# CSU-KangHu/HiTE

Measured on AMD Instinct MI355X. Metric: candidate TE boundaries/sec on 1 Gbp synthetic genome (fine stage: copy finding+gather+align+vote+judge), higher is better.
Workload: dtype u8; 1 GPU; C3: 1000 Mbp synthetic genome, 2500 TIR + 2500 LTR families, 50000 candidates/GPU judged as TIR (copy finding by minimizer-index lookup inside the timed step; index build 0.0 s untimed); genome_bp=1000000000, candidates_per_gpu=50000, candidate_bases=192511237, copies=799813, copy_table=found, is_te=34225, parallelism=replicated genome, candidates per rank x1, all-gather of 32-B calls

## Files before the change

hite_amd/csrc/hite_align.hip:

```cpp
#include "hite_common.h"
#include "hite_scan.h"
#include "hite_arena.h"
#include "hite_sort.h"
#include "hite_align.h"

#define AL_GAP 3
#define AL_STEER 24
#define AL_MARGIN 48
#define AL_PADR 1056
#define AL_WIDE_NW 64
#define AL_STRIP 16
#define AL_RECB 4096
#define AL_DEFAULT_CAP 8
#define AL_KBINS 2048
#define AL_LANES_MIN_STRIPS 32

struct AlignArgs {
    const uint8_t *win;
    const int64_t *win_off;
    const int32_t *win_len;
    const int32_t *row_first;
    int n_cand;
    const int32_t *row_cand;
    const uint4 *planes;
    const int64_t *plane_off;
    const unsigned long long *rec;
    int32_t *U, *kst, *st, *lvl, *U4;
    const int64_t *ops_base;
    uint16_t *ops;
    const int64_t *full_off;
    uint32_t *fullbuf;
    int32_t *fullt;
};

__device__ __forceinline__ uint32_t alignbit(uint32_t hi, uint32_t lo, uint32_t sh) { return __builtin_amdgcn_alignbit(hi, lo, sh); }
__device__ __forceinline__ uint32_t add_co_mask(uint32_t a, uint32_t b, unsigned long long &carry_mask) {
    uint32_t r;
    asm volatile("v_add_co_u32_e64 %0, %1, %2, %3" : "=v"(r), "=s"(carry_mask) : "v"(a), "v"(b));
    return r;
}
__device__ __forceinline__ uint32_t add_mask_bit(uint32_t a, unsigned long long mask) {
    uint32_t r;
    unsigned long long dummy;
    asm volatile("v_addc_co_u32_e64 %0, %1, %2, 0, %3" : "=v"(r), "=s"(dummy) : "v"(a), "s"(mask));
    return r;
}
__device__ __forceinline__ int wave_max_i32(int v) {
#pragma unroll
    for (int d = 32; d >= 1; d >>= 1) { int o = __shfl_xor(v, d, 64); v = o > v ? o : v; }
    return v;
}
__device__ __forceinline__ bool is_acgt_byte(unsigned c) { c &= 0xdfu; return c - 0x41u < 32u && ((0x00080045u >> (c - 0x41u)) & 1u); }

struct BaseMask { uint32_t m0, m1, inv; };
__device__ __forceinline__ BaseMask base_mask(unsigned ch) {
    BaseMask b;
    b.m0 = (uint32_t)(-(int)((ch >> 1) & 1u));
    b.m1 = (uint32_t)(-(int)((ch >> 2) & 1u));
    b.inv = is_acgt_byte(ch) ? 0u : 0xffffffffu;
    return b;
}

template <int NW, bool DIRS, int TAP>
__device__ __forceinline__ void bp_core(uint32_t (&X2)[NW], uint32_t (&X1)[NW], uint32_t (&X0)[NW], const uint32_t (&A0)[NW],
                                        const uint32_t (&A1)[NW], const uint32_t (&AN)[NW], const BaseMask bm, uint32_t cin, uint32_t vpc,
                                        uint32_t h2c, uint32_t h1c, uint32_t h0c, uint32_t *dg, uint32_t *up, uint32_t *tap) {
#pragma unroll
    for (int w = 0; w < NW; w++) {
        if (TAP >= 0 && w == TAP) { tap[0] = cin; tap[1] = vpc; tap[2] = h2c; tap[3] = h1c; tap[4] = h0c; }
        const uint32_t eq = ~((A0[w] ^ bm.m0) | (A1[w] ^ bm.m1) | AN[w] | bm.inv);
        const uint32_t x2 = X2[w], x1 = X1[w], x0 = X0[w];
        const uint32_t vneg = ~(x2 | x1 | x0), vpos = x2 & x1;
        const uint32_t B = eq | vneg, P = (vpos << 1) | vpc;
        vpc = vpos >> 31;
        const uint32_t Y = P | B;
        unsigned cout;
        const uint32_t sum = __builtin_addc(B, Y, cin, &cout);
        cin = cout;
        const uint32_t Z = B | (P & (sum ^ B ^ Y));
        const uint32_t h0 = ~(Z ^ x0), b1 = Z & x0, h1 = ~(x1 ^ b1), b2 = x1 & b1, h2 = ~(x2 ^ b2);
        const uint32_t s2 = (h2 << 1) | h2c, s1 = (h1 << 1) | h1c, s0 = (h0 << 1) | h0c;
        h2c = h2 >> 31; h1c = h1 >> 31; h0c = h0 >> 31;
        const uint32_t n0 = ~(Z ^ s0), c1 = Z & s0, n1 = ~(s1 ^ c1), c2 = s1 & c1, n2 = ~(s2 ^ c2);
        X2[w] = n2; X1[w] = n1; X0[w] = n0;
        if (DIRS) { dg[w] = eq | ~Z; up[w] = n2 & n1; }
    }
}
__device__ __forceinline__ int slope_count(uint32_t x2, uint32_t x1, uint32_t x0) { return __popc(x2) - __popc(~x2 & ~(x1 & x0)); }
__device__ __forceinline__ int plane_sum(uint32_t x2, uint32_t x1, uint32_t x0, uint32_t mask) {
    return 4 * __popc(x2 & mask) + 2 * __popc(x1 & mask) + __popc(x0 & mask);
}

__global__ void __launch_bounds__(256) align_rows_kernel(int n_cand, const int32_t *__restrict__ row_first,
                                                         const int32_t *__restrict__ win_len, int32_t *__restrict__ row_cand,
                                                         int32_t *__restrict__ strips, unsigned long long *__restrict__ keys,
                                                         unsigned *__restrict__ vals) {
    const int c = blockIdx.x;
    if (c >= n_cand) return;
    const int g0 = row_first[c], g1 = row_first[c + 1];
    for (int g = g0 + threadIdx.x; g < g1; g += 256) {
        row_cand[g] = c;
        const int k = g == g0 ? 0 : (win_len[g] + AL_STRIP - 1) / AL_STRIP;
        strips[g] = k;
        keys[g] = (unsigned long long)(AL_KBINS - 1 - (k >= AL_KBINS ? AL_KBINS - 1 : k));
        vals[g] = (unsigned)g;
    }
}
__global__ void align_plane_words_kernel(int n_cand, const int32_t *__restrict__ row_first, const int32_t *__restrict__ win_len,
                                         int32_t *__restrict__ words) {
    const int c = blockIdx.x * blockDim.x + threadIdx.x;
    if (c >= n_cand) return;
    const int g0 = row_first[c];
    words[c] = row_first[c + 1] > g0 ? (win_len[g0] + 2 * AL_PADR) / 32 + 3 : 0;
}
__global__ void __launch_bounds__(256) align_planes_kernel(int n_cand, const uint8_t *__restrict__ win, const int64_t *__restrict__ win_off,
                                                           const int32_t *__restrict__ win_len, const int32_t *__restrict__ row_first,
                                                           const int64_t *__restrict__ plane_off, uint4 *__restrict__ planes) {
    const int c = blockIdx.x;
    if (c >= n_cand) return;
    const int g0 = row_first[c];
    if (row_first[c + 1] <= g0) return;
    const int m = win_len[g0];
    const uint8_t *a = win + win_off[g0];
    const int nw = (m + 2 * AL_PADR) / 32 + 3;
    uint4 *out = planes + plane_off[c];
    for (int wi = threadIdx.x; wi < nw; wi += 256) {
        uint32_t p0 = 0, p1 = 0, pn = 0;
        unsigned chs[32];
#pragma unroll
        for (int k = 0; k < 32; k++) {
            const int r = wi * 32 + k - AL_PADR + 1;
            chs[k] = a[r < 1 || m < 1 ? 0 : (r > m ? m - 1 : r - 1)];
        }
#pragma unroll
        for (int k = 0; k < 32; k++) {
            const int r = wi * 32 + k - AL_PADR + 1;
            const unsigned ch = (r >= 1 && r <= m) ? chs[k] : 0u;
            if (is_acgt_byte(ch)) { p0 |= ((ch >> 1) & 1u) << k; p1 |= ((ch >> 2) & 1u) << k; }
            else pn |= 1u << k;
        }
        out[wi] = make_uint4(p0, p1, pn, 0u);
    }
}

#ifdef ALIGN_CLOCKS
#define ALIGN_CLK_MAX (1 << 17)
__device__ unsigned long long g_aclk[2][4][ALIGN_CLK_MAX];
extern "C" int hite_debug_align_clocks(int which, unsigned long long *out, int n) {
    if (which < 0 || which > 1 || n > ALIGN_CLK_MAX) return -1;
    for (int k = 0; k < 4; k++)
        if (hipMemcpyFromSymbol(out + (size_t)k * n, HIP_SYMBOL(g_aclk), sizeof(unsigned long long) * n,
                                ((size_t)which * 4 + k) * ALIGN_CLK_MAX * sizeof(unsigned long long)) != hipSuccess) return -1;
    unsigned long long *z = (unsigned long long *)calloc((size_t)4 * ALIGN_CLK_MAX, sizeof(unsigned long long));
    if (z) { (void)hipMemcpyToSymbol(HIP_SYMBOL(g_aclk), z, sizeof(unsigned long long) * 4 * ALIGN_CLK_MAX, (size_t)which * 4 * ALIGN_CLK_MAX * sizeof(unsigned long long)); free(z); }
    return 0;
}
__device__ __forceinline__ unsigned aclk_hw_id() {
    unsigned v, x;
    asm volatile("s_getreg_b32 %0, hwreg(HW_REG_HW_ID)" : "=s"(v));
    asm volatile("s_getreg_b32 %0, hwreg(HW_REG_XCC_ID)" : "=s"(x));
    return ((x & 0xfu) << 16) | (v & 0xffffu);
}
#define ACLK_BEGIN(which) const unsigned long long aclk_t0 = wall_clock64(); const int aclk_w = (which)
#define ACLK_END() do { if (threadIdx.x == 0 && blockIdx.x < ALIGN_CLK_MAX) { g_aclk[aclk_w][0][blockIdx.x] = aclk_t0; \
    g_aclk[aclk_w][1][blockIdx.x] = wall_clock64(); g_aclk[aclk_w][2][blockIdx.x] = aclk_hw_id(); g_aclk[aclk_w][3][blockIdx.x] = (unsigned long long)nmax; } } while (0)
#else
#define ACLK_BEGIN(which) do { } while (0)
#define ACLK_END() do { } while (0)
#endif

template <int NW>
__device__ __forceinline__ void align_fwd_body(const AlignArgs &P, const int32_t *__restrict__ list, int nlist) {
    constexpr int W = 32 * NW, H = W / 2, S0 = NW / 2 - 1;
    ACLK_BEGIN(0);
    const int li = blockIdx.x * 64 + threadIdx.x;
    const int g = li < nlist ? list[li] : -1;
    int m = 0, n = 0, g0 = 0, c = 0;
    if (g >= 0) {
        c = P.row_cand[g];
        g0 = P.row_first[c];
        if (g != g0) { m = P.win_len[g0]; n = P.win_len[g]; }
    }
    const int nmax = wave_max_i32(n);
    if (nmax == 0) return;
    const uint8_t *b = P.win + (g >= 0 ? P.win_off[g] : 0);
    const uint4 *pl = P.planes + (g >= 0 ? P.plane_off[c] : 0);
    char *rec0 = g >= 0 ? reinterpret_cast<char *>(P.rec[g]) : nullptr;
    uint32_t X2[NW], X1[NW], X0[NW], A0[NW], A1[NW], AN[NW];
    int t = -H;
#pragma unroll
    for (int w = 0; w < NW; w++) { X2[w] = w >= NW / 2 ? 0xffffffffu : 0u; X1[w] = X2[w]; X0[w] = 0u; }
    bool act = n > 0;
    if (act) {
        const int q0 = (t + AL_PADR) >> 5;
#pragma unroll
        for (int w = 0; w < NW; w++) { const uint4 v = pl[q0 + w]; A0[w] = v.x; A1[w] = v.y; AN[w] = v.z; }
    } else {
#pragma unroll
        for (int w = 0; w < NW; w++) { A0[w] = 0; A1[w] = 0; AN[w] = 0xffffffffu; }
    }
    int stop = AL_GAP * H, LO = -(1 << 28), HI = 1 << 28, status = 0;
    int fq = (t + W + AL_PADR) >> 5;
    uint4 Wa = make_uint4(0, 0, 0xffffffffu, 0), Wb = Wa, Wc = Wa, bnext = make_uint4(0, 0, 0, 0);
    if (act) { Wa = pl[fq]; Wb = pl[fq + 1]; Wc = pl[fq + 2]; bnext = *reinterpret_cast<const uint4 *>(b); }
    for (int k = 0; k * AL_STRIP < nmax; k++) {
        const bool sa = act && k * AL_STRIP < n;
        uint4 bw = make_uint4(0, 0, 0, 0);
        uint32_t f0 = 0, f1 = 0, fn = 0;
        uint32_t brec[8] = {0, 0, 0, 0, 0, 0, 0, 0};
        if (sa) {
            uint4 *ck = reinterpret_cast<uint4 *>(rec0 + (size_t)k * AL_RECB);
            ck[0] = make_uint4(X2[S0], X2[S0 + 1], X1[S0], X1[S0 + 1]);
            ck[1] = make_uint4(X0[S0], X0[S0 + 1], (uint32_t)(t + 32 * S0), 0u);
            bw = bnext;
            if ((k + 1) * AL_STRIP < n) bnext = *reinterpret_cast<const uint4 *>(b + (k + 1) * AL_STRIP);
            const int fx = t + W + AL_PADR;
            if ((fx >> 5) != fq) { Wa = Wb; Wb = Wc; fq++; Wc = pl[fq + 2]; }
            const uint32_t sh = (uint32_t)fx & 31u;
            f0 = alignbit(Wb.x, Wa.x, sh); f1 = alignbit(Wb.y, Wa.y, sh); fn = alignbit(Wb.z, Wa.z, sh);
        }
#pragma unroll
        for (int cc = 0; cc < AL_STRIP; cc++) {
            const int j = k * AL_STRIP + cc + 1;
            if (sa && j <= n) {
                if ((cc & 3) == 0) {
                    const int ds = slope_count(X2[S0], X1[S0], X0[S0]) + slope_count(X2[S0 + 1], X1[S0 + 1], X0[S0 + 1]);
                    int s = ds > AL_STEER ? 0 : (ds < -AL_STEER ? 8 : 4);
                    const int tr = m - H;
                    if (t + s > tr) s = (tr - t) & ~3;
                    const int need = tr - 3 - 8 * ((n - j) >> 2) - t;
                    if (s < need) s = (need + 3) & ~3;
                    if (s > 8) { status = 2; act = false; s = 8; }
                    stop += plane_sum(X2[0], X1[0], X0[0], (1u << s) - 1u) - AL_GAP * s;
                    unsigned long long rec = (unsigned long long)(s >> 2);
                    if (NW > 2) {
                        rec |= (unsigned long long)(X2[S0 + 2 < NW ? S0 + 2 : 0] & 0xffu) << 2;
                        rec |= (unsigned long long)(X1[S0 + 2 < NW ? S0 + 2 : 0] & 0xffu) << 10;
                        rec |= (unsigned long long)(X0[S0 + 2 < NW ? S0 + 2 : 0] & 0xffu) << 18;
                    }
                    brec[(cc >> 2) * 2] = (uint32_t)rec;
#pragma unroll
                    for (int w = 0; w < NW - 1; w++) {
                        X2[w] = alignbit(X2[w + 1], X2[w], (uint32_t)s); X1[w] = alignbit(X1[w + 1], X1[w], (uint32_t)s);
                        X0[w] = alignbit(X0[w + 1], X0[w], (uint32_t)s);
                        A0[w] = alignbit(A0[w + 1], A0[w], (uint32_t)s); A1[w] = alignbit(A1[w + 1], A1[w], (uint32_t)s);
                        AN[w] = alignbit(AN[w + 1], AN[w], (uint32_t)s);
                    }
                    X2[NW - 1] = alignbit(0xffffffffu, X2[NW - 1], (uint32_t)s);
                    X1[NW - 1] = alignbit(0xffffffffu, X1[NW - 1], (uint32_t)s);
                    X0[NW - 1] = X0[NW - 1] >> s;
                    A0[NW - 1] = alignbit(f0, A0[NW - 1], (uint32_t)s); A1[NW - 1] = alignbit(f1, A1[NW - 1], (uint32_t)s);
                    AN[NW - 1] = alignbit(fn, AN[NW - 1], (uint32_t)s);
                    f0 >>= s; f1 >>= s; fn >>= s;
                    t += s;
                    if (t >= 1) { const int v = t + 1 - j; LO = v > LO ? v : LO; }
                    if (t + W < m) { const int jl = j + 3 < n ? j + 3 : n; const int v = t + W - jl; HI = v < HI ? v : HI; }
                }
                stop += AL_GAP;
                const uint32_t word = cc < 4 ? bw.x : (cc < 8 ? bw.y : (cc < 12 ? bw.z : bw.w));
                const BaseMask bm = base_mask((word >> (8 * (cc & 3))) & 0xffu);
                uint32_t tap[5] = {0, 0, 1, 1, 0};
                bp_core<NW, false, (NW > 2 ? S0 : -1)>(X2, X1, X0, A0, A1, AN, bm, 0u, 0u, 1u, 1u, 0u, nullptr, nullptr, tap);
                if (NW > 2) {
                    const uint32_t c5 = tap[0] | (tap[1] << 1) | (tap[2] << 2) | (tap[3] << 3) | (tap[4] << 4);
                    const int sh = 26 + 5 * (cc & 3);
                    if (sh + 5 <= 32) brec[(cc >> 2) * 2] |= c5 << sh;
                    else if (sh >= 32) brec[(cc >> 2) * 2 + 1] |= c5 << (sh - 32);
                    else { brec[(cc >> 2) * 2] |= c5 << sh; brec[(cc >> 2) * 2 + 1] |= c5 >> (32 - sh); }
                    brec[(cc >> 2) * 2 + 1] |= ((bm.m0 & 1u) | (bm.m1 & 2u) | (bm.inv & 4u)) << (14 + 3 * (cc & 3));
                }
            }
        }
        if (NW > 2 && sa) {
            uint4 *bp = reinterpret_cast<uint4 *>(rec0 + (size_t)k * AL_RECB + AL_RECB / 2);
            bp[0] = make_uint4(brec[0], brec[1], brec[2], brec[3]);
            bp[1] = make_uint4(brec[4], brec[5], brec[6], brec[7]);
        }
    }
    if (n > 0) {
        int U = -1, kstar = -1;
        if (status == 0) {
            int u = stop - AL_GAP * H;
#pragma unroll
            for (int w = 0; w < NW / 2; w++) u += plane_sum(X2[w], X1[w], X0[w], 0xffffffffu);
            {
                const int extra = m - H - t;
                u += plane_sum(X2[NW / 2], X1[NW / 2], X0[NW / 2], (1u << extra) - 1u) - AL_GAP * extra;
            }
            U = u;
            const int d = m - n, dmin = d < 0 ? d : 0, dmax = d > 0 ? d : 0, ad = d < 0 ? -d : d;
            int E = dmin - LO;
            if (HI - dmax < E) E = HI - dmax;
            if (E > (1 << 27)) kstar = 0x7fffffff;
            else if (E >= 0) kstar = AL_GAP * ad + 2 * AL_GAP * E + 2 * AL_GAP - 1;
        }
        P.U[g] = U; P.kst[g] = kstar; P.st[g] = status; P.lvl[g] = NW;
        if (NW == 4) P.U4[g] = U;
    }
    if (NW == 4) ACLK_END();
}
template <int NW>
__global__ void __launch_bounds__(64) align_fwd_kernel(AlignArgs P, const int32_t *__restrict__ list, int nlist) { align_fwd_body<NW>(P, list, nlist); }
#ifdef ALIGN_FWD4_OCC
#define ALIGN_FWD4_ATTR __attribute__((amdgpu_waves_per_eu(ALIGN_FWD4_OCC, ALIGN_FWD4_OCC)))
#else
#define ALIGN_FWD4_ATTR
#endif
__global__ void __launch_bounds__(64) ALIGN_FWD4_ATTR align_fwd4_kernel(AlignArgs P, const int32_t *__restrict__ list, int nlist) { align_fwd_body<4>(P, list, nlist); }

__device__ __forceinline__ uint32_t pair_partner(uint32_t v) { return (uint32_t)__builtin_amdgcn_update_dpp(0, (int)v, 0xB1, 0xf, 0xf, false); }

__global__ void __launch_bounds__(64) align_fwd8_pair_kernel(AlignArgs P, const int32_t *__restrict__ list, int nlist) {
    constexpr int NW = 8, HW = 4, W = 32 * NW, H = W / 2, S0 = NW / 2 - 1;
    const int half = threadIdx.x & 1;
    const int li = blockIdx.x * 32 + (threadIdx.x >> 1);
    const int g = li < nlist ? list[li] : -1;
    int m = 0, n = 0, g0 = 0, c = 0;
    if (g >= 0) {
        c = P.row_cand[g];
        g0 = P.row_first[c];
        if (g != g0) { m = P.win_len[g0]; n = P.win_len[g]; }
    }
    const int nmax = wave_max_i32(n);
    if (nmax == 0) return;
    const uint8_t *b = P.win + (g >= 0 ? P.win_off[g] : 0);
    const uint4 *pl = P.planes + (g >= 0 ? P.plane_off[c] : 0);
    char *rec0 = g >= 0 ? reinterpret_cast<char *>(P.rec[g]) : nullptr;
    uint32_t X2[HW], X1[HW], X0[HW], A0[HW], A1[HW], AN[HW];
    int t = -H;
#pragma unroll
    for (int w = 0; w < HW; w++) { X2[w] = half ? 0xffffffffu : 0u; X1[w] = X2[w]; X0[w] = 0u; }
    bool act = n > 0;
    if (act) {
        const int q0 = ((t + AL_PADR) >> 5) + half * HW;
#pragma unroll
        for (int w = 0; w < HW; w++) { const uint4 v = pl[q0 + w]; A0[w] = v.x; A1[w] = v.y; AN[w] = v.z; }
    } else {
#pragma unroll
        for (int w = 0; w < HW; w++) { A0[w] = 0; A1[w] = 0; AN[w] = 0xffffffffu; }
    }
    int stop = AL_GAP * H, LO = -(1 << 28), HI = 1 << 28, status = 0;
    int fq = (t + W + AL_PADR) >> 5;
    uint4 Wa = make_uint4(0, 0, 0xffffffffu, 0), Wb = Wa, Wc = Wa, bnext = make_uint4(0, 0, 0, 0);
    if (act) { Wa = pl[fq]; Wb = pl[fq + 1]; Wc = pl[fq + 2]; bnext = *reinterpret_cast<const uint4 *>(b); }
    for (int k = 0; k * AL_STRIP < nmax; k++) {
        const bool sa = act && k * AL_STRIP < n;
        uint4 bw = make_uint4(0, 0, 0, 0);
        uint32_t f0 = 0, f1 = 0, fn = 0;
        uint32_t brec[8] = {0, 0, 0, 0, 0, 0, 0, 0};
        {
            const uint32_t p2 = pair_partner(X2[0]), p1 = pair_partner(X1[0]), p0 = pair_partner(X0[0]);
            if (sa && !half) {
                uint4 *ck = reinterpret_cast<uint4 *>(rec0 + (size_t)k * AL_RECB);
                ck[0] = make_uint4(X2[HW - 1], p2, X1[HW - 1], p1);
                ck[1] = make_uint4(X0[HW - 1], p0, (uint32_t)(t + 32 * S0), 0u);
            }
        }
        if (sa) {
            bw = bnext;
            if ((k + 1) * AL_STRIP < n) bnext = *reinterpret_cast<const uint4 *>(b + (k + 1) * AL_STRIP);
            const int fx = t + W + AL_PADR;
            if ((fx >> 5) != fq) { Wa = Wb; Wb = Wc; fq++; Wc = pl[fq + 2]; }
            const uint32_t sh = (uint32_t)fx & 31u;
            f0 = alignbit(Wb.x, Wa.x, sh); f1 = alignbit(Wb.y, Wa.y, sh); fn = alignbit(Wb.z, Wa.z, sh);
        }
#pragma unroll
        for (int cc = 0; cc < AL_STRIP; cc++) {
            const int j = k * AL_STRIP + cc + 1;
            const bool on = sa && j <= n;
            if ((cc & 3) == 0) {
                const int own = half ? slope_count(X2[0], X1[0], X0[0]) : slope_count(X2[HW - 1], X1[HW - 1], X0[HW - 1]);
                const int ds = own + (int)pair_partner((uint32_t)own);
                const uint32_t i2 = pair_partner(X2[1] & 0xffu), i1 = pair_partner(X1[1] & 0xffu), i0 = pair_partner(X0[1] & 0xffu);
                const uint32_t u2 = pair_partner(X2[0]), u1 = pair_partner(X1[0]), u0 = pair_partner(X0[0]);
                const uint32_t ua0 = pair_partner(A0[0]), ua1 = pair_partner(A1[0]), uan = pair_partner(AN[0]);
                if (on) {
                    int s = ds > AL_STEER ? 0 : (ds < -AL_STEER ? 8 : 4);
                    const int tr = m - H;
                    if (t + s > tr) s = (tr - t) & ~3;
                    const int need = tr - 3 - 8 * ((n - j) >> 2) - t;
                    if (s < need) s = (need + 3) & ~3;
                    if (s > 8) { status = 2; act = false; s = 8; }
                    if (!half) {
                        stop += plane_sum(X2[0], X1[0], X0[0], (1u << s) - 1u) - AL_GAP * s;
                        brec[(cc >> 2) * 2] = (uint32_t)(s >> 2) | (i2 << 2) | (i1 << 10) | (i0 << 18);
                    }
#pragma unroll
                    for (int w = 0; w < HW - 1; w++) {
                        X2[w] = alignbit(X2[w + 1], X2[w], (uint32_t)s); X1[w] = alignbit(X1[w + 1], X1[w], (uint32_t)s);
                        X0[w] = alignbit(X0[w + 1], X0[w], (uint32_t)s);
                        A0[w] = alignbit(A0[w + 1], A0[w], (uint32_t)s); A1[w] = alignbit(A1[w + 1], A1[w], (uint32_t)s);
                        AN[w] = alignbit(AN[w + 1], AN[w], (uint32_t)s);
                    }
                    X2[HW - 1] = alignbit(half ? 0xffffffffu : u2, X2[HW - 1], (uint32_t)s);
                    X1[HW - 1] = alignbit(half ? 0xffffffffu : u1, X1[HW - 1], (uint32_t)s);
                    X0[HW - 1] = alignbit(half ? 0u : u0, X0[HW - 1], (uint32_t)s);
                    A0[HW - 1] = alignbit(half ? f0 : ua0, A0[HW - 1], (uint32_t)s);
                    A1[HW - 1] = alignbit(half ? f1 : ua1, A1[HW - 1], (uint32_t)s);
                    AN[HW - 1] = alignbit(half ? fn : uan, AN[HW - 1], (uint32_t)s);
                    f0 >>= s; f1 >>= s; fn >>= s;
                    t += s;
                    if (t >= 1) { const int v = t + 1 - j; LO = v > LO ? v : LO; }
                    if (t + W < m) { const int jl = j + 3 < n ? j + 3 : n; const int v = t + W - jl; HI = v < HI ? v : HI; }
                }
            }
            const uint32_t word = cc < 4 ? bw.x : (cc < 8 ? bw.y : (cc < 12 ? bw.z : bw.w));
            const BaseMask bm = base_mask((word >> (8 * (cc & 3))) & 0xffu);
            uint32_t Bv[HW], Pv[HW], Yv[HW], Sv[HW], eqv[HW], vposv[HW];
#pragma unroll
            for (int w = 0; w < HW; w++) {
                eqv[w] = ~((A0[w] ^ bm.m0) | (A1[w] ^ bm.m1) | AN[w] | bm.inv);
                vposv[w] = X2[w] & X1[w];
                Bv[w] = eqv[w] | ~(X2[w] | X1[w] | X0[w]);
            }
            const uint32_t pvpos = pair_partner(vposv[HW - 1]);
            const uint32_t vin = half ? pvpos >> 31 : 0u;
            uint32_t cin = 0u, tap0 = 0u;
#pragma unroll
            for (int w = 0; w < HW; w++) {
                if (w == HW - 1) tap0 = cin;
                Pv[w] = (vposv[w] << 1) | (w ? vposv[w - 1] >> 31 : vin);
                Yv[w] = Pv[w] | Bv[w];
                unsigned cout;
                Sv[w] = __builtin_addc(Bv[w], Yv[w], cin, &cout);
                cin = cout;
            }
            {
                const uint32_t pc = pair_partner(cin);
                uint32_t e = half ? pc : 0u;
#pragma unroll
                for (int w = 0; w < HW; w++) { const uint32_t o = Sv[w]; Sv[w] = o + e; e &= (o == 0xffffffffu) ? 1u : 0u; }
            }
            uint32_t Zv[HW], h2v[HW], h1v[HW], h0v[HW];
#pragma unroll
            for (int w = 0; w < HW; w++) {
                Zv[w] = Bv[w] | (Pv[w] & (Sv[w] ^ Bv[w] ^ Yv[w]));
                const uint32_t b1 = Zv[w] & X0[w], b2 = X1[w] & b1;
                h0v[w] = ~(Zv[w] ^ X0[w]); h1v[w] = ~(X1[w] ^ b1); h2v[w] = ~(X2[w] ^ b2);
            }
            const uint32_t q2 = pair_partner(h2v[HW - 1]) >> 31, q1 = pair_partner(h1v[HW - 1]) >> 31, q0 = pair_partner(h0v[HW - 1]) >> 31;
            const uint32_t hin2 = half ? q2 : 1u, hin1 = half ? q1 : 1u, hin0 = half ? q0 : 0u;
            if (on) {
#pragma unroll
                for (int w = 0; w < HW; w++) {
                    const uint32_t s2 = (h2v[w] << 1) | (w ? h2v[w - 1] >> 31 : hin2), s1 = (h1v[w] << 1) | (w ? h1v[w - 1] >> 31 : hin1),
                                   s0 = (h0v[w] << 1) | (w ? h0v[w - 1] >> 31 : hin0);
                    const uint32_t c1 = Zv[w] & s0, c2 = s1 & c1;
                    X0[w] = ~(Zv[w] ^ s0); X1[w] = ~(s1 ^ c1); X2[w] = ~(s2 ^ c2);
                }
                if (!half) {
                    stop += AL_GAP;
                    const uint32_t c5 = tap0 | ((vposv[HW - 2] >> 31) << 1) | ((h2v[HW - 2] >> 31) << 2) | ((h1v[HW - 2] >> 31) << 3) | ((h0v[HW - 2] >> 31) << 4);
                    const int sh = 26 + 5 * (cc & 3);
                    if (sh + 5 <= 32) brec[(cc >> 2) * 2] |= c5 << sh;
                    else if (sh >= 32) brec[(cc >> 2) * 2 + 1] |= c5 << (sh - 32);
                    else { brec[(cc >> 2) * 2] |= c5 << sh; brec[(cc >> 2) * 2 + 1] |= c5 >> (32 - sh); }
                    brec[(cc >> 2) * 2 + 1] |= ((bm.m0 & 1u) | (bm.m1 & 2u) | (bm.inv & 4u)) << (14 + 3 * (cc & 3));
                }
            }
        }
        if (sa && !half) {
            uint4 *bp = reinterpret_cast<uint4 *>(rec0 + (size_t)k * AL_RECB + AL_RECB / 2);
            bp[0] = make_uint4(brec[0], brec[1], brec[2], brec[3]);
            bp[1] = make_uint4(brec[4], brec[5], brec[6], brec[7]);
        }
    }
    {
        const int extra = m - H - t;
        const uint32_t part = pair_partner((uint32_t)plane_sum(X2[0], X1[0], X0[0], (1u << (extra & 31)) - 1u));
        if (n > 0 && !half) {
            int U = -1, kstar = -1;
            if (status == 0) {
                int u = stop - AL_GAP * H;
#pragma unroll
                for (int w = 0; w < HW; w++) u += plane_sum(X2[w], X1[w], X0[w], 0xffffffffu);
                u += (int)part - AL_GAP * extra;
                U = u;
                const int d = m - n, dmin = d < 0 ? d : 0, dmax = d > 0 ? d : 0, ad = d < 0 ? -d : d;
                int E = dmin - LO;
                if (HI - dmax < E) E = HI - dmax;
                if (E > (1 << 27)) kstar = 0x7fffffff;
                else if (E >= 0) kstar = AL_GAP * ad + 2 * AL_GAP * E + 2 * AL_GAP - 1;
            }
            P.U[g] = U; P.kst[g] = kstar; P.st[g] = status; P.lvl[g] = NW;
        }
    }
}

template <int CTRL>
__device__ __forceinline__ uint32_t dpp_row(uint32_t v) { return (uint32_t)__builtin_amdgcn_update_dpp(0, (int)v, CTRL, 0xf, 0xf, true); }
template <int G>
__device__ __forceinline__ int grp_sum(int v) {
    v += (int)dpp_row<0xB1>((uint32_t)v);
    v += (int)dpp_row<0x4E>((uint32_t)v);
    if (G == 8) v += (int)dpp_row<0x141>((uint32_t)v);
    return v;
}
__device__ __forceinline__ int wave_min_i32(int v) {
#pragma unroll
    for (int d = 32; d >= 1; d >>= 1) { int o = __shfl_xor(v, d, 64); v = o < v ? o : v; }
    return v;
}
__device__ __forceinline__ uint32_t bit_mask(uint32_t w, int bit) { return (uint32_t)((int32_t)(w << (31 - bit)) >> 31); }
template <int GI>
__device__ __forceinline__ uint32_t quad_bcast(uint32_t v) { return dpp_row<GI * 0x55>(v); }
struct LaneFwd {
    uint32_t X2, X1, X0, A0, A1, AN, f0, f1, fn;
    int t, stop, LO, HI, status;
    bool act;
};
template <int G, bool FULL>
__device__ __forceinline__ void lanes_strip(LaneFwd &S, const uint4 bw, const uint32_t invm, const uint32_t code12, const bool sa, const int k,
                                            const int m, const int n, const int q, const uint32_t K1, const unsigned long long TOPM, uint32_t (&brec)[8]) {
    constexpr int NW = G, W = 32 * NW, H = W / 2, S0 = NW / 2 - 1;
    const bool top = q == G - 1;
#pragma unroll
    for (int cc = 0; cc < AL_STRIP; cc++) {
        const int j = k * AL_STRIP + cc + 1;
        const bool on = FULL || (sa && j <= n);
        if ((cc & 3) == 0) {
            const int ds = grp_sum<G>((q == S0 || q == S0 + 1) ? slope_count(S.X2, S.X1, S.X0) : 0);
            const uint32_t i2 = dpp_row<0x102>(S.X2) & 0xffu, i1 = dpp_row<0x102>(S.X1) & 0xffu, i0 = dpp_row<0x102>(S.X0) & 0xffu;
            const uint32_t u2 = dpp_row<0x101>(S.X2), u1 = dpp_row<0x101>(S.X1), u0 = dpp_row<0x101>(S.X0);
            const uint32_t ua0 = dpp_row<0x101>(S.A0), ua1 = dpp_row<0x101>(S.A1), uan = dpp_row<0x101>(S.AN);
            constexpr int gi = 0;
            const uint32_t cg = (cc >> 2) == 0 ? quad_bcast<0>(code12) : ((cc >> 2) == 1 ? quad_bcast<1>(code12) : ((cc >> 2) == 2 ? quad_bcast<2>(code12) : quad_bcast<3>(code12)));
            (void)gi;
            if (on) {
                int s = ds > AL_STEER ? 0 : (ds < -AL_STEER ? 8 : 4);
                const int tr = m - H;
                if (S.t + s > tr) s = (tr - S.t) & ~3;
                const int need = tr - 3 - 8 * ((n - j) >> 2) - S.t;
                if (s < need) s = (need + 3) & ~3;
                if (s > 8) { S.status = 2; S.act = false; s = 8; }
                S.stop += plane_sum(S.X2, S.X1, S.X0, (1u << s) - 1u) - AL_GAP * s;
                brec[(cc >> 2) * 2] = (uint32_t)(s >> 2) | (i2 << 2) | (i1 << 10) | (i0 << 18);
                brec[(cc >> 2) * 2 + 1] = cg << 14;
                S.X2 = alignbit(top ? 0xffffffffu : u2, S.X2, (uint32_t)s);
                S.X1 = alignbit(top ? 0xffffffffu : u1, S.X1, (uint32_t)s);
                S.X0 = alignbit(top ? 0u : u0, S.X0, (uint32_t)s);
                S.A0 = alignbit(top ? S.f0 : ua0, S.A0, (uint32_t)s);
                S.A1 = alignbit(top ? S.f1 : ua1, S.A1, (uint32_t)s);
                S.AN = alignbit(top ? S.fn : uan, S.AN, (uint32_t)s);
                S.f0 >>= s; S.f1 >>= s; S.fn >>= s;
                S.t += s;
                if (S.t >= 1) { const int v = S.t + 1 - j; S.LO = v > S.LO ? v : S.LO; }
                if (S.t + W < m) { const int jl = j + 3 < n ? j + 3 : n; const int v = S.t + W - jl; S.HI = v < S.HI ? v : S.HI; }
            }
        }
        const uint32_t word = cc < 4 ? bw.x : (cc < 8 ? bw.y : (cc < 12 ? bw.z : bw.w));
        const uint32_t m0 = bit_mask(word, 8 * (cc & 3) + 1), m1 = bit_mask(word, 8 * (cc & 3) + 2), inv = bit_mask(invm, cc);
        const uint32_t eq = ~((S.A0 ^ m0) | (S.A1 ^ m1) | S.AN | inv);
        const uint32_t vpos = S.X2 & S.X1;
        const uint32_t B = eq | ~(S.X2 | S.X1 | S.X0);
        const uint32_t pvr = dpp_row<0x111>(vpos);
        const uint32_t Pp = alignbit(vpos, pvr, 31) & ~K1;
        const uint32_t Y = Pp | B;
        unsigned long long Gm;
        const uint32_t sum0 = add_co_mask(B, Y, Gm);
        uint32_t sum;
        {
            const unsigned long long Pm = __ballot(sum0 == 0xffffffffu);
            const unsigned long long Gc = Gm & ~TOPM, Yy = (Pm | Gm) & ~TOPM, ss = Gc + Yy;
            sum = add_mask_bit(sum0, ss ^ Gc ^ Yy);
        }
        const uint32_t Z = B | (Pp & (sum ^ B ^ Y));
        const uint32_t h0 = ~(Z ^ S.X0), b1 = Z & S.X0, h1 = ~(S.X1 ^ b1), b2 = S.X1 & b1, h2 = ~(S.X2 ^ b2);
        const uint32_t r2 = dpp_row<0x111>(h2), r1 = dpp_row<0x111>(h1), r0 = dpp_row<0x111>(h0);
        if (on) {
            const uint32_t s2 = alignbit(h2, r2, 31) | K1, s1 = alignbit(h1, r1, 31) | K1, s0 = alignbit(h0, r0, 31) & ~K1;
            const uint32_t c1 = Z & s0, c2 = s1 & c1;
            S.X0 = ~(Z ^ s0); S.X1 = ~(s1 ^ c1); S.X2 = ~(s2 ^ c2);
            uint32_t c5 = alignbit(r0 >> 31, r1, 31);
            c5 = alignbit(c5, r2, 31);
            c5 = alignbit(c5, pvr, 31);
            c5 = (c5 << 1) | (sum - sum0);
            const int sh = 26 + 5 * (cc & 3);
            if (sh + 5 <= 32) brec[(cc >> 2) * 2] |= c5 << sh;
            else if (sh >= 32) brec[(cc >> 2) * 2 + 1] |= c5 << (sh - 32);
            else { brec[(cc >> 2) * 2] |= c5 << sh; brec[(cc >> 2) * 2 + 1] |= c5 >> (32 - sh); }
        }
    }
}
__device__ __forceinline__ uint32_t decode_bases4(uint32_t w) {
    uint32_t r = 0;
#pragma unroll
    for (int x = 0; x < 4; x++) {
        const unsigned ch = (w >> (8 * x)) & 0xffu;
        const uint32_t bad = is_acgt_byte(ch) ? 0u : 1u;
        r |= (bad << x) | ((((ch >> 1) & 3u) | (bad << 2)) << (4 + 3 * x));
    }
    return r;
}
template <int G>
__global__ void __launch_bounds__(64) align_fwd_lanes_kernel(AlignArgs P, const int32_t *__restrict__ list, int nlist) {
    constexpr int NW = G, W = 32 * NW, H = W / 2, S0 = NW / 2 - 1, PPW = 64 / G;
    const int q = threadIdx.x & (G - 1);
    const int li = blockIdx.x * PPW + (int)(threadIdx.x / G);
    const int g = li < nlist ? list[li] : -1;
    int m = 0, n = 0, g0 = 0, c = 0;
    if (g >= 0) {
        c = P.row_cand[g];
        g0 = P.row_first[c];
        if (g != g0) { m = P.win_len[g0]; n = P.win_len[g]; }
    }
    const int nmax = wave_max_i32(n);
    if (nmax == 0) return;
    const int nfull = wave_min_i32(n > 0 ? n : 0x7fffffff);
    const bool wr = q == S0;
    const uint32_t K1 = q == 0 ? 1u : 0u;
    const unsigned long long TOPM = G == 4 ? 0x8888888888888888ull : 0x8080808080808080ull;
    const uint8_t *b = P.win + (g >= 0 ? P.win_off[g] : 0);
    const uint4 *pl = P.planes + (g >= 0 ? P.plane_off[c] : 0);
    char *rec0 = g >= 0 ? reinterpret_cast<char *>(P.rec[g]) : nullptr;
    LaneFwd S;
    S.X2 = q >= NW / 2 ? 0xffffffffu : 0u; S.X1 = S.X2; S.X0 = 0u; S.A0 = 0u; S.A1 = 0u; S.AN = 0xffffffffu;
    S.f0 = S.f1 = S.fn = 0u;
    S.t = -H;
    S.act = n > 0;
    if (S.act) { const uint4 v = pl[((S.t + AL_PADR) >> 5) + q]; S.A0 = v.x; S.A1 = v.y; S.AN = v.z; }
    S.stop = AL_GAP * H; S.LO = -(1 << 28); S.HI = 1 << 28; S.status = 0;
    int fq = (S.t + W + AL_PADR) >> 5;
    uint4 Wa = make_uint4(0, 0, 0xffffffffu, 0), Wb = Wa, Wc = Wa, bnext = make_uint4(0, 0, 0, 0);
    if (S.act) { Wa = pl[fq]; Wb = pl[fq + 1]; Wc = pl[fq + 2]; bnext = *reinterpret_cast<const uint4 *>(b); }
    for (int k = 0; k * AL_STRIP < nmax; k++) {
        const bool sa = S.act && k * AL_STRIP < n;
        uint4 bw = make_uint4(0, 0, 0, 0);
        uint32_t brec[8] = {0, 0, 0, 0, 0, 0, 0, 0};
        {
            const uint32_t p2 = dpp_row<0x101>(S.X2), p1 = dpp_row<0x101>(S.X1), p0 = dpp_row<0x101>(S.X0);
            if (sa && wr) {
                uint4 *ck = reinterpret_cast<uint4 *>(rec0 + (size_t)k * AL_RECB);
                ck[0] = make_uint4(S.X2, p2, S.X1, p1);
                ck[1] = make_uint4(S.X0, p0, (uint32_t)(S.t + 32 * S0), 0u);
            }
        }
        S.f0 = S.f1 = S.fn = 0u;
        if (sa) {
            bw = bnext;
            if ((k + 1) * AL_STRIP < n) bnext = *reinterpret_cast<const uint4 *>(b + (k + 1) * AL_STRIP);
            const int fx = S.t + W + AL_PADR;
            if ((fx >> 5) != fq) { Wa = Wb; Wb = Wc; fq++; Wc = pl[fq + 2]; }
            const uint32_t sh = (uint32_t)fx & 31u;
            S.f0 = alignbit(Wb.x, Wa.x, sh); S.f1 = alignbit(Wb.y, Wa.y, sh); S.fn = alignbit(Wb.z, Wa.z, sh);
        }
        const uint32_t dq = (q & 3) == 0 ? bw.x : ((q & 3) == 1 ? bw.y : ((q & 3) == 2 ? bw.z : bw.w));
        const uint32_t dec = decode_bases4(dq);
        uint32_t invm = (dec & 15u) << (4 * (q & 3));
        invm |= dpp_row<0xB1>(invm);
        invm |= dpp_row<0x4E>(invm);
        const bool failed = __any(n > 0 && S.status != 0);
        if ((k + 1) * AL_STRIP <= nfull && !failed) lanes_strip<G, true>(S, bw, invm, dec >> 4, sa, k, m, n, q, K1, TOPM, brec);
        else lanes_strip<G, false>(S, bw, invm, dec >> 4, sa, k, m, n, q, K1, TOPM, brec);
        if (sa && wr) {
            uint4 *bp = reinterpret_cast<uint4 *>(rec0 + (size_t)k * AL_RECB + AL_RECB / 2);
            bp[0] = make_uint4(brec[0], brec[1], brec[2], brec[3]);
            bp[1] = make_uint4(brec[4], brec[5], brec[6], brec[7]);
        }
    }
    {
        const int extra = m - H - S.t;
        const int part = q < NW / 2 ? plane_sum(S.X2, S.X1, S.X0, 0xffffffffu) : (q == NW / 2 ? plane_sum(S.X2, S.X1, S.X0, (1u << (extra & 31)) - 1u) : 0);
        const int tot = grp_sum<G>(part + (q == 0 ? S.stop : 0));
        if (n > 0 && wr) {
            int U = -1, kstar = -1;
            if (S.status == 0) {
                U = tot + AL_GAP * n - AL_GAP * H - AL_GAP * extra;
                const int d = m - n, dmin = d < 0 ? d : 0, dmax = d > 0 ? d : 0, ad = d < 0 ? -d : d;
                int E = dmin - S.LO;
                if (S.HI - dmax < E) E = S.HI - dmax;
                if (E > (1 << 27)) kstar = 0x7fffffff;
                else if (E >= 0) kstar = AL_GAP * ad + 2 * AL_GAP * E + 2 * AL_GAP - 1;
            }
            P.U[g] = U; P.kst[g] = kstar; P.st[g] = S.status; P.lvl[g] = NW;
            if (NW == 4) P.U4[g] = U;
        }
    }
}

typedef unsigned int tb_u32x4 __attribute__((ext_vector_type(4)));
#if defined(ALIGN_TB_STORE8)
struct OpsOut {
    uint16_t *ops;
    unsigned long long acc, top;
    int m;
    __device__ __forceinline__ void init(uint16_t *row, int m_) { ops = row; m = m_; acc = 0ull; top = 0ull; }
    __device__ __forceinline__ void push(int pos, uint32_t val) {
        acc = (acc << 16) | (unsigned long long)(val & 0xffffu);
        if ((pos & 3) == 0) {
            if (pos + 4 <= m) *reinterpret_cast<unsigned long long *>(ops + pos) = acc;
            else top = acc;
        }
    }
    __device__ __forceinline__ void finish() {
        const int k = m & 3, p0 = m & ~3;
        for (int x = 0; x < k; x++) ops[p0 + x] = (uint16_t)(top >> (16 * x));
    }
};
#elif defined(ALIGN_TB_STORE32)
struct OpsOut {
    uint16_t *ops;
    unsigned long long acc;
    unsigned long long g0, g1, g2, g3;
    int m, off;
    int q_low;
    __device__ __forceinline__ void init(uint16_t *row, int m_) {
        ops = row; m = m_; acc = 0ull; g0 = g1 = g2 = g3 = 0ull;
        off = (int)((reinterpret_cast<uintptr_t>(row) >> 1) & 15);
        q_low = m_ + off;
    }
    __device__ __forceinline__ uint16_t held(int q, int q_acc_low) const {
        if ((q >> 2) == (q_acc_low >> 2) && (q_acc_low & 3)) return (uint16_t)(acc >> (16 * (q - q_acc_low)));
        const int g = (q >> 2) & 3;
        const unsigned long long s = g == 0 ? g0 : (g == 1 ? g1 : (g == 2 ? g2 : g3));
        return (uint16_t)(s >> (16 * (q & 3)));
    }
    __device__ __forceinline__ void push(int pos, uint32_t val) {
        acc = (acc << 16) | (unsigned long long)(val & 0xffffu);
        const int q = pos + off;
        if ((q & 3) == 0) {
            const int g = (q >> 2) & 3;
            g0 = g == 0 ? acc : g0; g1 = g == 1 ? acc : g1; g2 = g == 2 ? acc : g2; g3 = g == 3 ? acc : g3;
            if (g == 0) {
                if (pos + 16 <= m) {
                    tb_u32x4 *dst = reinterpret_cast<tb_u32x4 *>(ops + pos);
                    tb_u32x4 v0, v1;
                    v0.x = (unsigned)g0; v0.y = (unsigned)(g0 >> 32); v0.z = (unsigned)g1; v0.w = (unsigned)(g1 >> 32);
                    v1.x = (unsigned)g2; v1.y = (unsigned)(g2 >> 32); v1.z = (unsigned)g3; v1.w = (unsigned)(g3 >> 32);
                    dst[0] = v0; dst[1] = v1;
                } else {
                    for (int x = pos; x < m; x++) ops[x] = held(x + off, q);
                }
                q_low = q;
            }
        }
    }
    __device__ __forceinline__ void finish() {
        const int top = q_low - off < m ? q_low - off : m;
        for (int x = 0; x < top; x++) ops[x] = held(x + off, off);
    }
};

#else
struct OpsOut {
    uint16_t *ops;
    unsigned long long acc, hi;
    unsigned long long tacc, thi;
    int m, off;
    __device__ __forceinline__ void init(uint16_t *row, int m_) {
        ops = row; m = m_; acc = 0ull; hi = 0ull; tacc = 0ull; thi = 0ull;
        off = (int)((reinterpret_cast<uintptr_t>(row) >> 1) & 7);
    }
    __device__ __forceinline__ void push(int pos, uint32_t val) {
        acc = (acc << 16) | (unsigned long long)(val & 0xffffu);
        const int q = pos + off;
        if ((q & 3) == 0) {
            if (q & 4) hi = acc;
            else if (pos + 8 <= m) {
                tb_u32x4 v;
                v.x = (unsigned)acc; v.y = (unsigned)(acc >> 32); v.z = (unsigned)hi; v.w = (unsigned)(hi >> 32);
                *reinterpret_cast<tb_u32x4 *>(ops + pos) = v;
            } else { tacc = acc; thi = hi; }
        }
    }
    __device__ __forceinline__ void finish() {
        const int t0 = m - ((m + off) & 7);
        if (t0 >= 0) for (int x = t0; x < m; x++) { const int qq = x + off; ops[x] = (uint16_t)(((qq & 4) ? thi : tacc) >> (16 * (qq & 3))); }
        const int b0 = (8 - off) & 7;
        const int lowm = b0 < m ? b0 : m;
        for (int x = 0; x < lowm; x++) {
            const int qq = x + off;
            const bool in_acc = (off & 3) != 0 && (qq >> 2) == (off >> 2);
            ops[x] = in_acc ? (uint16_t)(acc >> (16 * x)) : (uint16_t)(hi >> (16 * (qq & 3)));
        }
    }
};
#endif

#ifdef ALIGN_TB_OCC
#define ALIGN_TB_ATTR __attribute__((amdgpu_waves_per_eu(ALIGN_TB_OCC, ALIGN_TB_OCC)))
#else
#define ALIGN_TB_ATTR
#endif
__global__ void __launch_bounds__(64) ALIGN_TB_ATTR align_tb_kernel(AlignArgs P, const int32_t *__restrict__ list, int nlist) {
    ACLK_BEGIN(1);
    const int li = blockIdx.x * 64 + threadIdx.x;
    const int g = li < nlist ? list[li] : -1;
    int m = 0, n = 0, g0 = 0, c = 0;
    if (g >= 0) {
        c = P.row_cand[g];
        g0 = P.row_first[c];
        if (g != g0 && P.st[g] == 0) { m = P.win_len[g0]; n = P.win_len[g]; }
    }
    const int nmax = wave_max_i32(n);
    if (nmax == 0) return;
    const uint4 *pl = P.planes + (g >= 0 ? P.plane_off[c] : 0);
    const char *rec0 = g >= 0 ? reinterpret_cast<const char *>(P.rec[g]) : nullptr;
    uint16_t *ops = P.ops + (g >= 0 ? P.ops_base[c] + (int64_t)(g - g0) * (m + 1) : 0);
    int i = m, j = n;
    bool fail = false;
    OpsOut out;
    out.init(ops, m);
    const int Kmax = (nmax + AL_STRIP - 1) / AL_STRIP;
    const int K = (n + AL_STRIP - 1) / AL_STRIP;
    struct Pw { uint32_t x, y, z; };
    uint4 ckA0, ckA1, ckB0, ckB1, bdA0, bdA1;
    Pw plA[4];
    ckA0 = ckA1 = ckB0 = ckB1 = bdA0 = bdA1 = make_uint4(0, 0, 0, 0);
#pragma unroll
    for (int w = 0; w < 4; w++) { plA[w].x = 0; plA[w].y = 0; plA[w].z = 0; }
    {
        const int k = Kmax - 1;
        if (k < K) {
            const uint4 *ck = reinterpret_cast<const uint4 *>(rec0 + (size_t)k * AL_RECB);
            ckA0 = ck[0]; ckA1 = ck[1];
            const uint4 *bp = reinterpret_cast<const uint4 *>(rec0 + (size_t)k * AL_RECB + AL_RECB / 2);
            bdA0 = bp[0]; bdA1 = bp[1];
            const int q0 = ((int)ckA1.z + AL_PADR) >> 5;
#pragma unroll
            for (int w = 0; w < 4; w++) { const uint4 v = pl[q0 + w]; plA[w].x = v.x; plA[w].y = v.y; plA[w].z = v.z; }
        }
        if (k >= 1 && k - 1 < K) {
            const uint4 *ck = reinterpret_cast<const uint4 *>(rec0 + (size_t)(k - 1) * AL_RECB);
            ckB0 = ck[0]; ckB1 = ck[1];
        }
    }
    for (int k = Kmax - 1; k >= 0; k--) {
        const bool sa = n > 0 && !fail && i > 0 && k < K;
        uint4 ckC0 = make_uint4(0, 0, 0, 0), ckC1 = ckC0, bdB0 = ckC0, bdB1 = ckC0;
        Pw plB[4];
#pragma unroll
        for (int w = 0; w < 4; w++) { plB[w].x = 0; plB[w].y = 0; plB[w].z = 0; }
        if (k >= 1 && k - 1 < K && !fail && i > 0) {
            const uint4 *bp = reinterpret_cast<const uint4 *>(rec0 + (size_t)(k - 1) * AL_RECB + AL_RECB / 2);
            bdB0 = bp[0]; bdB1 = bp[1];
            const int q0 = ((int)ckB1.z + AL_PADR) >> 5;
#pragma unroll
            for (int w = 0; w < 4; w++) { const uint4 v = pl[q0 + w]; plB[w].x = v.x; plB[w].y = v.y; plB[w].z = v.z; }
        }
        if (k >= 2 && k - 2 < K && !fail && i > 0) {
            const uint4 *ck = reinterpret_cast<const uint4 *>(rec0 + (size_t)(k - 2) * AL_RECB);
            ckC0 = ck[0]; ckC1 = ck[1];
        }
        if (__any(sa)) {
        uint32_t X2[2], X1[2], X0[2], A0[2], A1[2], AN[2];
        uint32_t f0 = 0, f1 = 0, fn = 0;
        uint32_t brec[8] = {0, 0, 0, 0, 0, 0, 0, 0};
        int t = 0;
        if (sa) {
            X2[0] = ckA0.x; X2[1] = ckA0.y; X1[0] = ckA0.z; X1[1] = ckA0.w; X0[0] = ckA1.x; X0[1] = ckA1.y;
            t = (int)ckA1.z;
            brec[0] = bdA0.x; brec[1] = bdA0.y; brec[2] = bdA0.z; brec[3] = bdA0.w;
            brec[4] = bdA1.x; brec[5] = bdA1.y; brec[6] = bdA1.z; brec[7] = bdA1.w;
            const uint32_t sh = (uint32_t)(t + AL_PADR) & 31u;
#pragma unroll
            for (int w = 0; w < 2; w++) {
                A0[w] = alignbit(plA[w + 1].x, plA[w].x, sh); A1[w] = alignbit(plA[w + 1].y, plA[w].y, sh);
                AN[w] = alignbit(plA[w + 1].z, plA[w].z, sh);
            }
            f0 = alignbit(plA[3].x, plA[2].x, sh); f1 = alignbit(plA[3].y, plA[2].y, sh); fn = alignbit(plA[3].z, plA[2].z, sh);
        } else {
#pragma unroll
            for (int w = 0; w < 2; w++) { X2[w] = 0; X1[w] = 0; X0[w] = 0; A0[w] = 0; A1[w] = 0; AN[w] = 0; }
        }
        unsigned long long dg[AL_STRIP], up[AL_STRIP];
        uint32_t sbits = 0;
#pragma unroll
        for (int cc = 0; cc < AL_STRIP; cc++) {
            const int jc = k * AL_STRIP + cc + 1;
            dg[cc] = 0ull; up[cc] = 0ull;
            if (sa && jc <= n) {
                const uint32_t rlo = brec[(cc >> 2) * 2], rhi = brec[(cc >> 2) * 2 + 1];
                if ((cc & 3) == 0) {
                    const uint32_t s = (rlo & 3u) << 2;
                    const uint32_t in2 = (rlo >> 2) & 0xffu, in1 = (rlo >> 10) & 0xffu, in0 = (rlo >> 18) & 0xffu;
                    X2[0] = alignbit(X2[1], X2[0], s); X1[0] = alignbit(X1[1], X1[0], s); X0[0] = alignbit(X0[1], X0[0], s);
                    A0[0] = alignbit(A0[1], A0[0], s); A1[0] = alignbit(A1[1], A1[0], s); AN[0] = alignbit(AN[1], AN[0], s);
                    X2[1] = alignbit(in2, X2[1], s); X1[1] = alignbit(in1, X1[1], s); X0[1] = alignbit(in0, X0[1], s);
                    A0[1] = alignbit(f0, A0[1], s); A1[1] = alignbit(f1, A1[1], s); AN[1] = alignbit(fn, AN[1], s);
                    f0 >>= s; f1 >>= s; fn >>= s;
                    t += (int)s;
                    sbits |= (rlo & 3u) << (2 * (cc >> 2));
                }
                const int sh = 26 + 5 * (cc & 3);
                const uint32_t c5 = (sh + 5 <= 32 ? rlo >> sh : (sh >= 32 ? rhi >> (sh - 32) : (rlo >> sh) | (rhi << (32 - sh)))) & 31u;
                const uint32_t code = rhi >> (14 + 3 * (cc & 3));
                BaseMask bm;
                bm.m0 = 0u - (code & 1u); bm.m1 = 0u - ((code >> 1) & 1u); bm.inv = 0u - ((code >> 2) & 1u);
                uint32_t tap[5], dgc[2], upc[2];
                bp_core<2, true, -1>(X2, X1, X0, A0, A1, AN, bm, c5 & 1u, (c5 >> 1) & 1u, (c5 >> 2) & 1u, (c5 >> 3) & 1u, (c5 >> 4) & 1u, dgc, upc, tap);
                dg[cc] = ((unsigned long long)dgc[1] << 32) | dgc[0];
                up[cc] = ((unsigned long long)upc[1] << 32) | upc[0];
            }
        }
        int tcur = t;
#pragma unroll
        for (int cc = AL_STRIP - 1; cc >= 0; cc--) {
            const int jc = k * AL_STRIP + cc + 1;
            if (sa && !fail && i > 0 && j == jc) {
                const int kb = i - tcur - 1;
                if ((unsigned)kb >= 64u) fail = true;
                else {
                    const unsigned long long stopm = (dg[cc] | ~up[cc]) & (0xffffffffffffffffull >> (63 - kb));
                    if (stopm == 0ull) fail = true;
                    else {
                        const int ps = 63 - __clzll(stopm);
                        int ups = kb - ps;
                        if (ups > i) ups = i;
                        const uint32_t gapv = (uint32_t)j | 0x8000u;
                        for (int x = 0; x < ups; x++) out.push(i - 1 - x, gapv);
                        i -= ups;
                        if (i > 0) {
                            if ((dg[cc] >> ps) & 1ull) { out.push(i - 1, (uint32_t)(j - 1)); i--; j--; }
                            else j--;
                        }
                    }
                }
            }
            if ((cc & 3) == 0) tcur -= (int)(((sbits >> (2 * (cc >> 2))) & 3u) << 2);
        }
        }
        ckA0 = ckB0; ckA1 = ckB1; ckB0 = ckC0; ckB1 = ckC1; bdA0 = bdB0; bdA1 = bdB1;
#pragma unroll
        for (int w = 0; w < 4; w++) plA[w] = plB[w];
    }
    if (n > 0) {
        if (fail) P.st[g] = 1;
        else {
            for (int q = i - 1; q >= 0; q--) out.push(q, 0x8000u);
            out.finish();
        }
    }
    ACLK_END();
}

__device__ __forceinline__ uint32_t lane_above(uint32_t v, uint32_t fill) { return (uint32_t)__builtin_amdgcn_update_dpp((int)fill, (int)v, 0x130, 0xf, 0xf, false); }
__device__ __forceinline__ uint32_t lane_below(uint32_t v, uint32_t fill) { return (uint32_t)__builtin_amdgcn_update_dpp((int)fill, (int)v, 0x138, 0xf, 0xf, false); }
__device__ __forceinline__ int wave_sum_i32(int v) {
#pragma unroll
    for (int d = 32; d >= 1; d >>= 1) v += __shfl_xor(v, d, 64);
    return v;
}

__device__ __forceinline__ uint32_t lane_below_keep(uint32_t v, uint32_t &keep) {
    asm volatile("s_nop 1\n\tv_mov_b32_dpp %0, %1 wave_shr:1 row_mask:0xf bank_mask:0xf" : "+v"(keep) : "v"(v));
    return keep;
}
__device__ __forceinline__ void lane_below_keep3(uint32_t v2, uint32_t v1, uint32_t v0, uint32_t &k2, uint32_t &k1, uint32_t &k0) {
    asm volatile("s_nop 1\n\tv_mov_b32_dpp %0, %3 wave_shr:1 row_mask:0xf bank_mask:0xf\n\tv_mov_b32_dpp %1, %4 wave_shr:1 row_mask:0xf bank_mask:0xf\n\t"
                 "v_mov_b32_dpp %2, %5 wave_shr:1 row_mask:0xf bank_mask:0xf" : "+v"(k2), "+v"(k1), "+v"(k0) : "v"(v2), "v"(v1), "v"(v0));
}
struct WideFwd {
    uint32_t X2, X1, X0, A0, A1, AN, f0, f1, fn;
    uint32_t kz0, kz1, ko0, ko1;
    int t, stop, LO, HI, status;
};
template <bool FULL>
__device__ __forceinline__ void wide_fwd_strip(WideFwd &S, const AlignArgs &P, int lane, int m, int n, int j0, int64_t full0, unsigned long long M0,
                                               unsigned long long M1, unsigned long long MI) {
    constexpr int NW = AL_WIDE_NW, W = 32 * NW, H = W / 2, S0 = NW / 2 - 1;
    uint32_t *fb = P.fullbuf + (full0 + j0) * (2 * NW) + lane;
#pragma unroll
    for (int cc = 0; cc < AL_STRIP; cc++) {
        const int j = j0 + cc;
        if (FULL || (j <= n && S.status == 0)) {
            if ((cc & 3) == 0) {
                const int dv = slope_count(S.X2, S.X1, S.X0);
                const int ds = __builtin_amdgcn_readlane(dv, S0) + __builtin_amdgcn_readlane(dv, S0 + 1);
                int s = ds > AL_STEER ? 0 : (ds < -AL_STEER ? 8 : 4);
                const int tr = m - H;
                if (S.t + s > tr) s = (tr - S.t) & ~3;
                const int need = tr - 3 - 8 * ((n - j) >> 2) - S.t;
                if (s < need) s = (need + 3) & ~3;
                if (s > 8) { S.status = 2; s = 8; }
                const uint32_t smask = (1u << s) - 1u;
                S.stop += plane_sum((uint32_t)__builtin_amdgcn_readlane((int)S.X2, 0), (uint32_t)__builtin_amdgcn_readlane((int)S.X1, 0),
                                    (uint32_t)__builtin_amdgcn_readlane((int)S.X0, 0), smask) - AL_GAP * s;
                S.X2 = alignbit(lane_above(S.X2, 0xffffffffu), S.X2, (uint32_t)s);
                S.X1 = alignbit(lane_above(S.X1, 0xffffffffu), S.X1, (uint32_t)s);
                S.X0 = alignbit(lane_above(S.X0, 0u), S.X0, (uint32_t)s);
                S.A0 = alignbit(lane_above(S.A0, S.f0), S.A0, (uint32_t)s);
                S.A1 = alignbit(lane_above(S.A1, S.f1), S.A1, (uint32_t)s);
                S.AN = alignbit(lane_above(S.AN, S.fn), S.AN, (uint32_t)s);
                S.f0 >>= s; S.f1 >>= s; S.fn >>= s;
                S.t += s;
                if (S.t >= 1) { const int v = S.t + 1 - j; S.LO = v > S.LO ? v : S.LO; }
                if (S.t + W < m) { const int jl = j + 3 < n ? j + 3 : n; const int v = S.t + W - jl; S.HI = v < S.HI ? v : S.HI; }
                if (lane < 4 && j + lane <= n) P.fullt[full0 + j + lane] = S.t;
            }
            S.stop += AL_GAP;
            BaseMask bm;
            bm.m0 = 0u - (uint32_t)((M0 >> cc) & 1ull); bm.m1 = 0u - (uint32_t)((M1 >> cc) & 1ull); bm.inv = 0u - (uint32_t)((MI >> cc) & 1ull);
            const uint32_t eq = ~((S.A0 ^ bm.m0) | (S.A1 ^ bm.m1) | S.AN | bm.inv);
            const uint32_t vneg = ~(S.X2 | S.X1 | S.X0), vpos = S.X2 & S.X1;
            const uint32_t B = eq | vneg, Pp = alignbit(vpos, lane_below_keep(vpos, S.kz0), 31);
            const uint32_t Y = Pp | B;
            unsigned long long Gm;
            uint32_t sum = add_co_mask(B, Y, Gm);
            {
                const unsigned long long Pm = __ballot(sum == 0xffffffffu);
                const unsigned long long Yy = Pm | Gm, ss = Gm + Yy;
                const unsigned long long into = ss ^ Gm ^ Yy;
                sum = add_mask_bit(sum, into);
            }
            const uint32_t Z = B | (Pp & (sum ^ B ^ Y));
            const uint32_t h0 = ~(Z ^ S.X0), b1 = Z & S.X0, h1 = ~(S.X1 ^ b1), b2 = S.X1 & b1, h2 = ~(S.X2 ^ b2);
            lane_below_keep3(h2, h1, h0, S.ko0, S.ko1, S.kz1);
            const uint32_t s2 = alignbit(h2, S.ko0, 31), s1 = alignbit(h1, S.ko1, 31), s0 = alignbit(h0, S.kz1, 31);
            const uint32_t n0 = ~(Z ^ s0), c1 = Z & s0, n1 = ~(s1 ^ c1), c2 = s1 & c1, n2 = ~(s2 ^ c2);
            S.X2 = n2; S.X1 = n1; S.X0 = n0;
            fb[cc * (2 * NW)] = eq | ~Z;
            fb[cc * (2 * NW) + NW] = n2 & n1;
        }
    }
}
__global__ void __launch_bounds__(64) align_wide_fwd_kernel(AlignArgs P, const int32_t *__restrict__ list, int nlist) {
    constexpr int NW = AL_WIDE_NW, W = 32 * NW, H = W / 2;
    const int pi = blockIdx.x;
    if (pi >= nlist) return;
    const int lane = threadIdx.x;
    const int g = list[pi];
    const int c = P.row_cand[g], g0 = P.row_first[c];
    if (g == g0) return;
    const int m = P.win_len[g0], n = P.win_len[g];
    const uint8_t *b = P.win + P.win_off[g];
    const uint4 *pl = P.planes + P.plane_off[c];
    const int64_t full0 = P.full_off[g];
    WideFwd S;
    S.t = -H;
    S.X2 = lane >= NW / 2 ? 0xffffffffu : 0u; S.X1 = S.X2; S.X0 = 0u;
    { const uint4 v = pl[((S.t + AL_PADR) >> 5) + lane]; S.A0 = v.x; S.A1 = v.y; S.AN = v.z; }
    S.stop = AL_GAP * H; S.LO = -(1 << 28); S.HI = 1 << 28; S.status = 0;
    S.kz0 = 0u; S.kz1 = 0u; S.ko0 = 0x80000000u; S.ko1 = 0x80000000u;
    unsigned chn = b[lane & 15];
    for (int j0 = 1; j0 <= n && S.status == 0; j0 += AL_STRIP) {
        const unsigned ch = chn;
        chn = b[j0 - 1 + AL_STRIP + (lane & 15)];
        const unsigned long long M0 = __ballot((ch >> 1) & 1u), M1 = __ballot((ch >> 2) & 1u), MI = __ballot(!is_acgt_byte(ch));
        {
            const int fx = S.t + W + AL_PADR;
            const uint4 F = pl[fx >> 5], G = pl[(fx >> 5) + 1];
            const uint32_t sh = (uint32_t)fx & 31u;
            S.f0 = alignbit(G.x, F.x, sh); S.f1 = alignbit(G.y, F.y, sh); S.fn = alignbit(G.z, F.z, sh);
        }
        if (j0 + AL_STRIP - 1 <= n) wide_fwd_strip<true>(S, P, lane, m, n, j0, full0, M0, M1, MI);
        else wide_fwd_strip<false>(S, P, lane, m, n, j0, full0, M0, M1, MI);
    }
    int U = -1, kstar = -1;
    if (S.status == 0) {
        const int extra = m - H - S.t;
        U = S.stop - AL_GAP * H - AL_GAP * extra +
            wave_sum_i32(lane < NW / 2 ? plane_sum(S.X2, S.X1, S.X0, 0xffffffffu) : (lane == NW / 2 ? plane_sum(S.X2, S.X1, S.X0, (1u << extra) - 1u) : 0));
        const int d = m - n, dmin = d < 0 ? d : 0, dmax = d > 0 ? d : 0, ad = d < 0 ? -d : d;
        int E = dmin - S.LO;
        if (S.HI - dmax < E) E = S.HI - dmax;
        if (E > (1 << 27)) kstar = 0x7fffffff;
        else if (E >= 0) kstar = AL_GAP * ad + 2 * AL_GAP * E + 2 * AL_GAP - 1;
    }
    if (lane == 0) { P.U[g] = U; P.kst[g] = kstar; P.st[g] = S.status; P.lvl[g] = NW | 0x100; }
}

struct WideOps {
    uint16_t *ops;
    int m, lane;
    uint32_t acc;
    __device__ __forceinline__ void flush(int base) { if (base + lane < m) ops[base + lane] = (uint16_t)acc; }
    __device__ __forceinline__ void put(int pos, uint32_t val) {
        if (lane == (pos & 63)) acc = val;
        if ((pos & 63) == 0) flush(pos);
    }
    __device__ __forceinline__ void run_diag(int hi, int count, int delta) {
        while (count > 0) {
            const int base = hi & ~63;
            const int lo = hi - count + 1 > base ? hi - count + 1 : base;
            if (base + lane >= lo && base + lane <= hi) acc = (uint32_t)(base + lane + delta);
            const int k = hi - lo + 1;
            count -= k; hi -= k;
            if (lo == base) flush(base);
        }
    }
    __device__ __forceinline__ void run(int hi, int count, uint32_t val) {
        while (count > 0) {
            const int base = hi & ~63;
            const int lo = hi - count + 1 > base ? hi - count + 1 : base;
            if (base + lane >= lo && base + lane <= hi) acc = val;
            const int k = hi - lo + 1;
            count -= k; hi -= k;
            if (lo == base) flush(base);
        }
    }
};
__global__ void __launch_bounds__(64) align_wide_tb_kernel(AlignArgs P, const int32_t *__restrict__ list, int nlist) {
    constexpr int NW = AL_WIDE_NW, W = 32 * NW, PF = 8;
    const int pi = blockIdx.x;
    if (pi >= nlist) return;
    const int lane = threadIdx.x;
    const int g = list[pi];
    const int c = P.row_cand[g], g0 = P.row_first[c];
    if (g == g0 || P.st[g] != 0) return;
    const int m = P.win_len[g0], n = P.win_len[g];
    WideOps out;
    out.ops = P.ops + P.ops_base[c] + (int64_t)(g - g0) * (m + 1); out.m = m; out.lane = lane; out.acc = 0u;
    const int64_t full0 = P.full_off[g];
    int i = m, j = n;
    bool fail = false;
    uint32_t dgn[PF];
    int ttn[PF];
#pragma unroll
    for (int q = 0; q < PF; q++) {
        const int jq = j - q > 0 ? j - q : 1;
        dgn[q] = P.fullbuf[(full0 + jq) * (2 * NW) + lane]; ttn[q] = P.fullt[full0 + jq];
    }
    while (i > 0 && j > 0 && !fail) {
        uint32_t dgs[PF];
        int tts[PF];
#pragma unroll
        for (int q = 0; q < PF; q++) { dgs[q] = dgn[q]; tts[q] = ttn[q]; }
#pragma unroll
        for (int q = 0; q < PF; q++) {
            const int jq = j - PF - q > 0 ? j - PF - q : 1;
            dgn[q] = P.fullbuf[(full0 + jq) * (2 * NW) + lane]; ttn[q] = P.fullt[full0 + jq];
        }
#pragma unroll
        for (int q = 0; q < PF; q++) {
            if (i > 0 && j > 0 && !fail) {
                const uint32_t dgw = dgs[q];
                const int kb = i - tts[q] - 1;
                if ((unsigned)kb >= (unsigned)W) fail = true;
                else {
                    const int wq = kb >> 5;
                    const uint32_t dcur = (uint32_t)__builtin_amdgcn_readlane((int)dgw, wq);
                    if ((dcur >> (kb & 31)) & 1u) { out.put(i - 1, (uint32_t)(j - 1)); i--; j--; }
                    else {
                        const uint32_t upw = P.fullbuf[(full0 + j) * (2 * NW) + NW + lane];
                        const uint32_t low = 0xffffffffu >> (31 - (kb & 31));
                        const uint32_t sbit = dgw | ~upw;
                        const uint32_t mk = lane > wq ? 0u : (lane == wq ? sbit & low : sbit);
                        const unsigned long long nz = __ballot(mk != 0u);
                        if (nz == 0ull) fail = true;
                        else {
                            const int tl = 63 - __clzll(nz);
                            const uint32_t mt = (uint32_t)__builtin_amdgcn_readlane((int)mk, tl), dt = (uint32_t)__builtin_amdgcn_readlane((int)dgw, tl);
                            const int ps = 32 * tl + 31 - __clz(mt);
                            int nup = kb - ps;
                            if (nup > i) nup = i;
                            out.run(i - 1, nup, (uint32_t)j | 0x8000u);
                            i -= nup;
                            if (i > 0) {
                                if ((dt >> (ps & 31)) & 1u) { out.put(i - 1, (uint32_t)(j - 1)); i--; j--; }
                                else j--;
                            }
                        }
                    }
                }
            }
        }
    }
    if (fail) { if (lane == 0) P.st[g] = 1; }
    else out.run(i - 1, i, 0x8000u);
}

__device__ __forceinline__ unsigned long long readlane_u64(unsigned long long v, int l) {
    return ((unsigned long long)(uint32_t)__builtin_amdgcn_readlane((int)(uint32_t)(v >> 32), l) << 32) | (uint32_t)__builtin_amdgcn_readlane((int)(uint32_t)v, l);
}
__global__ void __launch_bounds__(64) align_tb_strips_kernel(AlignArgs P, const int32_t *__restrict__ list, int nlist) {
    __shared__ unsigned long long s_dg[64][AL_STRIP + 1], s_up[64][AL_STRIP + 1];
    __shared__ int s_t[64][4];
    const int pi = blockIdx.x;
    if (pi >= nlist) return;
    const int lane = threadIdx.x;
    const int g = list[pi];
    const int c = P.row_cand[g], g0 = P.row_first[c];
    if (g == g0 || P.st[g] != 0) return;
    const int m = P.win_len[g0], n = P.win_len[g];
    if (n <= 0) return;
    const uint4 *pl = P.planes + P.plane_off[c];
    const char *rec0 = reinterpret_cast<const char *>(P.rec[g]);
    WideOps out;
    out.ops = P.ops + P.ops_base[c] + (int64_t)(g - g0) * (m + 1); out.m = m; out.lane = lane; out.acc = 0u;
    const int K = (n + AL_STRIP - 1) / AL_STRIP;
    int i = m, j = n;
    bool fail = false;
    for (int kb0 = K - 1; kb0 >= 0 && !fail && i > 0; kb0 -= 64) {
        {
            const int k = kb0 - lane;
            if (k >= 0) {
                const uint4 *ck = reinterpret_cast<const uint4 *>(rec0 + (size_t)k * AL_RECB);
                const uint4 *bp = reinterpret_cast<const uint4 *>(rec0 + (size_t)k * AL_RECB + AL_RECB / 2);
                const uint4 ck0 = ck[0], ck1 = ck[1], bd0 = bp[0], bd1 = bp[1];
                uint32_t X2[2] = {ck0.x, ck0.y}, X1[2] = {ck0.z, ck0.w}, X0[2] = {ck1.x, ck1.y}, A0[2], A1[2], AN[2];
                int t = (int)ck1.z;
                const uint32_t brec[8] = {bd0.x, bd0.y, bd0.z, bd0.w, bd1.x, bd1.y, bd1.z, bd1.w};
                const int q0 = (t + AL_PADR) >> 5;
                const uint4 p0 = pl[q0], p1 = pl[q0 + 1], p2 = pl[q0 + 2], p3 = pl[q0 + 3];
                const uint32_t sh = (uint32_t)(t + AL_PADR) & 31u;
                A0[0] = alignbit(p1.x, p0.x, sh); A1[0] = alignbit(p1.y, p0.y, sh); AN[0] = alignbit(p1.z, p0.z, sh);
                A0[1] = alignbit(p2.x, p1.x, sh); A1[1] = alignbit(p2.y, p1.y, sh); AN[1] = alignbit(p2.z, p1.z, sh);
                uint32_t f0 = alignbit(p3.x, p2.x, sh), f1 = alignbit(p3.y, p2.y, sh), fn = alignbit(p3.z, p2.z, sh);
#pragma unroll
                for (int cc = 0; cc < AL_STRIP; cc++) {
                    const int jc = k * AL_STRIP + cc + 1;
                    unsigned long long dgv = 0ull, upv = 0ull;
                    if (jc <= n) {
                        const uint32_t rlo = brec[(cc >> 2) * 2], rhi = brec[(cc >> 2) * 2 + 1];
                        if ((cc & 3) == 0) {
                            const uint32_t s = (rlo & 3u) << 2;
                            const uint32_t in2 = (rlo >> 2) & 0xffu, in1 = (rlo >> 10) & 0xffu, in0 = (rlo >> 18) & 0xffu;
                            X2[0] = alignbit(X2[1], X2[0], s); X1[0] = alignbit(X1[1], X1[0], s); X0[0] = alignbit(X0[1], X0[0], s);
                            A0[0] = alignbit(A0[1], A0[0], s); A1[0] = alignbit(A1[1], A1[0], s); AN[0] = alignbit(AN[1], AN[0], s);
                            X2[1] = alignbit(in2, X2[1], s); X1[1] = alignbit(in1, X1[1], s); X0[1] = alignbit(in0, X0[1], s);
                            A0[1] = alignbit(f0, A0[1], s); A1[1] = alignbit(f1, A1[1], s); AN[1] = alignbit(fn, AN[1], s);
                            f0 >>= s; f1 >>= s; fn >>= s;
                            t += (int)s;
                        }
                        const int sh5 = 26 + 5 * (cc & 3);
                        const uint32_t c5 = (sh5 + 5 <= 32 ? rlo >> sh5 : (sh5 >= 32 ? rhi >> (sh5 - 32) : (rlo >> sh5) | (rhi << (32 - sh5)))) & 31u;
                        const uint32_t code = rhi >> (14 + 3 * (cc & 3));
                        BaseMask bm;
                        bm.m0 = 0u - (code & 1u); bm.m1 = 0u - ((code >> 1) & 1u); bm.inv = 0u - ((code >> 2) & 1u);
                        uint32_t tap[5], dgc[2], upc[2];
                        bp_core<2, true, -1>(X2, X1, X0, A0, A1, AN, bm, c5 & 1u, (c5 >> 1) & 1u, (c5 >> 2) & 1u, (c5 >> 3) & 1u, (c5 >> 4) & 1u, dgc, upc, tap);
                        dgv = ((unsigned long long)dgc[1] << 32) | dgc[0];
                        upv = ((unsigned long long)upc[1] << 32) | upc[0];
                    }
                    s_dg[lane][cc] = dgv; s_up[lane][cc] = upv;
                    if ((cc & 3) == 0) s_t[lane][cc >> 2] = t;
                }
            }
        }
        __syncthreads();
        const int nst = kb0 + 1 < 64 ? kb0 + 1 : 64;
        unsigned long long dgn = s_dg[0][lane & 15], upn = s_up[0][lane & 15];
        int tn = s_t[0][(lane & 15) >> 2];
        for (int l = 0; l < nst && !fail && i > 0; l++) {
            const unsigned long long dgl = dgn, upl = upn;
            const int tl = tn;
            if (l + 1 < nst) { dgn = s_dg[l + 1][lane & 15]; upn = s_up[l + 1][lane & 15]; tn = s_t[l + 1][(lane & 15) >> 2]; }
            const int j0 = (kb0 - l) * AL_STRIP;
            while (!fail && i > 0) {
                i = __builtin_amdgcn_readfirstlane(i); j = __builtin_amdgcn_readfirstlane(j);
                const int cur = j - j0 - 1;
                if (cur < 0) break;
                {
                    const int back = cur - (lane & 15);
                    const int kbl = i - back - tl - 1;
                    const bool ok = back >= 0 && i - back >= 1 && (unsigned)kbl < 64u && ((dgl >> (kbl & 63)) & 1ull);
                    const uint32_t okm = (uint32_t)__ballot(ok) & 0xffffu;
                    const uint32_t bad = ~okm & ((2u << cur) - 1u);
                    const int run = bad ? cur - (31 - __clz(bad)) : cur + 1;
                    if (run > 0) { out.run_diag(i - 1, run, j - i); i -= run; j -= run; }
                    if (run == cur + 1 || i <= 0) continue;
                }
                {
                    const int cc = j - j0 - 1;
                    const int kb = i - __builtin_amdgcn_readlane(tl, cc) - 1;
                    if ((unsigned)kb >= 64u) { fail = true; break; }
                    const unsigned long long dgv = readlane_u64(dgl, cc), upv = readlane_u64(upl, cc);
                    const unsigned long long stopm = (dgv | ~upv) & (0xffffffffffffffffull >> (63 - kb));
                    if (stopm == 0ull) { fail = true; break; }
                    const int ps = 63 - __clzll(stopm);
                    int ups = kb - ps;
                    if (ups > i) ups = i;
                    out.run(i - 1, ups, (uint32_t)j | 0x8000u);
                    i -= ups;
                    if (i > 0) {
                        if ((dgv >> ps) & 1ull) { out.put(i - 1, (uint32_t)(j - 1)); i--; j--; }
                        else j--;
                    }
                }
            }
        }
        __syncthreads();
    }
    if (fail) { if (lane == 0) P.st[g] = 1; }
    else out.run(i - 1, i, 0x8000u);
}

__global__ void align_flag_kernel(int64_t nrows, const int32_t *__restrict__ order, const int32_t *__restrict__ strips, AlignArgs P,
                                  int what, int level, int cap, int32_t *__restrict__ flag, int32_t *__restrict__ cols) {
    const int64_t x = (int64_t)blockIdx.x * blockDim.x + threadIdx.x;
    if (x >= nrows) return;
    const int g = order[x];
    int f = 0;
    if (strips[g] > 0) {
        if (what == 0) {
            const int u4 = P.U4[g];
            if (P.st[g] == 0 && u4 >= 0 && u4 + AL_GAP * AL_MARGIN <= 32 * AL_GAP * cap) {
                int first = 8;
                while (32 * AL_GAP * first < u4 + AL_GAP * AL_MARGIN) first *= 2;
                const bool cert = P.U[g] <= P.kst[g];
                f = level >= first && !cert;
            }
        } else if (what == 1) f = P.st[g] == 1;
        else {
            const int u4 = P.U4[g];
            const bool esc = P.st[g] == 0 && u4 >= 0 && u4 + AL_GAP * AL_MARGIN <= 32 * AL_GAP * cap && !(P.U[g] <= P.kst[g]);
            f = what == 2 ? esc : !esc;
        }
    }
    flag[x] = f;
    if (cols) cols[x] = f ? P.win_len[g] + 1 : 0;
}
__global__ void align_compact_kernel(int64_t nrows, const int32_t *__restrict__ order, const int32_t *__restrict__ flag,
                                     const int64_t *__restrict__ pos, int32_t *__restrict__ out, const int64_t *__restrict__ colpos,
                                     int64_t *__restrict__ full_off, int32_t *__restrict__ st) {
    const int64_t x = (int64_t)blockIdx.x * blockDim.x + threadIdx.x;
    if (x >= nrows) return;
    if (flag[x]) {
        const int g = order[x];
        out[pos[x]] = g;
        if (full_off) { full_off[g] = colpos[x]; st[g] = 0; }
    }
}
__global__ void __launch_bounds__(256) align_blockmax_kernel(int64_t cnt, const int32_t *__restrict__ list, const int32_t *__restrict__ strips,
                                                             int32_t *__restrict__ bk) {
    const int64_t x = (int64_t)blockIdx.x * 256 + threadIdx.x;
    const int k = wave_max_i32(x < cnt ? strips[list[x]] : 0);
    if ((threadIdx.x & 63) == 0 && x < cnt) bk[x >> 6] = k;
}
__global__ void align_assign_kernel(int64_t cnt, const int32_t *__restrict__ list, const int64_t *__restrict__ boff, char *region,
                                    unsigned long long *__restrict__ rec) {
    const int64_t x = (int64_t)blockIdx.x * blockDim.x + threadIdx.x;
    if (x < cnt) rec[list[x]] = (unsigned long long)(uintptr_t)(region + boff[x >> 6] * (int64_t)AL_RECB + (x & 63) * 32);
}
struct LaneCost { float thread_chain, lane_chain, thread_work, lane_work; };
__device__ __forceinline__ double lane_cost_at(int64_t k, int64_t nb, const int32_t *bk, const int64_t *boff, const LaneCost c) {
    const double chain_l = k > 0 ? (double)bk[0] * c.lane_chain : 0.0, chain_t = k < nb ? (double)bk[k] * c.thread_chain : 0.0;
    const double work = (double)boff[k] * c.lane_work + (double)(boff[nb] - boff[k]) * c.thread_work;
    double t = chain_l > chain_t ? chain_l : chain_t;
    return t > work ? t : work;
}
__global__ void align_long_blocks_kernel(int64_t nb, const int32_t *__restrict__ bk, const int64_t *__restrict__ boff, int64_t fixed_strips,
                                         LaneCost cf, LaneCost ct, int64_t *__restrict__ out) {
    if (blockIdx.x || threadIdx.x) return;
    for (int w = 0; w < 2; w++) {
        int64_t lo = 0, hi = nb;
        if (fixed_strips >= 0) {
            while (lo < hi) { const int64_t mid = (lo + hi) >> 1; if ((int64_t)bk[mid] >= fixed_strips) lo = mid + 1; else hi = mid; }
        } else {
            const LaneCost c = w ? ct : cf;
            while (lo < hi) {
                const int64_t mid = (lo + hi) >> 1;
                const double a = (double)bk[0] * c.lane_chain, wk = (double)boff[mid] * c.lane_work + (double)(boff[nb] - boff[mid]) * c.thread_work;
                const double tc = mid < nb ? (double)bk[mid] * c.thread_chain : 0.0;
                if ((a > wk ? a : wk) < tc) lo = mid + 1; else hi = mid;
            }
            if (lo > 0 && lane_cost_at(lo - 1, nb, bk, boff, c) <= lane_cost_at(lo, nb, bk, boff, c)) lo--;
            if (lo > 0 && (bk[0] < AL_LANES_MIN_STRIPS || lane_cost_at(lo, nb, bk, boff, c) > 0.9 * lane_cost_at(0, nb, bk, boff, c))) lo = 0;
        }
        out[w] = lo;
    }
}
__global__ void __launch_bounds__(256) align_stats_kernel(int64_t total_rows, const int32_t *__restrict__ strips, AlignArgs P, int32_t *__restrict__ row_dead,
                                                          int32_t *__restrict__ cand_status, unsigned long long *__restrict__ acc) {
    __shared__ unsigned long long s_acc[4][7];
    unsigned long long v[7] = {0, 0, 0, 0, 0, 0, 0};
    for (int64_t g = (int64_t)blockIdx.x * blockDim.x + threadIdx.x; g < total_rows; g += (int64_t)gridDim.x * blockDim.x) {
        if (strips[g] <= 0) {
            const bool empty_row = g != P.row_first[P.row_cand[g]];
            if (empty_row) { P.st[g] = 2; P.U[g] = -1; P.kst[g] = -1; P.lvl[g] = 0; v[0] += 1ull; v[4] += 1ull; }
            if (row_dead) row_dead[g] = empty_row;
            if (empty_row && cand_status) atomicExch(&cand_status[P.row_cand[g]], 2);
        }
        else {
            const int st = P.st[g];
            v[0] += 1ull;
            v[1] += st == 0 && P.U[g] <= P.kst[g];
            v[2] += st == 0 && (P.lvl[g] & 0xff) > 4;
            v[3] += (P.lvl[g] & 0x100) != 0;
            v[4] += st != 0;
            v[5] += st == 0 ? (unsigned long long)P.U[g] : 0ull;
            v[6] += (unsigned long long)P.win_len[g];
            if (row_dead) row_dead[g] = st != 0;
            if (st != 0 && cand_status) atomicExch(&cand_status[P.row_cand[g]], 2);
        }
    }
#pragma unroll
    for (int q = 0; q < 7; q++) {
        unsigned long long x = v[q];
#pragma unroll
        for (int d = 32; d >= 1; d >>= 1) x += __shfl_xor(x, d, 64);
        if ((threadIdx.x & 63) == 0) s_acc[threadIdx.x >> 6][q] = x;
    }
    __syncthreads();
    if (threadIdx.x < 7) {
        const unsigned long long x = s_acc[0][threadIdx.x] + s_acc[1][threadIdx.x] + s_acc[2][threadIdx.x] + s_acc[3][threadIdx.x];
        if (x) atomicAdd(&acc[threadIdx.x], x);
    }
}
__global__ void align_info_kernel(int64_t total_rows, AlignArgs P, int32_t *__restrict__ info ) {
    const int64_t g = (int64_t)blockIdx.x * blockDim.x + threadIdx.x;
    if (g >= total_rows) return;
    const int c = P.row_cand[g];
    if (g == P.row_first[c]) { for (int q = 0; q < 5; q++) info[g * 5 + q] = 0; return; }
    info[g * 5 + 0] = P.U[g];
    info[g * 5 + 1] = P.st[g] != 2 && P.U[g] <= P.kst[g];
    info[g * 5 + 2] = P.st[g];
    info[g * 5 + 3] = P.kst[g];
    info[g * 5 + 4] = P.lvl[g];
}

struct AlignState {
    Arena arena;
    int64_t *h_pin = nullptr;
    int64_t *d_scal = nullptr;
    int exact_cap = -1;
    int lanes_min = -1;
    float lanes_scale[4] = {1.f, 1.f, 1.f, 1.f};
    bool sort_attr = false;
    hipStream_t st2 = nullptr;
    hipEvent_t ev = nullptr, ev_fork = nullptr, ev_join = nullptr;
    int64_t stats[8] = {0, 0, 0, 0, 0, 0, 0, 0};
};

static hipError_t align_make_stream(hipStream_t *out) {
    int lo = 0, hi = 0;
    if (hipDeviceGetStreamPriorityRange(&lo, &hi) != hipSuccess) { lo = 0; hi = 0; }
    return hipStreamCreateWithPriority(out, hipStreamNonBlocking, hi);
}

static AlignState *align_state(hite_ctx *ctx) {
    if (!ctx->align_state) {
        AlignState *S = new AlignState();
        if (hipHostMalloc((void **)&S->h_pin, 64 * sizeof(int64_t)) != hipSuccess || hipMalloc((void **)&S->d_scal, 64 * sizeof(int64_t)) != hipSuccess ||
            align_make_stream(&S->st2) != hipSuccess || hipEventCreateWithFlags(&S->ev, hipEventDisableTiming) != hipSuccess ||
            hipEventCreateWithFlags(&S->ev_fork, hipEventDisableTiming) != hipSuccess || hipEventCreateWithFlags(&S->ev_join, hipEventDisableTiming) != hipSuccess) {
            delete S;
            return nullptr;
        }
        const char *e = getenv("HITE_ALIGN_EXACT");
        int cap = e && *e ? atoi(e) : AL_DEFAULT_CAP;
        if (cap != 0 && cap != 8 && cap != 16 && cap != 32) cap = AL_DEFAULT_CAP;
        S->exact_cap = cap;
        const char *l = getenv("HITE_ALIGN_LANES");
        if (l && *l) { const int v = atoi(l); S->lanes_min = v < -2 ? -1 : v; }
        const char *sc = getenv("HITE_ALIGN_LANES_SCALE");
        if (sc && *sc) sscanf(sc, "%f,%f,%f,%f", &S->lanes_scale[0], &S->lanes_scale[1], &S->lanes_scale[2], &S->lanes_scale[3]);
        ctx->align_state = S;
    }
    return (AlignState *)ctx->align_state;
}
void hite_align_release(hite_ctx *ctx) {
    AlignState *S = (AlignState *)ctx->align_state;
    if (!S) return;
    arena_free(S->arena);
    if (S->h_pin) (void)hipHostFree(S->h_pin);
    if (S->d_scal) (void)hipFree(S->d_scal);
    if (S->st2) (void)hipStreamDestroy(S->st2);
    if (S->ev) (void)hipEventDestroy(S->ev);
    if (S->ev_fork) (void)hipEventDestroy(S->ev_fork);
    if (S->ev_join) (void)hipEventDestroy(S->ev_join);
    delete S;
    ctx->align_state = nullptr;
}

extern "C" int hite_align_config(hite_ctx *ctx, int32_t exact_cap) {
    if (!ctx || (exact_cap != 0 && exact_cap != 8 && exact_cap != 16 && exact_cap != 32)) return HITE_EINVAL;
    AlignState *S = align_state(ctx);
    if (!S) return HITE_ENOMEM;
    S->exact_cap = exact_cap;
    return HITE_OK;
}
extern "C" int hite_align_lanes(hite_ctx *ctx, int32_t min_cols) {
    if (!ctx || min_cols < -2 || min_cols > 32767) return HITE_EINVAL;
    AlignState *S = align_state(ctx);
    if (!S) return HITE_ENOMEM;
    S->lanes_min = min_cols;
    return HITE_OK;
}
extern "C" int hite_align_stats(hite_ctx *ctx, int64_t *out8, int32_t reset) {
    if (!ctx || !out8) return HITE_EINVAL;
    AlignState *S = align_state(ctx);
    if (!S) return HITE_ENOMEM;
    memcpy(out8, S->stats, sizeof S->stats);
    out8[7] = S->exact_cap;
    if (reset) memset(S->stats, 0, sizeof S->stats);
    return HITE_OK;
}

#define ACHK(x) do { int rc__ = (x); if (rc__) return rc__; } while (0)

template <typename T>
static int aalloc(hite_ctx *ctx, Arena &A, size_t count, T **out) {
    void *p = nullptr;
    int rc = arena_alloc(ctx, A, count * sizeof(T), &p);
    *out = (T *)p;
    return rc;
}

static int build_list(hite_ctx *ctx, AlignState *S, hipStream_t st, int64_t nrows, const int32_t *order, const int32_t *strips,
                      AlignArgs &P, int what, int level, int cap, int32_t *flag, int32_t *cols, int64_t *pos, int64_t *colpos,
                      int64_t *scan_tmp, int32_t *list, int64_t *full_off, int64_t *count, int64_t *total_cols, int slot = 0) {
    const unsigned nb = (unsigned)((nrows + 255) / 256);
    hipLaunchKernelGGL(align_flag_kernel, dim3(nb), dim3(256), 0, st, nrows, order, strips, P, what, level, cap, flag, cols);
    ACHK(scan_excl_buf<int32_t>(ctx, scan_tmp, flag, nrows, pos, st));
    if (cols) ACHK(scan_excl_buf<int32_t>(ctx, scan_tmp, cols, nrows, colpos, st));
    hipLaunchKernelGGL(align_compact_kernel, dim3(nb), dim3(256), 0, st, nrows, order, flag, pos, list, cols ? colpos : nullptr,
                       cols ? full_off : nullptr, P.st);
    HITE_CHECK(ctx, hipMemcpyAsync(S->d_scal + slot, pos + nrows, 8, hipMemcpyDeviceToDevice, st));
    if (cols) HITE_CHECK(ctx, hipMemcpyAsync(S->d_scal + slot + 1, colpos + nrows, 8, hipMemcpyDeviceToDevice, st));
    HITE_CHECK(ctx, hipMemcpyAsync(S->h_pin + slot, S->d_scal + slot, 16, hipMemcpyDeviceToHost, st));
    HITE_CHECK(ctx, hipStreamSynchronize(st));
    *count = S->h_pin[slot];
    if (total_cols) *total_cols = cols ? S->h_pin[slot + 1] : 0;
    return HITE_OK;
}

static int assign_records(hite_ctx *ctx, AlignState *S, hipStream_t st, const int32_t *list, int64_t cnt, const int32_t *strips, int32_t *bk,
                          int64_t *boff, int64_t *scan_tmp, unsigned long long *rec, int slot, int words = 4, int64_t *n_long = nullptr, int64_t *n_long_tb = nullptr) {
    if (n_long) *n_long = 0;
    if (n_long_tb) *n_long_tb = 0;
    if (cnt <= 0) return HITE_OK;
    const int64_t nb = (cnt + 63) / 64;
    hipLaunchKernelGGL(align_blockmax_kernel, dim3((unsigned)((cnt + 255) / 256)), dim3(256), 0, st, cnt, list, strips, bk);
    ACHK(scan_excl_buf<int32_t>(ctx, scan_tmp, bk, nb, boff, st));
    HITE_CHECK(ctx, hipMemcpyAsync(S->d_scal + slot, boff + nb, 8, hipMemcpyDeviceToDevice, st));
    const bool lanes = n_long && S->lanes_min != -2;
    if (lanes) {
        LaneCost fwd4 = {5440.f, 3200.f, 4.3f, 12.5f}, fwd8 = {7040.f, 3200.f, 13.75f, 25.f}, tb = {6880.f, 530.f, 4.3f, 21.5f};
        fwd4.lane_work *= S->lanes_scale[0]; fwd8.lane_work *= S->lanes_scale[1]; tb.lane_work *= S->lanes_scale[2];
        fwd4.lane_chain *= S->lanes_scale[3]; fwd8.lane_chain *= S->lanes_scale[3];
        hipLaunchKernelGGL(align_long_blocks_kernel, dim3(1), dim3(1), 0, st, nb, bk, boff,
                           (int64_t)(S->lanes_min < 0 ? -1 : (S->lanes_min + AL_STRIP - 1) / AL_STRIP), words == 4 ? fwd4 : fwd8, tb, S->d_scal + slot + 1);
    }
    HITE_CHECK(ctx, hipMemcpyAsync(S->h_pin + slot, S->d_scal + slot, 24, hipMemcpyDeviceToHost, st));
    HITE_CHECK(ctx, hipStreamSynchronize(st));
    const int64_t block_strips = S->h_pin[slot];
    if (lanes) {
        const int64_t v = S->h_pin[slot + 1] * 64, vt = S->h_pin[slot + 2] * 64;
        *n_long = v < cnt ? v : cnt;
        if (n_long_tb) *n_long_tb = vt < cnt ? vt : cnt;
    }
    char *region;
    ACHK(aalloc(ctx, S->arena, (size_t)block_strips * AL_RECB + 256, &region));
    hipLaunchKernelGGL(align_assign_kernel, dim3((unsigned)((cnt + 255) / 256)), dim3(256), 0, st, cnt, list, boff, region, rec);
    return HITE_OK;
}

int hite_align_run(hite_ctx *ctx, int32_t n_cand, const uint8_t *d_win, const int64_t *d_win_off, const int32_t *d_win_len,
                   const int32_t *d_row_first, int64_t total_rows, const int64_t *d_ops_base, uint16_t *d_ops,
                   int32_t *d_row_dead, int32_t *d_cand_flag, int32_t *d_info, const char *tag, hipStream_t st) {
    if (!ctx || n_cand < 0 || total_rows < 0 || total_rows > 0x7fffffff) return HITE_EINVAL;
    if (n_cand == 0 || total_rows == 0) return HITE_OK;
    AlignState *S = align_state(ctx);
    if (!S) return HITE_ENOMEM;
    Arena &A = S->arena;
    ACHK(arena_reset(ctx, A, true));
    const int cap = S->exact_cap;
    AlignArgs P;
    memset(&P, 0, sizeof P);
    P.win = d_win; P.win_off = d_win_off; P.win_len = d_win_len; P.row_first = d_row_first; P.n_cand = n_cand;
    P.ops_base = d_ops_base; P.ops = d_ops;
    int32_t *row_cand, *strips, *order, *pwords, *flag, *flag2, *cols, *list, *list_esc, *list_fin;
    unsigned long long *skeys;
    int64_t *plane_off, *pos, *pos2, *colpos, *scan_tmp, *scan_tmp2, *full_off, *boff, *boff2;
    int32_t *bk, *bk2;
    unsigned long long *rec;
    ACHK(aalloc(ctx, A, (size_t)total_rows, &row_cand));
    ACHK(aalloc(ctx, A, (size_t)total_rows, &strips));
    ACHK(aalloc(ctx, A, (size_t)total_rows + 1, &skeys));
    ACHK(aalloc(ctx, A, (size_t)total_rows + 1, &order));
    Sorter srt;
    srt.ctx = ctx; srt.st = st; srt.cap = total_rows; srt.hist_n = sorter_hist_elems(total_rows);
    ACHK(aalloc(ctx, A, (size_t)total_rows + 1, &srt.k2));
    ACHK(aalloc(ctx, A, (size_t)total_rows + 1, &srt.v2));
    ACHK(aalloc(ctx, A, (size_t)srt.hist_n, &srt.hist));
    ACHK(aalloc(ctx, A, (size_t)srt.hist_n + 1, &srt.offs));
    ACHK(aalloc(ctx, A, (size_t)sorter_tmp_elems(srt.hist_n), &srt.bs));
    ACHK(aalloc(ctx, A, (size_t)n_cand, &pwords));
    ACHK(aalloc(ctx, A, (size_t)n_cand + 1, &plane_off));
    ACHK(aalloc(ctx, A, (size_t)total_rows, &rec));
    ACHK(aalloc(ctx, A, (size_t)total_rows / 64 + 2, &bk));
    ACHK(aalloc(ctx, A, (size_t)total_rows / 64 + 3, &boff));
    ACHK(aalloc(ctx, A, (size_t)total_rows / 64 + 2, &bk2));
    ACHK(aalloc(ctx, A, (size_t)total_rows / 64 + 3, &boff2));
    ACHK(aalloc(ctx, A, (size_t)total_rows, &flag));
    ACHK(aalloc(ctx, A, (size_t)total_rows, &cols));
    ACHK(aalloc(ctx, A, (size_t)total_rows, &list));
    ACHK(aalloc(ctx, A, (size_t)total_rows, &list_esc));
    ACHK(aalloc(ctx, A, (size_t)total_rows, &list_fin));
    ACHK(aalloc(ctx, A, (size_t)total_rows, &flag2));
    ACHK(aalloc(ctx, A, (size_t)total_rows + 1, &pos2));
    ACHK(aalloc(ctx, A, (size_t)scan_tmp_elems(total_rows) + 16, &scan_tmp2));
    ACHK(aalloc(ctx, A, (size_t)total_rows + 1, &pos));
    ACHK(aalloc(ctx, A, (size_t)total_rows + 1, &colpos));
    ACHK(aalloc(ctx, A, (size_t)total_rows, &full_off));
    ACHK(aalloc(ctx, A, (size_t)scan_tmp_elems(total_rows > n_cand ? total_rows : n_cand) + 16, &scan_tmp));
    ACHK(aalloc(ctx, A, (size_t)total_rows, &P.U));
    ACHK(aalloc(ctx, A, (size_t)total_rows, &P.kst));
    ACHK(aalloc(ctx, A, (size_t)total_rows, &P.st));
    ACHK(aalloc(ctx, A, (size_t)total_rows, &P.lvl));
    ACHK(aalloc(ctx, A, (size_t)total_rows, &P.U4));
    P.row_cand = row_cand; P.full_off = full_off;
    int tk = hite_prof_begin(ctx, "align_prep", st);
    HITE_CHECK(ctx, hipMemsetAsync(P.st, 0, (size_t)total_rows * 4, st));
    HITE_CHECK(ctx, hipMemsetAsync(P.lvl, 0, (size_t)total_rows * 4, st));
    hipLaunchKernelGGL(align_rows_kernel, dim3(n_cand), dim3(256), 0, st, n_cand, d_row_first, d_win_len, row_cand, strips, skeys, (unsigned *)order);
    if (!S->sort_attr) {
        HITE_CHECK(ctx, hipFuncSetAttribute(reinterpret_cast<const void *>(rs_scatter_staged_kernel<true>), hipFuncAttributeMaxDynamicSharedMemorySize, RSS_LDS_BYTES));
        S->sort_attr = true;
    }
    ACHK(sorter_sort(srt, skeys, (unsigned *)order, total_rows, 11));
    hipLaunchKernelGGL(align_plane_words_kernel, dim3((n_cand + 255) / 256), dim3(256), 0, st, n_cand, d_row_first, d_win_len, pwords);
    ACHK(scan_excl_buf<int32_t>(ctx, scan_tmp, pwords, n_cand, plane_off, st));
    HITE_CHECK(ctx, hipMemcpyAsync(S->d_scal, plane_off + n_cand, 8, hipMemcpyDeviceToDevice, st));
    HITE_CHECK(ctx, hipMemcpyAsync(S->h_pin, S->d_scal, 8, hipMemcpyDeviceToHost, st));
    int64_t nl4 = 0, nltb = 0;
    ACHK(assign_records(ctx, S, st, order, total_rows, strips, bk, boff, scan_tmp, rec, 1, 4, &nl4, &nltb));
    const int64_t plane_words = S->h_pin[0];
    uint4 *planes;
    ACHK(aalloc(ctx, A, (size_t)plane_words + 8, &planes));
    P.planes = planes; P.plane_off = plane_off; P.rec = rec;
    hipLaunchKernelGGL(align_planes_kernel, dim3(n_cand), dim3(256), 0, st, n_cand, d_win, d_win_off, d_win_len, d_row_first, plane_off, planes);
    hite_prof_end(ctx, tk, st);
    HITE_CHECK(ctx, hipGetLastError());
    char name[32];
    const int nrows = (int)total_rows;
    snprintf(name, sizeof name, "align_fwd4%s", tag ? tag : "");
    hipStream_t s2 = S->st2;
    char lname[40];
    if (getenv("HITE_ALIGN_DEBUG")) fprintf(stderr, "[align%s] rows %d  block-strips %lld  lane-parallel prefix %lld forward, %lld traceback\n", tag ? tag : "", nrows, (long long)S->h_pin[1], (long long)nl4, (long long)nltb);
    if (nl4 > 0) {
        HITE_CHECK(ctx, hipEventRecord(S->ev_fork, st));
        HITE_CHECK(ctx, hipStreamWaitEvent(s2, S->ev_fork, 0));
        snprintf(lname, sizeof lname, "align_fwd4_lanes%s", tag ? tag : "");
        const int tl = hite_prof_begin(ctx, lname, s2);
        hipLaunchKernelGGL(HIP_KERNEL_NAME(align_fwd_lanes_kernel<4>), dim3((unsigned)((nl4 + 15) / 16)), dim3(64), 0, s2, P, order, (int)nl4);
        hite_prof_end(ctx, tl, s2);
        HITE_CHECK(ctx, hipEventRecord(S->ev_join, s2));
    }
    if (nrows > nl4) {
        tk = hite_prof_begin(ctx, name, st);
        hipLaunchKernelGGL(align_fwd4_kernel, dim3((unsigned)((nrows - nl4 + 63) / 64)), dim3(64), 0, st, P, order + nl4, (int)(nrows - nl4));
        hite_prof_end(ctx, tk, st);
    }
    if (nl4 > 0) HITE_CHECK(ctx, hipStreamWaitEvent(st, S->ev_join, 0));
    snprintf(name, sizeof name, "align_tb%s", tag ? tag : "");
    char wname[32];
    snprintf(wname, sizeof wname, "align_fwd_wide%s", tag ? tag : "");
    int64_t n_esc = 0, n_fin = 0;
    const bool overlap = cap >= 16;
    if (cap >= 8 && !overlap) {
        tk = hite_prof_begin(ctx, wname, st);
        for (int level = 8; level <= cap; level *= 2) {
            int64_t cnt = 0;
            ACHK(build_list(ctx, S, st, total_rows, order, strips, P, 0, level, cap, flag, nullptr, pos, colpos, scan_tmp, list, nullptr, &cnt, nullptr));
            if (cnt == 0) continue;
            int64_t nl8 = 0;
            ACHK(assign_records(ctx, S, st, list, cnt, strips, bk, boff, scan_tmp, rec, 1, 8, &nl8));
            if (getenv("HITE_ALIGN_DEBUG")) fprintf(stderr, "[align%s] level %d: pairs %lld  block-strips %lld  lane-parallel prefix %lld\n", tag ? tag : "", level, (long long)cnt, (long long)S->h_pin[1], (long long)nl8);
            if (nl8 > 0) {
                HITE_CHECK(ctx, hipEventRecord(S->ev_fork, st));
                HITE_CHECK(ctx, hipStreamWaitEvent(s2, S->ev_fork, 0));
                snprintf(lname, sizeof lname, "align_fwd_wide_lanes%s", tag ? tag : "");
                const int tl = hite_prof_begin(ctx, lname, s2);
                hipLaunchKernelGGL(HIP_KERNEL_NAME(align_fwd_lanes_kernel<8>), dim3((unsigned)((nl8 + 7) / 8)), dim3(64), 0, s2, P, list, (int)nl8);
                hite_prof_end(ctx, tl, s2);
                HITE_CHECK(ctx, hipEventRecord(S->ev_join, s2));
            }
            if (cnt > nl8)
                hipLaunchKernelGGL(align_fwd8_pair_kernel, dim3((unsigned)((cnt - nl8 + 31) / 32)), dim3(64), 0, st, P, list + nl8, (int)(cnt - nl8));
            if (nl8 > 0) HITE_CHECK(ctx, hipStreamWaitEvent(st, S->ev_join, 0));
        }
        hite_prof_end(ctx, tk, st);
    }
    if (overlap) {
        ACHK(build_list(ctx, S, st, total_rows, order, strips, P, 2, 0, cap, flag, nullptr, pos, colpos, scan_tmp, list_esc, nullptr, &n_esc, nullptr));
        if (n_esc > 0)
            ACHK(build_list(ctx, S, st, total_rows, order, strips, P, 3, 0, cap, flag, nullptr, pos, colpos, scan_tmp, list_fin, nullptr, &n_fin, nullptr));
    }
    if (n_esc > 0) {
        if (n_fin > 0) {
            tk = hite_prof_begin(ctx, name, st);
            hipLaunchKernelGGL(align_tb_kernel, dim3((unsigned)((n_fin + 63) / 64)), dim3(64), 0, st, P, list_fin, (int)n_fin);
            hite_prof_end(ctx, tk, st);
        }
        tk = hite_prof_begin(ctx, wname, s2);
        for (int level = 8; level <= cap; level *= 2) {
            int64_t cnt = 0;
            ACHK(build_list(ctx, S, s2, total_rows, order, strips, P, 0, level, cap, flag2, nullptr, pos2, colpos, scan_tmp2, list, nullptr, &cnt, nullptr, 8));
            if (cnt == 0) continue;
            ACHK(assign_records(ctx, S, s2, list, cnt, strips, bk2, boff2, scan_tmp2, rec, 10));
            const dim3 grid((unsigned)((cnt + 63) / 64));
            if (level == 8) hipLaunchKernelGGL(HIP_KERNEL_NAME(align_fwd_kernel<8>), grid, dim3(64), 0, s2, P, list, (int)cnt);
            else if (level == 16) hipLaunchKernelGGL(HIP_KERNEL_NAME(align_fwd_kernel<16>), grid, dim3(64), 0, s2, P, list, (int)cnt);
            else hipLaunchKernelGGL(HIP_KERNEL_NAME(align_fwd_kernel<32>), grid, dim3(64), 0, s2, P, list, (int)cnt);
        }
        hite_prof_end(ctx, tk, s2);
        HITE_CHECK(ctx, hipEventRecord(S->ev, s2));
        HITE_CHECK(ctx, hipStreamWaitEvent(st, S->ev, 0));
        tk = hite_prof_begin(ctx, name, st);
        hipLaunchKernelGGL(align_tb_kernel, dim3((unsigned)((n_esc + 63) / 64)), dim3(64), 0, st, P, list_esc, (int)n_esc);
        hite_prof_end(ctx, tk, st);
    } else {
        if (nltb > 0) {
            HITE_CHECK(ctx, hipEventRecord(S->ev_fork, st));
            HITE_CHECK(ctx, hipStreamWaitEvent(s2, S->ev_fork, 0));
            snprintf(lname, sizeof lname, "align_tb_strips%s", tag ? tag : "");
            const int tl = hite_prof_begin(ctx, lname, s2);
            hipLaunchKernelGGL(align_tb_strips_kernel, dim3((unsigned)nltb), dim3(64), 0, s2, P, order, (int)nltb);
            hite_prof_end(ctx, tl, s2);
            HITE_CHECK(ctx, hipEventRecord(S->ev_join, s2));
        }
        if (nrows > nltb) {
            tk = hite_prof_begin(ctx, name, st);
            hipLaunchKernelGGL(align_tb_kernel, dim3((unsigned)((nrows - nltb + 63) / 64)), dim3(64), 0, st, P, order + nltb, (int)(nrows - nltb));
            hite_prof_end(ctx, tk, st);
        }
        if (nltb > 0) HITE_CHECK(ctx, hipStreamWaitEvent(st, S->ev_join, 0));
    }
    HITE_CHECK(ctx, hipGetLastError());
    {
        int64_t cnt = 0, tcols = 0;
        ACHK(build_list(ctx, S, st, total_rows, order, strips, P, 1, 0, cap, flag, cols, pos, colpos, scan_tmp, list, full_off, &cnt, &tcols));
        if (cnt > 0) {
            tk = hite_prof_begin(ctx, "align_fallback", st);
            ACHK(aalloc(ctx, A, (size_t)tcols * 2 * AL_WIDE_NW + 64, &P.fullbuf));
            ACHK(aalloc(ctx, A, (size_t)tcols + 16, &P.fullt));
            hipLaunchKernelGGL(align_wide_fwd_kernel, dim3((unsigned)cnt), dim3(64), 0, st, P, list, (int)cnt);
            hipLaunchKernelGGL(align_wide_tb_kernel, dim3((unsigned)cnt), dim3(64), 0, st, P, list, (int)cnt);
            hite_prof_end(ctx, tk, st);
        }
    }
    HITE_CHECK(ctx, hipMemsetAsync(S->d_scal, 0, 64, st));
    hipLaunchKernelGGL(align_stats_kernel, dim3((unsigned)(total_rows + 255 < 1024 * 256 ? (total_rows + 255) / 256 : 1024)), dim3(256), 0, st, total_rows, strips, P, d_row_dead, d_cand_flag,
                       (unsigned long long *)S->d_scal);
    if (d_info) hipLaunchKernelGGL(align_info_kernel, dim3((unsigned)((total_rows + 255) / 256)), dim3(256), 0, st, total_rows, P, d_info);
    HITE_CHECK(ctx, hipMemcpyAsync(S->h_pin, S->d_scal, 56, hipMemcpyDeviceToHost, st));
    HITE_CHECK(ctx, hipStreamSynchronize(st));
    for (int q = 0; q < 7; q++) S->stats[q] += S->h_pin[q];
    HITE_CHECK(ctx, hipGetLastError());
    return HITE_OK;
}
```

hite_amd/csrc/hite_pipeline.hip:

```cpp
#include "hite_common.h"
#include "hite_genome.h"
#include "hite_scan.h"
#include "hite_arena.h"
#include <vector>

extern "C" int hite_judge_dev(hite_ctx *ctx, int32_t te_type, int32_t plant, int32_t n, const uint8_t *d_msa,
                              const int64_t *d_msa_off, const int32_t *d_rows, const int32_t *d_cols,
                              const uint8_t *d_cand, const int64_t *d_cand_off, const int64_t *d_col_off,
                              int32_t max_cols, int32_t max_rows, hite_call *d_calls, uint8_t *d_cons, void *stream);

extern "C" int hite_judge_lds_enabled(int32_t n);
extern "C" int hite_judge_classify_dev(hite_ctx *ctx, int32_t n, const int32_t *d_rows, const int32_t *d_cols, uint8_t *d_cls, void *stream);

#define MAXROWS 100

struct PipeState {
    Arena keep, tmp;
    int64_t *h_pin = nullptr;
    int64_t *d_scal = nullptr;
};

extern "C" void hite_pipeline_release(void *state) {
    PipeState *s = (PipeState *)state;
    if (!s) return;
    arena_free(s->keep);
    arena_free(s->tmp);
    if (s->h_pin) (void)hipHostFree(s->h_pin);
    if (s->d_scal) (void)hipFree(s->d_scal);
    delete s;
}

template <typename TIn>
static int scan_excl(hite_ctx *ctx, Arena &tmp, const TIn *d_in, int64_t n, int64_t *d_out , hipStream_t st) {
    void *bs = nullptr;
    int rc = arena_alloc(ctx, tmp, (size_t)scan_tmp_elems(n) * 8, &bs);
    if (rc) return rc;
    return scan_excl_buf<TIn>(ctx, (int64_t *)bs, d_in, n, d_out, st);
}

__global__ void mode_a_kernel(int n, const int32_t *__restrict__ copy_first, const int64_t *__restrict__ len,
                              int32_t *__restrict__ mode) {
    int c = blockIdx.x * blockDim.x + threadIdx.x;
    if (c >= n) return;
    int any = 0, big = 0;
    for (int i = copy_first[c]; i < copy_first[c + 1]; i++) { any |= len[i] > 0; big |= len[i] > 1000; }
    mode[c] = big ? 2 : (any ? 1 : 0);
}
__global__ void mode_b_kernel(int n, const int32_t *__restrict__ mode_a, const hite_call *__restrict__ calls_a,
                              int32_t *__restrict__ mode) {
    int c = blockIdx.x * blockDim.x + threadIdx.x;
    if (c >= n) return;
    mode[c] = (mode_a[c] == 2 && calls_a[c].is_te) ? 1 : 0;
}

__device__ __forceinline__ int dec_digits(long long v) {
    int d = 1;
    while (v >= 10) { v /= 10; d++; }
    return d;
}
__device__ __forceinline__ long long pow10ll(int k) { long long r = 1; while (k-- > 0) r *= 10; return r; }
__device__ __forceinline__ int dec_str_cmp(long long a, long long b) {
    if (a == b) return 0;
    const int da = dec_digits(a), db = dec_digits(b);
    const int k = da < db ? da : db;
    const long long ta = a / pow10ll(da - k), tb = b / pow10ll(db - k);
    if (ta != tb) return ta < tb ? -1 : 1;
    return da < db ? -1 : 1;
}
__device__ __forceinline__ bool copy_name_gt(int r1, long long s1, long long e1, int m1, int r2, long long s2, long long e2, int m2) {
    if (r1 != r2) return r1 > r2;
    int c = dec_str_cmp(s1, s2);
    if (c) return c > 0;
    c = dec_str_cmp(e1, e2);
    if (c) return c > 0;
    return m1 > m2;
}

__global__ void __launch_bounds__(256) select_rows_kernel(int n, const int32_t *__restrict__ copy_first,
                                                          const int64_t *__restrict__ len,
                                                          const int32_t *__restrict__ mode, const int32_t *__restrict__ contig,
                                                          const int64_t *__restrict__ s1, const int64_t *__restrict__ e1,
                                                          const uint8_t *__restrict__ minus, const int32_t *__restrict__ contig_rank,
                                                          int32_t *__restrict__ nrows, int32_t *__restrict__ sel ) {
    __shared__ int s_scan[8];
    __shared__ int s_cnt;
    int c = blockIdx.x;
    if (c >= n) return;
    const int md = mode[c];
    const int f = copy_first[c], k = copy_first[c + 1] - f;
    if (md == 0 || k <= 0) { if (threadIdx.x == 0) nrows[c] = 0; return; }
    if (threadIdx.x == 0) s_cnt = 0;
    __syncthreads();
    int local = 0;
    for (int i = threadIdx.x; i < k; i += 256) { int64_t L = len[f + i]; local += md == 2 ? (L > 1000) : (L > 0); }
    atomicAdd(&s_cnt, local);
    __syncthreads();
    const int E = s_cnt;
    int running = 0;
    for (int base = 0; base < k; base += 256) {
        int i = base + threadIdx.x;
        int keep = 0;
        if (i < k) {
            int64_t L = len[f + i];
            bool el = md == 2 ? (L > 1000) : (L > 0);
            if (el) {
                if (E <= MAXROWS) keep = 1;
                else {
                    int64_t Li = md == 2 ? 1000 : L;
                    const int ri = contig_rank ? contig_rank[contig[f + i]] : contig[f + i];
                    const long long si = s1[f + i], ei = e1[f + i];
                    const int mi = minus[f + i] != 0;
                    int rank = 0;
                    for (int j = 0; j < k; j++) {
                        int64_t Lj = len[f + j];
                        bool ej = md == 2 ? (Lj > 1000) : (Lj > 0);
                        if (!ej) continue;
                        if (md == 2) Lj = 1000;
                        if (Lj > Li) rank++;
                        else if (Lj == Li && j != i) {
                            const int rj = contig_rank ? contig_rank[contig[f + j]] : contig[f + j];
                            const int mj = minus[f + j] != 0;
                            const bool gt = copy_name_gt(rj, s1[f + j], e1[f + j], mj, ri, si, ei, mi);
                            const bool same = rj == ri && s1[f + j] == si && e1[f + j] == ei && mj == mi;
                            rank += gt || (same && j < i);
                        }
                    }
                    keep = rank < MAXROWS;
                }
            }
        }
        int tot;
        int pre = block_excl_scan(keep, s_scan, &tot);
        if (keep) sel[(int64_t)c * MAXROWS + running + pre] = f + i;
        running += tot;
        __syncthreads();
    }
    if (threadIdx.x == 0) nrows[c] = running;
}

__device__ __forceinline__ void pad_lengths(const uint32_t *__restrict__ clip, const uint8_t *__restrict__ minus, int cp, int cp0, int &a, int &b) {
    a = 0; b = 0;
    if (!clip || cp == cp0) return;
    const uint32_t cl = clip[cp], c0 = clip[cp0];
    const bool mn = minus[cp] != 0, m0 = minus[cp0] != 0;
    const int ar = mn ? (int)(cl >> 16) : (int)(cl & 0xffffu), br = mn ? (int)(cl & 0xffffu) : (int)(cl >> 16);
    const int a0 = m0 ? (int)(c0 >> 16) : (int)(c0 & 0xffffu), b0 = m0 ? (int)(c0 & 0xffffu) : (int)(c0 >> 16);
    a = ar > a0 ? ar - a0 : 0;
    b = br > b0 ? br - b0 : 0;
}

__global__ void row_meta_kernel(int n, const int64_t *__restrict__ row_first, const int32_t *__restrict__ nrows,
                                const int32_t *__restrict__ sel, const int32_t *__restrict__ mode,
                                const int64_t *__restrict__ len, int32_t *__restrict__ row_first32,
                                int32_t *__restrict__ row_copy, int32_t *__restrict__ row_len,
                                int32_t *__restrict__ row_pad, uint8_t *__restrict__ row_trunc,
                                int32_t *__restrict__ maxlen, const uint32_t *__restrict__ clip ,
                                const uint8_t *__restrict__ minus,
                                int32_t *__restrict__ row_cp0 ) {
    int c = blockIdx.x;
    if (c >= n) return;
    if (threadIdx.x == 0) { row_first32[c] = (int32_t)row_first[c]; if (c == n - 1) row_first32[n] = (int32_t)row_first[n]; }
    int R = nrows[c];
    int md = mode[c];
    int mx = 0;
    for (int r = threadIdx.x; r < R; r += blockDim.x) {
        int64_t g = row_first[c] + r;
        int cp = sel[(int64_t)c * MAXROWS + r];
        int pa, pb;
        pad_lengths(clip, minus, cp, sel[(int64_t)c * MAXROWS], pa, pb);
        int L = md == 2 ? 1000 : (int)len[cp] + pa + pb;
        row_copy[g] = cp;
        if (clip) row_cp0[g] = sel[(int64_t)c * MAXROWS];
        row_len[g] = L;
        row_pad[g] = (L + 15) & ~15;
        row_trunc[g] = md == 2;
        mx = L > mx ? L : mx;
    }
#pragma unroll
    for (int d = 32; d >= 1; d >>= 1) { const int o = __shfl_xor(mx, d, 64); mx = o > mx ? o : mx; }
    if ((threadIdx.x & 63) == 0 && mx > 0 && mx > __atomic_load_n(maxlen, __ATOMIC_RELAXED)) atomicMax(maxlen, mx);
}

__device__ __forceinline__ unsigned window_byte(const uint32_t *__restrict__ bases, const uint32_t *__restrict__ nmask, int64_t g_lo, int64_t wlen,
                                                bool minus, int64_t p) {
    if (!minus) return fetch4(bases, nmask, g_lo + p) & 0xffu;
    const unsigned c = fetch4(bases, nmask, g_lo + wlen - 1 - p) & 0xffu;
    return c == 'A' ? 'T' : c == 'T' ? 'A' : c == 'C' ? 'G' : c == 'G' ? 'C' : 'N';
}
struct PadSrc { int64_t g_lo, len; bool minus; };
__device__ __forceinline__ void emit_padded(const uint32_t *__restrict__ bases, const uint32_t *__restrict__ nmask, int64_t g_lo, int64_t len,
                                            bool mn, int64_t a, int64_t b, int64_t ws, int64_t cnt, uint8_t *__restrict__ dst, int lane,
                                            const PadSrc &C) {
    int64_t n1 = a - ws; n1 = n1 < 0 ? 0 : (n1 > cnt ? cnt : n1);
    const int64_t off = ws + n1 - a;
    int64_t n2 = len - off; n2 = n2 < 0 ? 0 : (n2 > cnt - n1 ? cnt - n1 : n2);
    int64_t lead = n2 > 0 ? (int64_t)((0 - (uintptr_t)(dst + n1)) & 15) : 0;
    if (lead > n2) lead = n2;
    for (int64_t i = lane; i < n1 + lead; i += 64) {
        unsigned ch;
        if (i < n1) {
            const int64_t cpos = ws + i;
            ch = cpos < C.len ? (window_byte(bases, nmask, C.g_lo, C.len, C.minus, cpos) | 0x20u) : (unsigned)HITE_ROW_PAD;
        } else ch = window_byte(bases, nmask, g_lo, len, mn, off + (i - n1));
        dst[i] = (uint8_t)ch;
    }
    if (n2 > lead) emit_span(bases, nmask, g_lo, len, mn, off + lead, n2 - lead, dst + n1 + lead, lane);
    for (int64_t i = n1 + n2 + lane; i < cnt; i += 64) {
        const int64_t j = ws + i - a - len;
        const int64_t cpos = C.len - b + j;
        dst[i] = (cpos >= 0 && cpos < C.len) ? (uint8_t)(window_byte(bases, nmask, C.g_lo, C.len, C.minus, cpos) | 0x20u) : (uint8_t)HITE_ROW_PAD;
    }
}

__global__ void __launch_bounds__(256) row_gather_kernel(const uint32_t *__restrict__ bases,
                                                         const uint32_t *__restrict__ nmask,
                                                         const int64_t *__restrict__ coff, int32_t ncontig,
                                                         int64_t nrows_total, const int32_t *__restrict__ row_copy,
                                                         const uint8_t *__restrict__ row_trunc,
                                                         const int32_t *__restrict__ contig,
                                                         const int64_t *__restrict__ s1, const int64_t *__restrict__ e1,
                                                         const uint8_t *__restrict__ minus, int32_t flank,
                                                         const int64_t *__restrict__ win_off, uint8_t *__restrict__ win,
                                                         const uint32_t *__restrict__ clip, const int32_t *__restrict__ row_cp0) {
    int64_t g = (int64_t)blockIdx.x * 4 + (threadIdx.x >> 6);
    if (g >= nrows_total) return;
    int lane = threadIdx.x & 63;
    int cp = row_copy[g];
    int64_t len, tlen, g_lo;
    window_rule(coff, ncontig, contig[cp], s1[cp], e1[cp], flank, len, tlen, g_lo);
    if (len == 0) return;
    bool mn = minus[cp] != 0;
    uint8_t *dst = win + win_off[g];
    const int cp0 = clip ? row_cp0[g] : cp;
    int pa, pb;
    pad_lengths(clip, minus, cp, cp0, pa, pb);
    if (pa | pb) {
        const int64_t a = pa, b = pb;
        const int64_t plen = a + len + b;
        PadSrc C;
        int64_t tl0;
        window_rule(coff, ncontig, contig[cp0], s1[cp0], e1[cp0], flank, C.len, tl0, C.g_lo);
        C.minus = minus[cp0] != 0;
        if (row_trunc[g]) {
            emit_padded(bases, nmask, g_lo, len, mn, a, b, 0, 500, dst, lane, C);
            emit_padded(bases, nmask, g_lo, len, mn, a, b, plen - 500, 500, dst + 500, lane, C);
        } else {
            emit_padded(bases, nmask, g_lo, len, mn, a, b, 0, plen, dst, lane, C);
        }
        return;
    }
    if (row_trunc[g]) {
        emit_span(bases, nmask, g_lo, len, mn, 0, 500, dst, lane);
        emit_span(bases, nmask, g_lo, len, mn, len - 500, 500, dst + 500, lane);
    } else {
        emit_span(bases, nmask, g_lo, len, mn, 0, len, dst, lane);
    }
}

__global__ void ops_count_kernel(int n, const int64_t *__restrict__ row_first, const int32_t *__restrict__ nrows,
                                 const int32_t *__restrict__ row_len, int64_t *__restrict__ cnt,
                                 unsigned long long *__restrict__ acc) {
    int c = blockIdx.x * blockDim.x + threadIdx.x;
    unsigned long long bytes = 0, steps = 0;
    if (c < n) {
        int R = nrows[c];
        if (R <= 0) cnt[c] = 0;
        else {
            int64_t g0 = row_first[c];
            int64_t m = row_len[g0];
            cnt[c] = (int64_t)(R + 1) * (m + 1);
            for (int r = 1; r < R; r++) {
                int64_t nn = row_len[g0 + r];
                bytes += (unsigned long long)(m + nn + 2 * (m + 1));
                steps += (unsigned long long)(m + nn);
            }
        }
    }
#pragma unroll
    for (int d = 32; d >= 1; d >>= 1) {
        bytes += ((unsigned long long)(unsigned)__shfl_xor((int)(bytes >> 32), d, 64) << 32) | (unsigned)__shfl_xor((int)bytes, d, 64);
        steps += ((unsigned long long)(unsigned)__shfl_xor((int)(steps >> 32), d, 64) << 32) | (unsigned)__shfl_xor((int)steps, d, 64);
    }
    if ((threadIdx.x & 63) == 0 && bytes) { atomicAdd(&acc[0], bytes); atomicAdd(&acc[1], steps); }
}

__global__ void msa_size_kernel(int n, const int32_t *__restrict__ nrows, const int32_t *__restrict__ cols,
                                const uint8_t *__restrict__ cls, int64_t *__restrict__ bytes, int32_t *__restrict__ maxcols) {
    int c = blockIdx.x * blockDim.x + threadIdx.x;
    if (c >= n) return;
    int64_t b = (cls && cls[c] >= JUDGE_CLS_LDS) ? 0 : (int64_t)nrows[c] * cols[c];
    bytes[c] = (b + 15) & ~(int64_t)15;
    if (cols[c] > __atomic_load_n(maxcols, __ATOMIC_RELAXED)) atomicMax(maxcols, cols[c]);
}

__global__ void eff_rows_kernel(int n, const int32_t *__restrict__ nrows, const int32_t *__restrict__ cols,
                                int32_t *__restrict__ eff) {
    int c = blockIdx.x * blockDim.x + threadIdx.x;
    if (c >= n) return;
    eff[c] = cols[c] > 0 ? nrows[c] : 0;
}

extern "C" int hite_sparse_cols_dev(hite_ctx *ctx, int32_t n, const uint8_t *d_msa, const int64_t *d_msa_off,
                                    const int32_t *d_rows, const int32_t *d_cols, const int64_t *d_col_off,
                                    int64_t total_cols, uint8_t *d_out, int32_t *d_new_cols, void *stream);

__global__ void merge_calls_kernel(int n, const int32_t *__restrict__ mode_a, const hite_call *__restrict__ ca,
                                   const hite_call *__restrict__ cb, hite_call *__restrict__ out,
                                   int32_t *__restrict__ src_pass, int64_t *__restrict__ keep_len) {
    int c = blockIdx.x * blockDim.x + threadIdx.x;
    if (c >= n) return;
    hite_call r;
    r.is_te = 0; r.info = 0; r.row_num = 0; r.bstart = -1; r.bend = -1; r.cons_len = 0; r.cons_off = 0;
    int src = 0;
    if (mode_a[c] == 1) { r = ca[c]; src = 1; }
    else if (mode_a[c] == 2) {
        if (ca[c].is_te && cb) { r = cb[c]; src = 2; }
        else { r = ca[c]; src = 1; }
    }
    if (!r.is_te) r.cons_len = 0;
    out[c] = r;
    src_pass[c] = r.is_te ? src : 0;
    keep_len[c] = r.is_te ? r.cons_len : 0;
}
__global__ void __launch_bounds__(256) copy_cons_kernel(int n, hite_call *__restrict__ calls,
                                                        const int32_t *__restrict__ src_pass,
                                                        const uint8_t *__restrict__ cons_a,
                                                        const uint8_t *__restrict__ cons_b,
                                                        const int64_t *__restrict__ out_off, uint8_t *__restrict__ out,
                                                        int64_t out_cap) {
    int c = blockIdx.x;
    if (c >= n) return;
    int sp = src_pass[c];
    if (!sp) { if (threadIdx.x == 0) calls[c].cons_off = out_off[c]; return; }
    const uint8_t *src = (sp == 1 ? cons_a : cons_b) + calls[c].cons_off;
    int L = calls[c].cons_len;
    int64_t o = out_off[c];
    if (o + L <= out_cap) for (int i = threadIdx.x; i < L; i += 256) out[o + i] = src[i];
    __syncthreads();
    if (threadIdx.x == 0) calls[c].cons_off = o;
}

struct PassOut {
    hite_call *calls = nullptr;
    uint8_t *cons = nullptr;
};
struct StageTimes;

static int read_scalars(hite_ctx *ctx, PipeState *S, hipStream_t st, int count) {
    HITE_CHECK(ctx, hipMemcpyAsync(S->h_pin, S->d_scal, sizeof(int64_t) * count, hipMemcpyDeviceToHost, st));
    HITE_CHECK(ctx, hipStreamSynchronize(st));
    return HITE_OK;
}

#define ACHK(x) do { int rc__ = (x); if (rc__) return rc__; } while (0)

static int run_pass(hite_ctx *ctx, PipeState *S, int te_type, int plant, int n, const uint8_t *d_cand,
                    const int64_t *d_cand_off, const int32_t *d_copy_first, const int32_t *d_contig,
                    const int64_t *d_s1, const int64_t *d_e1, const uint8_t *d_minus, const uint32_t *d_clip, int flank, const int64_t *d_len,
                    const int32_t *d_mode, PassOut *out, int64_t *stats ,
                    int64_t *extra , int64_t *cols_acc , bool pass_b, hipStream_t st) {
    Arena &T = S->tmp, &K = S->keep;
    int32_t *nrows, *sel, *row_first32, *row_copy, *row_len, *row_pad, *cols, *status, *eff, *new_cols;
    int64_t *row_first, *win_off, *ops_cnt, *ops_base, *msa_bytes, *msa_off, *col_off2;
    uint8_t *row_trunc, *win, *clean;
    void *p;
    ACHK(arena_alloc(ctx, T, (size_t)n * 4, &p)); nrows = (int32_t *)p;
    ACHK(arena_alloc(ctx, T, (size_t)n * MAXROWS * 4, &p)); sel = (int32_t *)p;
    int tk = hite_prof_begin(ctx, "select_rows_kernel", st);
    hipLaunchKernelGGL(select_rows_kernel, dim3(n), dim3(256), 0, st, n, d_copy_first, d_len, d_mode, d_contig, d_s1, d_e1, d_minus,
                       (const int32_t *)ctx->d_contig_rank, nrows, sel);
    hite_prof_end(ctx, tk, st);
    ACHK(arena_alloc(ctx, T, (size_t)(n + 1) * 8, &p)); row_first = (int64_t *)p;
    ACHK(scan_excl<int32_t>(ctx, T, nrows, n, row_first, st));
    HITE_CHECK(ctx, hipMemcpyAsync(S->d_scal, row_first + n, 8, hipMemcpyDeviceToDevice, st));
    ACHK(read_scalars(ctx, S, st, 1));
    const int64_t total_rows = S->h_pin[0];
    stats[0] += total_rows;
    ACHK(arena_alloc(ctx, K, sizeof(hite_call) * (size_t)n, &p)); out->calls = (hite_call *)p;
    HITE_CHECK(ctx, hipMemsetAsync(out->calls, 0, sizeof(hite_call) * (size_t)n, st));
    if (total_rows == 0) { ACHK(arena_alloc(ctx, K, 256, &p)); out->cons = (uint8_t *)p; return HITE_OK; }
    if (total_rows > 0x7fffffff) return HITE_EINVAL;

    ACHK(arena_alloc(ctx, T, (size_t)(n + 1) * 4, &p)); row_first32 = (int32_t *)p;
    ACHK(arena_alloc(ctx, T, (size_t)total_rows * 4, &p)); row_copy = (int32_t *)p;
    ACHK(arena_alloc(ctx, T, (size_t)total_rows * 4, &p)); row_len = (int32_t *)p;
    ACHK(arena_alloc(ctx, T, (size_t)total_rows * 4, &p)); row_pad = (int32_t *)p;
    ACHK(arena_alloc(ctx, T, (size_t)total_rows, &p)); row_trunc = (uint8_t *)p;
    int32_t *row_cp0 = nullptr;
    if (d_clip) { ACHK(arena_alloc(ctx, T, (size_t)total_rows * 4, &p)); row_cp0 = (int32_t *)p; }
    HITE_CHECK(ctx, hipMemsetAsync(S->d_scal, 0, 64, st));
    hipLaunchKernelGGL(row_meta_kernel, dim3(n), dim3(128), 0, st, n, row_first, nrows, sel, d_mode, d_len, row_first32,
                       row_copy, row_len, row_pad, row_trunc, (int32_t *)(S->d_scal + 2), d_clip, d_minus, row_cp0);
    ACHK(arena_alloc(ctx, T, (size_t)(total_rows + 1) * 8, &p)); win_off = (int64_t *)p;
    ACHK(scan_excl<int32_t>(ctx, T, row_pad, total_rows, win_off, st));
    ACHK(arena_alloc(ctx, T, (size_t)n * 8, &p)); ops_cnt = (int64_t *)p;
    ACHK(arena_alloc(ctx, T, (size_t)(n + 1) * 8, &p)); ops_base = (int64_t *)p;
    hipLaunchKernelGGL(ops_count_kernel, dim3((n + 255) / 256), dim3(256), 0, st, n, row_first, nrows, row_len, ops_cnt,
                       (unsigned long long *)(S->d_scal + 4));
    ACHK(scan_excl<int64_t>(ctx, T, ops_cnt, n, ops_base, st));
    HITE_CHECK(ctx, hipMemcpyAsync(S->d_scal, win_off + total_rows, 8, hipMemcpyDeviceToDevice, st));
    HITE_CHECK(ctx, hipMemcpyAsync(S->d_scal + 1, ops_base + n, 8, hipMemcpyDeviceToDevice, st));
    ACHK(read_scalars(ctx, S, st, 6));
    const int64_t win_bytes = S->h_pin[0], ops_elems = S->h_pin[1];
    const int max_len = (int)(((int32_t *)(S->h_pin + 2))[0]);
    stats[1] += win_bytes;
    stats[3] += S->h_pin[4];
    extra[0] += S->h_pin[5];

    ACHK(arena_alloc(ctx, T, (size_t)win_bytes + 64, &p)); win = (uint8_t *)p;
    tk = hite_prof_begin(ctx, "row_gather_kernel", st);
    hipLaunchKernelGGL(row_gather_kernel, dim3((unsigned)((total_rows + 3) / 4)), dim3(256), 0, st, ctx->d_bases, ctx->d_nmask,
                       ctx->d_contig_off, ctx->n_contigs, total_rows, row_copy, row_trunc, d_contig, d_s1, d_e1, d_minus,
                       flank, win_off, win, d_clip, row_cp0);
    hite_prof_end(ctx, tk, st);
    HITE_CHECK(ctx, hipGetLastError());

    ACHK(arena_alloc(ctx, T, (size_t)n * 4, &p)); cols = (int32_t *)p;
    ACHK(arena_alloc(ctx, T, (size_t)n * 4, &p)); status = (int32_t *)p;
    ACHK(arena_alloc(ctx, T, (size_t)n * 4, &p)); new_cols = (int32_t *)p;
    int32_t *last_extra;
    ACHK(arena_alloc(ctx, T, (size_t)n * 4, &p)); last_extra = (int32_t *)p;
    int32_t *rows_al;
    ACHK(arena_alloc(ctx, T, (size_t)n * 4, &p)); rows_al = (int32_t *)p;
    ACHK(hite_star_msa_sparse_dev(ctx, n, win, win_off, row_len, row_first32, total_rows, ops_base, ops_elems, max_len > 0 ? max_len : 1,
                                  cols, status, new_cols, last_extra, rows_al, st));
    ACHK(arena_alloc(ctx, T, (size_t)n * 4, &p)); eff = (int32_t *)p;
    hipLaunchKernelGGL(eff_rows_kernel, dim3((n + 255) / 256), dim3(256), 0, st, n, rows_al, cols, eff);
    ACHK(arena_alloc(ctx, T, (size_t)n * 8, &p)); msa_bytes = (int64_t *)p;
    ACHK(arena_alloc(ctx, T, (size_t)(n + 1) * 8, &p)); msa_off = (int64_t *)p;
    ACHK(arena_alloc(ctx, T, (size_t)(n + 1) * 8, &p)); col_off2 = (int64_t *)p;
    HITE_CHECK(ctx, hipMemsetAsync(S->d_scal, 0, 64, st));
    uint8_t *jcls = nullptr;
    {
        const char *e = getenv("HITE_JUDGE_FUSE");
        if (!(e && *e && atoi(e) == 0) && hite_judge_lds_enabled(n)) {
            ACHK(arena_alloc(ctx, T, (size_t)n + 16, &p)); jcls = (uint8_t *)p;
            ACHK(hite_judge_classify_dev(ctx, n, eff, new_cols, jcls, st));
        }
    }
    hipLaunchKernelGGL(msa_size_kernel, dim3((n + 255) / 256), dim3(256), 0, st, n, eff, new_cols, jcls, msa_bytes, (int32_t *)(S->d_scal + 2));
    ACHK(scan_excl<int64_t>(ctx, T, msa_bytes, n, msa_off, st));
    ACHK(scan_excl<int32_t>(ctx, T, new_cols, n, col_off2, st));
    HITE_CHECK(ctx, hipMemcpyAsync(S->d_scal, col_off2 + n, 8, hipMemcpyDeviceToDevice, st));
    HITE_CHECK(ctx, hipMemcpyAsync(S->d_scal + 1, msa_off + n, 8, hipMemcpyDeviceToDevice, st));
    ACHK(read_scalars(ctx, S, st, 3));
    const int64_t msa_total = S->h_pin[1];
    stats[2] += msa_total;
    ACHK(arena_alloc(ctx, T, (size_t)msa_total + 64, &p)); clean = (uint8_t *)p;
    tk = hite_prof_begin(ctx, extra == nullptr ? "star_fill_sparse_kernel" : (pass_b ? "star_fill_sparse_kernel_passB" : "star_fill_sparse_kernel_passA"), st);
    struct FuseGuard {
        hite_ctx *c;
        ~FuseGuard() { c->d_judge_cls = nullptr; c->judge_fuse = JudgeFuse{}; }
    } fuse_guard{ctx};
    if (jcls) {
        JudgeFuse F;
        F.win = win; F.win_off = ctx->d_msa_win_off ? ctx->d_msa_win_off : win_off; F.win_len = ctx->d_msa_win_len ? ctx->d_msa_win_len : row_len;
        F.row_first = row_first32; F.ops_base = ops_base;
        F.ops = (const uint16_t *)ctx->d_scratch2; F.lay = ctx->d_msa_lay; F.last_extra = last_extra;
        F.row_map = ctx->d_msa_row_map; F.rows_eff = ctx->d_msa_rows_eff;
        ctx->judge_fuse = F; ctx->d_judge_cls = jcls;
    }
    ACHK(hite_star_msa_fill_sparse_dev(ctx, n, win, win_off, row_len, row_first32, ops_base, new_cols, last_extra, msa_off, clean, st));
    hite_prof_end(ctx, tk, st);
    const int64_t total_cols2 = S->h_pin[0];
    if (cols_acc) *cols_acc += total_cols2;
    const int max_cols2 = (int)(((int32_t *)(S->h_pin + 2))[0]);
    ACHK(arena_alloc(ctx, K, (size_t)total_cols2 + 8 * (size_t)n + 64, &p)); out->cons = (uint8_t *)p;
    tk = hite_prof_begin(ctx, extra == nullptr ? "judge_kernel" : (pass_b ? "judge_kernel_passB" : "judge_kernel_passA"), st);
    if (max_cols2 > 0)
        ACHK(hite_judge_dev(ctx, te_type, plant, n, clean, msa_off, eff, new_cols, d_cand, d_cand_off, col_off2, max_cols2,
                            MAXROWS + 1, out->calls, out->cons, st));
    hite_prof_end(ctx, tk, st);
    return HITE_OK;
}

#define CLIP_K 21
#define CLIP_MM 5
__device__ __forceinline__ unsigned long long probe_code(unsigned ch, unsigned long long nval) {
    const unsigned c = ch & 0xdfu;
    return (c == 'A' || c == 'C' || c == 'G' || c == 'T') ? (unsigned long long)((c >> 1) & 3u) : nval;
}
__global__ void __launch_bounds__(256) clip_probe_kernel(const uint32_t *__restrict__ bases, const uint32_t *__restrict__ nmask,
                                                         const int64_t *__restrict__ coff, int32_t ncontig, int64_t n_copies, int32_t n_cand,
                                                         const int32_t *__restrict__ copy_first, const uint8_t *__restrict__ cand,
                                                         const int64_t *__restrict__ cand_off, const int32_t *__restrict__ contig,
                                                         const int64_t *__restrict__ s1, const int64_t *__restrict__ e1,
                                                         const uint8_t *__restrict__ minus, uint16_t *__restrict__ clip_out ) {
    const int64_t tid = (int64_t)blockIdx.x * blockDim.x + threadIdx.x;
    if (tid >= 2 * n_copies) return;
    const int64_t cp = tid >> 1;
    const int right = (int)(tid & 1);
    int lo = 0, hi = n_cand;
    while (hi - lo > 1) { const int mid = (lo + hi) >> 1; if ((int64_t)copy_first[mid] <= cp) lo = mid; else hi = mid; }
    const uint8_t *q = cand + cand_off[lo];
    const int64_t Lq = cand_off[lo + 1] - cand_off[lo];
    const int ct = contig[cp];
    int64_t ys = s1[cp] - 1, ye = e1[cp];
    int clip = -1;
    int64_t dmax = 0, Ly = 0;
    bool mn = false;
    if (ct >= 0 && ct < ncontig) {
        const int64_t clen = coff[ct + 1] - coff[ct];
        if (ys < 0) ys = 0;
        if (ye > clen) ye = clen;
        Ly = ye - ys;
        const int64_t g_lo = coff[ct] + ys;
        mn = minus[cp] != 0;
        if (Ly >= CLIP_K && Lq >= CLIP_K) {
            dmax = Lq / 20 + 32;
            if (dmax > Lq - CLIP_K) dmax = Lq - CLIP_K;
            if (dmax > 0xffff) dmax = 0xffff;
            const unsigned long long M3 = 0x1249249249249249ull, M63 = 0x7fffffffffffffffull;
            for (int att = 0; att < 2 && clip < 0; att++) {
                const int64_t sh = (int64_t)att * CLIP_K;
                if (Ly < sh + CLIP_K) break;
                int64_t dm = dmax;
                if (dm > Lq - CLIP_K - sh) dm = Lq - CLIP_K - sh;
                if (dm < 0) break;
                unsigned long long Y = 0, Q = 0;
                for (int i = 0; i < CLIP_K; i++) {
                    const int64_t yp = right ? Ly - sh - CLIP_K + i : sh + i;
                    Y |= probe_code(window_byte(bases, nmask, g_lo, Ly, mn, yp), 4ull) << (3 * i);
                    const int64_t qp = right ? Lq - sh - CLIP_K + i : sh + i;
                    Q |= probe_code(q[qp], 7ull) << (3 * i);
                }
                int best = CLIP_K + 1, arg = 0;
                for (int64_t d = 0; d <= dm; d++) {
                    if (d > 0) {
                        if (!right) Q = (Q >> 3) | (probe_code(q[d + sh + CLIP_K - 1], 7ull) << (3 * (CLIP_K - 1)));
                        else Q = ((Q << 3) & M63) | probe_code(q[Lq - d - sh - CLIP_K], 7ull);
                    }
                    const unsigned long long x = Q ^ Y;
                    const int mm = __popcll((x | (x >> 1) | (x >> 2)) & M3);
                    if (mm < best) { best = mm; arg = (int)d; }
                }
                if (best <= CLIP_MM) clip = arg;
            }
        }
    }
    const int other = __shfl_xor(clip, 1, 64);
    if (clip < 0) {
        int64_t v = other >= 0 ? (Lq - Ly) - other : 0;
        clip = (int)(v < 0 ? 0 : (v > dmax ? dmax : v));
    }
    clip_out[2 * cp + ((right != 0) != mn ? 1 : 0)] = (uint16_t)clip;
}

extern "C" int hite_flank_region_align_clip_dev(hite_ctx *ctx, void **state_io, int32_t te_type, int32_t plant, int32_t n_cand,
                                                const uint8_t *d_cand, const int64_t *d_cand_off, const int32_t *d_copy_first,
                                                int64_t n_copies, const int32_t *d_contig, const int64_t *d_start1,
                                                const int64_t *d_end1, const uint8_t *d_minus, const uint32_t *d_clip ,
                                                int32_t flank, hite_call *d_calls, uint8_t *d_cons, int64_t cons_cap,
                                                int64_t *stats_out , void *stream) {
    if (!ctx || !ctx->d_bases || !state_io || n_cand < 0 || n_copies < 0 || te_type < 0 || te_type > 2) return HITE_EINVAL;
    if (n_cand == 0) return HITE_OK;
    hipStream_t st = (hipStream_t)stream;
    HITE_CHECK(ctx, hipSetDevice(ctx->device));
    PipeState *S = (PipeState *)*state_io;
    if (!S) {
        S = new PipeState();
        HITE_CHECK(ctx, hipHostMalloc((void **)&S->h_pin, 64 * sizeof(int64_t)));
        HITE_CHECK(ctx, hipMalloc((void **)&S->d_scal, 64 * sizeof(int64_t)));
        *state_io = S;
    }
    ACHK(arena_reset(ctx, S->keep, true));
    ACHK(arena_reset(ctx, S->tmp, true));
    int64_t stats[12] = {0, 0, 0, 0, 0, 0, 0, 0, 0, 0, 0, 0};
    void *p;
    int64_t *len;
    int32_t *mode_a, *mode_b, *src_pass;
    int64_t *keep_len, *out_off;
    ACHK(arena_alloc(ctx, S->keep, (size_t)(n_copies + 1) * 8, &p)); len = (int64_t *)p;
    ACHK(arena_alloc(ctx, S->keep, (size_t)n_cand * 4, &p)); mode_a = (int32_t *)p;
    ACHK(arena_alloc(ctx, S->keep, (size_t)n_cand * 4, &p)); mode_b = (int32_t *)p;
    ACHK(arena_alloc(ctx, S->keep, (size_t)n_cand * 4, &p)); src_pass = (int32_t *)p;
    ACHK(arena_alloc(ctx, S->keep, (size_t)n_cand * 8, &p)); keep_len = (int64_t *)p;
    ACHK(arena_alloc(ctx, S->keep, (size_t)(n_cand + 1) * 8, &p)); out_off = (int64_t *)p;
    if (n_copies > 0)
        hipLaunchKernelGGL(flank_sizes_kernel, dim3((unsigned)((n_copies + 255) / 256)), dim3(256), 0, st, ctx->d_contig_off,
                           ctx->n_contigs, n_copies, d_contig, d_start1, d_end1, flank, len, (int64_t *)nullptr);
    if (!d_clip && n_copies > 0) {
        uint16_t *est;
        ACHK(arena_alloc(ctx, S->keep, (size_t)n_copies * 4 + 16, &p)); est = (uint16_t *)p;
        const int tkp = hite_prof_begin(ctx, "clip_probe_kernel", st);
        hipLaunchKernelGGL(clip_probe_kernel, dim3((unsigned)((2 * n_copies + 255) / 256)), dim3(256), 0, st, ctx->d_bases, ctx->d_nmask,
                           ctx->d_contig_off, ctx->n_contigs, n_copies, n_cand, d_copy_first, d_cand, d_cand_off, d_contig, d_start1, d_end1,
                           d_minus, est);
        hite_prof_end(ctx, tkp, st);
        d_clip = reinterpret_cast<const uint32_t *>(est);
    }
    hipLaunchKernelGGL(mode_a_kernel, dim3((n_cand + 255) / 256), dim3(256), 0, st, n_cand, d_copy_first, len, mode_a);
    HITE_CHECK(ctx, hipGetLastError());
    PassOut A, B;
    ACHK(run_pass(ctx, S, te_type, plant, n_cand, d_cand, d_cand_off, d_copy_first, d_contig, d_start1, d_end1, d_minus, d_clip, flank,
                  len, mode_a, &A, stats, stats + 8, stats + 11, false, st));
    ACHK(arena_reset(ctx, S->tmp, false));
    hipLaunchKernelGGL(mode_b_kernel, dim3((n_cand + 255) / 256), dim3(256), 0, st, n_cand, mode_a, A.calls, mode_b);
    ACHK(run_pass(ctx, S, te_type, plant, n_cand, d_cand, d_cand_off, d_copy_first, d_contig, d_start1, d_end1, d_minus, d_clip, flank,
                  len, mode_b, &B, stats + 4, stats + 9, stats + 11, true, st));
    hipLaunchKernelGGL(merge_calls_kernel, dim3((n_cand + 255) / 256), dim3(256), 0, st, n_cand, mode_a, A.calls, B.calls, d_calls,
                       src_pass, keep_len);
    ACHK(scan_excl<int64_t>(ctx, S->tmp, keep_len, n_cand, out_off, st));
    hipLaunchKernelGGL(copy_cons_kernel, dim3(n_cand), dim3(256), 0, st, n_cand, d_calls, src_pass, A.cons, B.cons, out_off, d_cons,
                       cons_cap);
    HITE_CHECK(ctx, hipGetLastError());
    HITE_CHECK(ctx, hipMemcpyAsync(S->d_scal, out_off + n_cand, 8, hipMemcpyDeviceToDevice, st));
    ACHK(read_scalars(ctx, S, st, 1));
    if (stats_out) { memcpy(stats_out, stats, sizeof stats); stats_out[10] = S->h_pin[0]; }
    const int64_t cons_need = S->h_pin[0];
    ACHK(arena_reset(ctx, S->keep, true));
    ACHK(arena_reset(ctx, S->tmp, true));
    if (cons_need > cons_cap) return HITE_ECAP;
    return HITE_OK;
}

extern "C" int hite_clip_probe(hite_ctx *ctx, int32_t n_cand, const uint8_t *cand, const int64_t *cand_off, const int32_t *copy_first,
                               int64_t n_copies, const int32_t *contig, const int64_t *start1, const int64_t *end1, const uint8_t *minus,
                               uint32_t *clip_out) {
    if (!ctx || !ctx->d_bases || n_cand < 0 || n_copies < 0 || (n_copies > 0 && (!cand || !cand_off || !copy_first || !contig || !start1 || !end1 || !minus || !clip_out)))
        return HITE_EINVAL;
    if (n_copies == 0 || n_cand == 0) return HITE_OK;
    HITE_CHECK(ctx, hipSetDevice(ctx->device));
    uint8_t *d = nullptr;
    const size_t cb = (size_t)cand_off[n_cand], o1 = (cb + 64 + 255) & ~(size_t)255, o2 = o1 + (((size_t)(n_cand + 1) * 8 + 255) & ~(size_t)255),
                 o3 = o2 + (((size_t)(n_cand + 1) * 4 + 255) & ~(size_t)255), o4 = o3 + (((size_t)n_copies * 4 + 255) & ~(size_t)255),
                 o5 = o4 + (((size_t)n_copies * 8 + 255) & ~(size_t)255), o6 = o5 + (((size_t)n_copies * 8 + 255) & ~(size_t)255),
                 o7 = o6 + (((size_t)n_copies + 255) & ~(size_t)255), total = o7 + (size_t)n_copies * 4 + 256;
    HITE_CHECK(ctx, hipMalloc((void **)&d, total));
    hipError_t e = hipMemcpy(d, cand, cb, hipMemcpyHostToDevice);
    if (e == hipSuccess) e = hipMemcpy(d + o1, cand_off, (size_t)(n_cand + 1) * 8, hipMemcpyHostToDevice);
    if (e == hipSuccess) e = hipMemcpy(d + o2, copy_first, (size_t)(n_cand + 1) * 4, hipMemcpyHostToDevice);
    if (e == hipSuccess) e = hipMemcpy(d + o3, contig, (size_t)n_copies * 4, hipMemcpyHostToDevice);
    if (e == hipSuccess) e = hipMemcpy(d + o4, start1, (size_t)n_copies * 8, hipMemcpyHostToDevice);
    if (e == hipSuccess) e = hipMemcpy(d + o5, end1, (size_t)n_copies * 8, hipMemcpyHostToDevice);
    if (e == hipSuccess) e = hipMemcpy(d + o6, minus, (size_t)n_copies, hipMemcpyHostToDevice);
    if (e == hipSuccess) {
        hipLaunchKernelGGL(clip_probe_kernel, dim3((unsigned)((2 * n_copies + 255) / 256)), dim3(256), 0, 0, ctx->d_bases, ctx->d_nmask,
                           ctx->d_contig_off, ctx->n_contigs, n_copies, n_cand, (const int32_t *)(d + o2), d, (const int64_t *)(d + o1),
                           (const int32_t *)(d + o3), (const int64_t *)(d + o4), (const int64_t *)(d + o5), d + o6, (uint16_t *)(d + o7));
        e = hipGetLastError();
    }
    if (e == hipSuccess) e = hipMemcpy(clip_out, d + o7, (size_t)n_copies * 4, hipMemcpyDeviceToHost);
    (void)hipFree(d);
    HITE_CHECK(ctx, e);
    return HITE_OK;
}

extern "C" int hite_flank_region_align_dev(hite_ctx *ctx, void **state_io, int32_t te_type, int32_t plant, int32_t n_cand,
                                           const uint8_t *d_cand, const int64_t *d_cand_off, const int32_t *d_copy_first,
                                           int64_t n_copies, const int32_t *d_contig, const int64_t *d_start1,
                                           const int64_t *d_end1, const uint8_t *d_minus, int32_t flank, hite_call *d_calls,
                                           uint8_t *d_cons, int64_t cons_cap, int64_t *stats_out, void *stream) {
    return hite_flank_region_align_clip_dev(ctx, state_io, te_type, plant, n_cand, d_cand, d_cand_off, d_copy_first, n_copies, d_contig,
                                            d_start1, d_end1, d_minus, nullptr, flank, d_calls, d_cons, cons_cap, stats_out, stream);
}

struct PBuf {
    void *p = nullptr;
    ~PBuf() { if (p) (void)hipFree(p); }
    hipError_t alloc(size_t n) { return hipMalloc(&p, n ? n : 16); }
    hipError_t up(const void *h, size_t n) {
        hipError_t e = alloc(n + 16);
        if (e != hipSuccess) return e;
        return n ? hipMemcpy(p, h, n, hipMemcpyHostToDevice) : hipSuccess;
    }
};
__global__ void fold_bytes_kernel(uint8_t *__restrict__ p, int64_t n) {
    for (int64_t i = (int64_t)blockIdx.x * blockDim.x + threadIdx.x; i < n; i += (int64_t)gridDim.x * blockDim.x) p[i] = fold_sym(p[i]);
}

extern "C" int hite_flank_region_align_clip(hite_ctx *ctx, int32_t te_type, int32_t plant, int32_t n_cand, const uint8_t *cand,
                                            const int64_t *cand_off, const int32_t *copy_first, int64_t n_copies,
                                            const int32_t *contig, const int64_t *start1, const int64_t *end1,
                                            const uint8_t *minus, const uint32_t *clip , int32_t flank,
                                            hite_call *calls, uint8_t *cons, int64_t cons_cap, int64_t *stats_out) {
    if (!ctx || n_cand < 0 || !cand || !cand_off || !copy_first || !calls || !cons) return HITE_EINVAL;
    if (n_cand == 0) return HITE_OK;
    HITE_CHECK(ctx, hipSetDevice(ctx->device));
    PBuf dc, dco, dcf, dct, ds, de, dm, dcl, dcalls, dcons;
    hipError_t e;
    e = dc.up(cand, cand_off[n_cand]); if (e == hipSuccess) e = dco.up(cand_off, (n_cand + 1) * 8);
    if (e == hipSuccess) e = dcf.up(copy_first, (n_cand + 1) * 4); if (e == hipSuccess) e = dct.up(contig, n_copies * 4);
    if (e == hipSuccess) e = ds.up(start1, n_copies * 8); if (e == hipSuccess) e = de.up(end1, n_copies * 8);
    if (e == hipSuccess) e = dm.up(minus, n_copies); if (e == hipSuccess) e = dcalls.alloc(sizeof(hite_call) * n_cand);
    if (e == hipSuccess) e = dcons.alloc(cons_cap + 16);
    if (e == hipSuccess && clip) e = dcl.up(clip, n_copies * 4);
    HITE_CHECK(ctx, e);
    hipLaunchKernelGGL(fold_bytes_kernel, dim3(256), dim3(256), 0, nullptr, (uint8_t *)dc.p, cand_off[n_cand]);
    void *state = nullptr;
    int rc = hite_flank_region_align_clip_dev(ctx, &state, te_type, plant, n_cand, (uint8_t *)dc.p, (int64_t *)dco.p, (int32_t *)dcf.p,
                                              n_copies, (int32_t *)dct.p, (int64_t *)ds.p, (int64_t *)de.p, (uint8_t *)dm.p,
                                              clip ? (const uint32_t *)dcl.p : nullptr, flank, (hite_call *)dcalls.p, (uint8_t *)dcons.p,
                                              cons_cap, stats_out, nullptr);
    hipError_t es = hipDeviceSynchronize();
    if (rc == HITE_OK || rc == HITE_ECAP) {
        if (es == hipSuccess) es = hipMemcpy(calls, dcalls.p, sizeof(hite_call) * n_cand, hipMemcpyDeviceToHost);
        if (es == hipSuccess && rc == HITE_OK) es = hipMemcpy(cons, dcons.p, cons_cap, hipMemcpyDeviceToHost);
    }
    hite_pipeline_release(state);
    if (es != hipSuccess) return HITE_EHIP;
    return rc;
}

extern "C" int hite_flank_region_align(hite_ctx *ctx, int32_t te_type, int32_t plant, int32_t n_cand, const uint8_t *cand,
                                       const int64_t *cand_off, const int32_t *copy_first, int64_t n_copies,
                                       const int32_t *contig, const int64_t *start1, const int64_t *end1,
                                       const uint8_t *minus, int32_t flank, hite_call *calls, uint8_t *cons, int64_t cons_cap,
                                       int64_t *stats_out) {
    return hite_flank_region_align_clip(ctx, te_type, plant, n_cand, cand, cand_off, copy_first, n_copies, contig, start1, end1, minus,
                                        nullptr, flank, calls, cons, cons_cap, stats_out);
}
```

hite_amd/csrc/hite_scan.h:

```cpp
#pragma once
#include "hite_common.h"

#define SCAN_TILE 4096
template <typename TIn>
static __global__ void __launch_bounds__(256) scan_sums_kernel(const TIn *__restrict__ in, int64_t n, int64_t *__restrict__ bsum) {
    __shared__ long long s_w[4];
    int64_t base = (int64_t)blockIdx.x * SCAN_TILE;
    long long acc = 0;
    for (int i = threadIdx.x; i < SCAN_TILE; i += 256) {
        int64_t k = base + i;
        if (k < n) acc += (long long)in[k];
    }
    for (int d = 32; d >= 1; d >>= 1) acc += __shfl_down(acc, d, 64);
    if ((threadIdx.x & 63) == 0) s_w[threadIdx.x >> 6] = acc;
    __syncthreads();
    if (threadIdx.x == 0) bsum[blockIdx.x] = s_w[0] + s_w[1] + s_w[2] + s_w[3];
}
static __global__ void __launch_bounds__(1024) scan_bsums_kernel(int64_t *__restrict__ bsum, int64_t nb, int64_t *__restrict__ total) {
    __shared__ long long s_w[16];
    const int lane = threadIdx.x & 63, w = threadIdx.x >> 6;
    long long carry = 0;
    for (int64_t base = 0; base < nb; base += 1024) {
        const int64_t k = base + threadIdx.x;
        const long long v = k < nb ? bsum[k] : 0;
        long long x = v;
        for (int d = 1; d < 64; d <<= 1) { long long y = __shfl_up(x, d, 64); if (lane >= d) x += y; }
        __syncthreads();
        if (lane == 63) s_w[w] = x;
        __syncthreads();
        long long pre = 0, tot = 0;
        for (int q = 0; q < 16; q++) { const long long t = s_w[q]; if (q < w) pre += t; tot += t; }
        if (k < nb) bsum[k] = carry + pre + x - v;
        carry += tot;
    }
    if (threadIdx.x == 0) *total = carry;
}
template <typename TIn>
static __global__ void __launch_bounds__(256) scan_apply_kernel(const TIn *__restrict__ in, int64_t n, const int64_t *__restrict__ bsum,
                                                         int64_t *__restrict__ out) {
    __shared__ long long s_w[4];
    int64_t base = (int64_t)blockIdx.x * SCAN_TILE;
    long long running = bsum[blockIdx.x];
    for (int i0 = 0; i0 < SCAN_TILE; i0 += 256) {
        int64_t k = base + i0 + threadIdx.x;
        long long v = k < n ? (long long)in[k] : 0;
        long long x = v;
        int lane = threadIdx.x & 63, w = threadIdx.x >> 6;
        for (int d = 1; d < 64; d <<= 1) { long long y = __shfl_up(x, d, 64); if (lane >= d) x += y; }
        __syncthreads();
        if (lane == 63) s_w[w] = x;
        __syncthreads();
        long long pre = 0, tot = 0;
        for (int q = 0; q < 4; q++) { if (q < w) pre += s_w[q]; tot += s_w[q]; }
        if (k < n) out[k] = running + pre + x - v;
        running += tot;
    }
}
static inline int64_t scan_tmp_elems(int64_t n) { int64_t nb = (n + SCAN_TILE - 1) / SCAN_TILE; return nb < 1 ? 1 : nb; }
template <typename TIn>
static int scan_excl_buf(hite_ctx *ctx, int64_t *d_bs, const TIn *d_in, int64_t n, int64_t *d_out , hipStream_t st) {
    int64_t nb = scan_tmp_elems(n);
    hipLaunchKernelGGL(HIP_KERNEL_NAME(scan_sums_kernel<TIn>), dim3((unsigned)nb), dim3(256), 0, st, d_in, n, d_bs);
    hipLaunchKernelGGL(scan_bsums_kernel, dim3(1), dim3(1024), 0, st, d_bs, nb, d_out + n);
    hipLaunchKernelGGL(HIP_KERNEL_NAME(scan_apply_kernel<TIn>), dim3((unsigned)nb), dim3(256), 0, st, d_in, n, d_bs, d_out);
    HITE_CHECK(ctx, hipGetLastError());
    return HITE_OK;
}
```

Baseline: 658,200 candidates/s.

## Fuse list build scans, write scan totals to pinned host, add early fallback group

The flag, scan and compact kernels behind list building are merged into a sums kernel, a two-segment block-sum scan and a compact kernel that scans flags and column counts together. Scan totals are written straight into pinned host memory, which removes the device-to-device and device-to-host scalar copies around each synchronisation. The wide align kernels also raise their wave priority with s_setprio, and a new early-fallback group count is computed in the long-blocks kernel, along with a debug reporting helper. The host-mapped writes assume the pinned buffer is coherently visible after stream sync, and the early group changes how work is scheduled.

```diff
diff --git a/hite_amd/csrc/hite_align.hip b/hite_amd/csrc/hite_align.hip
--- a/hite_amd/csrc/hite_align.hip
+++ b/hite_amd/csrc/hite_align.hip
@@ -13,6 +13,7 @@
 #define AL_RECB 4096
 #define AL_DEFAULT_CAP 8
 #define AL_KBINS 2048
+#define AL_EARLY_FREE_BLOCKS 16
 #define AL_LANES_MIN_STRIPS 32
 
 struct AlignArgs {
@@ -1016,6 +1017,7 @@
 }
 __global__ void __launch_bounds__(64) align_wide_fwd_kernel(AlignArgs P, const int32_t *__restrict__ list, int nlist) {
     constexpr int NW = AL_WIDE_NW, W = 32 * NW, H = W / 2;
+    __builtin_amdgcn_s_setprio(3);
     const int pi = blockIdx.x;
     if (pi >= nlist) return;
     const int lane = threadIdx.x;
@@ -1092,6 +1094,7 @@
 };
 __global__ void __launch_bounds__(64) align_wide_tb_kernel(AlignArgs P, const int32_t *__restrict__ list, int nlist) {
     constexpr int NW = AL_WIDE_NW, W = 32 * NW, PF = 8;
+    __builtin_amdgcn_s_setprio(3);
     const int pi = blockIdx.x;
     if (pi >= nlist) return;
     const int lane = threadIdx.x;
@@ -1276,11 +1279,7 @@
     else out.run(i - 1, i, 0x8000u);
 }
 
-__global__ void align_flag_kernel(int64_t nrows, const int32_t *__restrict__ order, const int32_t *__restrict__ strips, AlignArgs P,
-                                  int what, int level, int cap, int32_t *__restrict__ flag, int32_t *__restrict__ cols) {
-    const int64_t x = (int64_t)blockIdx.x * blockDim.x + threadIdx.x;
-    if (x >= nrows) return;
-    const int g = order[x];
+__device__ __forceinline__ int align_flag_of(const AlignArgs &P, const int32_t *__restrict__ strips, int g, int what, int level, int cap) {
     int f = 0;
     if (strips[g] > 0) {
         if (what == 0) {
@@ -1298,18 +1297,59 @@
             f = what == 2 ? esc : !esc;
         }
     }
-    flag[x] = f;
-    if (cols) cols[x] = f ? P.win_len[g] + 1 : 0;
-}
-__global__ void align_compact_kernel(int64_t nrows, const int32_t *__restrict__ order, const int32_t *__restrict__ flag,
-                                     const int64_t *__restrict__ pos, int32_t *__restrict__ out, const int64_t *__restrict__ colpos,
-                                     int64_t *__restrict__ full_off, int32_t *__restrict__ st) {
-    const int64_t x = (int64_t)blockIdx.x * blockDim.x + threadIdx.x;
-    if (x >= nrows) return;
-    if (flag[x]) {
-        const int g = order[x];
-        out[pos[x]] = g;
-        if (full_off) { full_off[g] = colpos[x]; st[g] = 0; }
+    return f;
+}
+__global__ void __launch_bounds__(256) align_list_sums_kernel(int64_t nrows, const int32_t *__restrict__ order, const int32_t *__restrict__ strips,
+                                                              AlignArgs P, int what, int level, int cap, int32_t *__restrict__ flag,
+                                                              int32_t *__restrict__ cols, int64_t *__restrict__ bsum) {
+    __shared__ long long s_w[2][4];
+    const int64_t base = (int64_t)blockIdx.x * SCAN_TILE;
+    long long af = 0, ac = 0;
+    for (int i = threadIdx.x; i < SCAN_TILE; i += 256) {
+        const int64_t x = base + i;
+        if (x < nrows) {
+            const int g = order[x];
+            const int f = align_flag_of(P, strips, g, what, level, cap);
+            flag[x] = f;
+            af += f;
+            if (cols) { const int c = f ? P.win_len[g] + 1 : 0; cols[x] = c; ac += c; }
+        }
+    }
+    for (int d = 32; d >= 1; d >>= 1) { af += __shfl_down(af, d, 64); ac += __shfl_down(ac, d, 64); }
+    if ((threadIdx.x & 63) == 0) { s_w[0][threadIdx.x >> 6] = af; s_w[1][threadIdx.x >> 6] = ac; }
+    __syncthreads();
+    if (threadIdx.x == 0) {
+        bsum[blockIdx.x] = s_w[0][0] + s_w[0][1] + s_w[0][2] + s_w[0][3];
+        if (cols) bsum[gridDim.x + blockIdx.x] = s_w[1][0] + s_w[1][1] + s_w[1][2] + s_w[1][3];
+    }
+}
+__global__ void __launch_bounds__(256) align_list_compact_kernel(int64_t nrows, const int32_t *__restrict__ order, const int32_t *__restrict__ flag,
+                                                                 const int32_t *__restrict__ cols, const int64_t *__restrict__ bsum,
+                                                                 int32_t *__restrict__ out, int64_t *__restrict__ full_off, int32_t *__restrict__ st) {
+    __shared__ long long s_w[2][4];
+    const int64_t base = (int64_t)blockIdx.x * SCAN_TILE;
+    const int lane = threadIdx.x & 63, w = threadIdx.x >> 6;
+    long long runf = bsum[blockIdx.x], runc = cols ? bsum[gridDim.x + blockIdx.x] : 0;
+    for (int i0 = 0; i0 < SCAN_TILE; i0 += 256) {
+        const int64_t x = base + i0 + threadIdx.x;
+        const int f = x < nrows ? flag[x] : 0;
+        const long long c = cols && x < nrows ? (long long)cols[x] : 0;
+        long long xf = f, xc = c;
+        for (int d = 1; d < 64; d <<= 1) {
+            const long long yf = __shfl_up(xf, d, 64), yc = __shfl_up(xc, d, 64);
+            if (lane >= d) { xf += yf; xc += yc; }
+        }
+        __syncthreads();
+        if (lane == 63) { s_w[0][w] = xf; s_w[1][w] = xc; }
+        __syncthreads();
+        long long pf = 0, tf = 0, pc = 0, tc = 0;
+        for (int q = 0; q < 4; q++) { if (q < w) { pf += s_w[0][q]; pc += s_w[1][q]; } tf += s_w[0][q]; tc += s_w[1][q]; }
+        if (f) {
+            const int g = order[x];
+            out[runf + pf + xf - f] = g;
+            if (cols) { full_off[g] = runc + pc + xc - c; st[g] = 0; }
+        }
+        runf += tf; runc += tc;
     }
 }
 __global__ void __launch_bounds__(256) align_blockmax_kernel(int64_t cnt, const int32_t *__restrict__ list, const int32_t *__restrict__ strips,
@@ -1350,6 +1390,17 @@
         }
         out[w] = lo;
     }
+    {
+        const int64_t half = ((int64_t)bk[0] + 1) >> 1;
+        int64_t lo = 0, hi = nb;
+        while (lo < hi) { const int64_t mid = (lo + hi) >> 1; if ((int64_t)bk[mid] >= half) lo = mid + 1; else hi = mid; }
+        int64_t k = lo, wl = 0, wh = nb;
+        while (wl < wh) { const int64_t mid = (wl + wh + 1) >> 1; if (100 * boff[mid] <= boff[nb]) wl = mid; else wh = mid - 1; }
+        const int64_t kmax = wl > AL_EARLY_FREE_BLOCKS ? wl : AL_EARLY_FREE_BLOCKS;
+        if (k > kmax) k = kmax;
+        if (bk[0] < AL_LANES_MIN_STRIPS) k = 0;
+        out[2] = k;
+    }
 }
 __global__ void __launch_bounds__(256) align_stats_kernel(int64_t total_rows, const int32_t *__restrict__ strips, AlignArgs P, int32_t *__restrict__ row_dead,
                                                           int32_t *__restrict__ cand_status, unsigned long long *__restrict__ acc) {
@@ -1400,10 +1451,12 @@
     info[g * 5 + 4] = P.lvl[g];
 }
 
+enum { AL_PIN_PLANES = 0, AL_PIN_LIST = 1, AL_PIN_REC = 3, AL_PIN2_LIST = 8, AL_PIN2_REC = 10, AL_PIN_STATS = 16 };
 struct AlignState {
     Arena arena;
     int64_t *h_pin = nullptr;
     int64_t *d_scal = nullptr;
+    bool fallback_early = true;
     int exact_cap = -1;
     int lanes_min = -1;
     float lanes_scale[4] = {1.f, 1.f, 1.f, 1.f};
@@ -1435,6 +1488,8 @@
         const char *l = getenv("HITE_ALIGN_LANES");
         if (l && *l) { const int v = atoi(l); S->lanes_min = v < -2 ? -1 : v; }
         const char *sc = getenv("HITE_ALIGN_LANES_SCALE");
+        const char *fe = getenv("HITE_ALIGN_FALLBACK_EARLY");
+        if (fe && *fe) S->fallback_early = atoi(fe) != 0;
         if (sc && *sc) sscanf(sc, "%f,%f,%f,%f", &S->lanes_scale[0], &S->lanes_scale[1], &S->lanes_scale[2], &S->lanes_scale[3]);
         ctx->align_state = S;
     }
@@ -1489,51 +1544,80 @@
 }
 
 static int build_list(hite_ctx *ctx, AlignState *S, hipStream_t st, int64_t nrows, const int32_t *order, const int32_t *strips,
-                      AlignArgs &P, int what, int level, int cap, int32_t *flag, int32_t *cols, int64_t *pos, int64_t *colpos,
-                      int64_t *scan_tmp, int32_t *list, int64_t *full_off, int64_t *count, int64_t *total_cols, int slot = 0) {
-    const unsigned nb = (unsigned)((nrows + 255) / 256);
-    hipLaunchKernelGGL(align_flag_kernel, dim3(nb), dim3(256), 0, st, nrows, order, strips, P, what, level, cap, flag, cols);
-    ACHK(scan_excl_buf<int32_t>(ctx, scan_tmp, flag, nrows, pos, st));
-    if (cols) ACHK(scan_excl_buf<int32_t>(ctx, scan_tmp, cols, nrows, colpos, st));
-    hipLaunchKernelGGL(align_compact_kernel, dim3(nb), dim3(256), 0, st, nrows, order, flag, pos, list, cols ? colpos : nullptr,
+                      AlignArgs &P, int what, int level, int cap, int32_t *flag, int32_t *cols, int64_t *scan_tmp, int32_t *list,
+                      int64_t *full_off, int64_t *count, int64_t *total_cols, int pin = AL_PIN_LIST) {
+    *count = 0;
+    if (total_cols) *total_cols = 0;
+    if (nrows <= 0) return HITE_OK;
+    const int64_t nt = scan_tmp_elems(nrows);
+    hipLaunchKernelGGL(align_list_sums_kernel, dim3((unsigned)nt), dim3(256), 0, st, nrows, order, strips, P, what, level, cap, flag, cols, scan_tmp);
+    hipLaunchKernelGGL(scan_bsums_kernel, dim3(cols ? 2 : 1), dim3(1024), 0, st, scan_tmp, nt, (int64_t *)nullptr, S->h_pin + pin);
+    hipLaunchKernelGGL(align_list_compact_kernel, dim3((unsigned)nt), dim3(256), 0, st, nrows, order, flag, cols, scan_tmp, list,
                        cols ? full_off : nullptr, P.st);
-    HITE_CHECK(ctx, hipMemcpyAsync(S->d_scal + slot, pos + nrows, 8, hipMemcpyDeviceToDevice, st));
-    if (cols) HITE_CHECK(ctx, hipMemcpyAsync(S->d_scal + slot + 1, colpos + nrows, 8, hipMemcpyDeviceToDevice, st));
-    HITE_CHECK(ctx, hipMemcpyAsync(S->h_pin + slot, S->d_scal + slot, 16, hipMemcpyDeviceToHost, st));
     HITE_CHECK(ctx, hipStreamSynchronize(st));
-    *count = S->h_pin[slot];
-    if (total_cols) *total_cols = cols ? S->h_pin[slot + 1] : 0;
+    *count = S->h_pin[pin];
+    if (total_cols && cols) *total_cols = S->h_pin[pin + 1];
     return HITE_OK;
 }
 
 static int assign_records(hite_ctx *ctx, AlignState *S, hipStream_t st, const int32_t *list, int64_t cnt, const int32_t *strips, int32_t *bk,
-                          int64_t *boff, int64_t *scan_tmp, unsigned long long *rec, int slot, int words = 4, int64_t *n_long = nullptr, int64_t *n_long_tb = nullptr) {
+                          int64_t *boff, int64_t *scan_tmp, unsigned long long *rec, int pin, int words = 4, int64_t *n_long = nullptr,
+                          int64_t *n_long_tb = nullptr, int64_t *n_early = nullptr) {
     if (n_long) *n_long = 0;
     if (n_long_tb) *n_long_tb = 0;
+    if (n_early) *n_early = 0;
     if (cnt <= 0) return HITE_OK;
     const int64_t nb = (cnt + 63) / 64;
     hipLaunchKernelGGL(align_blockmax_kernel, dim3((unsigned)((cnt + 255) / 256)), dim3(256), 0, st, cnt, list, strips, bk);
-    ACHK(scan_excl_buf<int32_t>(ctx, scan_tmp, bk, nb, boff, st));
-    HITE_CHECK(ctx, hipMemcpyAsync(S->d_scal + slot, boff + nb, 8, hipMemcpyDeviceToDevice, st));
-    const bool lanes = n_long && S->lanes_min != -2;
-    if (lanes) {
+    ACHK(scan_excl_buf<int32_t>(ctx, scan_tmp, bk, nb, boff, st, S->h_pin + pin));
+    const bool lanes = n_long && S->lanes_min != -2, early = n_early && S->fallback_early;
+    if (lanes || early) {
         LaneCost fwd4 = {5440.f, 3200.f, 4.3f, 12.5f}, fwd8 = {7040.f, 3200.f, 13.75f, 25.f}, tb = {6880.f, 530.f, 4.3f, 21.5f};
         fwd4.lane_work *= S->lanes_scale[0]; fwd8.lane_work *= S->lanes_scale[1]; tb.lane_work *= S->lanes_scale[2];
         fwd4.lane_chain *= S->lanes_scale[3]; fwd8.lane_chain *= S->lanes_scale[3];
-        hipLaunchKernelGGL(align_long_blocks_kernel, dim3(1), dim3(1), 0, st, nb, bk, boff,
-                           (int64_t)(S->lanes_min < 0 ? -1 : (S->lanes_min + AL_STRIP - 1) / AL_STRIP), words == 4 ? fwd4 : fwd8, tb, S->d_scal + slot + 1);
-    }
-    HITE_CHECK(ctx, hipMemcpyAsync(S->h_pin + slot, S->d_scal + slot, 24, hipMemcpyDeviceToHost, st));
+        const int64_t fixed = !lanes ? (int64_t)1 << 40 : (S->lanes_min < 0 ? -1 : (S->lanes_min + AL_STRIP - 1) / AL_STRIP);
+        hipLaunchKernelGGL(align_long_blocks_kernel, dim3(1), dim3(1), 0, st, nb, bk, boff, fixed, words == 4 ? fwd4 : fwd8, tb, S->h_pin + pin + 1);
+    }
     HITE_CHECK(ctx, hipStreamSynchronize(st));
-    const int64_t block_strips = S->h_pin[slot];
+    const int64_t block_strips = S->h_pin[pin];
     if (lanes) {
-        const int64_t v = S->h_pin[slot + 1] * 64, vt = S->h_pin[slot + 2] * 64;
+        const int64_t v = S->h_pin[pin + 1] * 64, vt = S->h_pin[pin + 2] * 64;
         *n_long = v < cnt ? v : cnt;
         if (n_long_tb) *n_long_tb = vt < cnt ? vt : cnt;
+    }
+    if (early) {
+        const int64_t v = S->h_pin[pin + 3] * 64;
+        *n_early = v < cnt ? v : cnt;
     }
     char *region;
     ACHK(aalloc(ctx, S->arena, (size_t)block_strips * AL_RECB + 256, &region));
     hipLaunchKernelGGL(align_assign_kernel, dim3((unsigned)((cnt + 255) / 256)), dim3(256), 0, st, cnt, list, boff, region, rec);
+    return HITE_OK;
+}
+
+static int align_debug_fallback(hite_ctx *ctx, const char *tag, int64_t total_rows, const int32_t *d_strips, const int32_t *d_lvl,
+                                int64_t n_early, int64_t cnt_early, int64_t cnt_rest) {
+    std::vector<int32_t> strips((size_t)total_rows), lvl((size_t)total_rows);
+    HITE_CHECK(ctx, hipMemcpy(strips.data(), d_strips, (size_t)total_rows * 4, hipMemcpyDeviceToHost));
+    HITE_CHECK(ctx, hipMemcpy(lvl.data(), d_lvl, (size_t)total_rows * 4, hipMemcpyDeviceToHost));
+    int smax = 0;
+    for (int64_t g = 0; g < total_rows; g++) smax = strips[g] > smax ? strips[g] : smax;
+    fprintf(stderr, "[align%s] fall-back: early group %lld pairs, %lld of them fell back, %lld of the others; longest pair %d strips\n", tag ? tag : "",
+            (long long)n_early, (long long)cnt_early, (long long)cnt_rest, smax);
+    for (int div = 2; div <= 16; div *= 2) {
+        const int thr = div == 16 ? 1 : (smax + div - 1) / div;
+        long long pairs = 0, fb = 0;
+        int fb_long_in = 0, fb_long_out = 0;
+        for (int64_t g = 0; g < total_rows; g++) {
+            if (strips[g] <= 0) continue;
+            const bool f = (lvl[g] & 0x100) != 0, in = strips[g] >= thr;
+            pairs += in; fb += in && f;
+            if (f && in && strips[g] > fb_long_in) fb_long_in = strips[g];
+            if (f && !in && strips[g] > fb_long_out) fb_long_out = strips[g];
+        }
+        fprintf(stderr, "[align%s]   pairs of >= %d strips: %lld, fell back %lld (longest %d strips); longest fall-back below: %d strips\n", tag ? tag : "", thr, pairs,
+                fb, fb_long_in, fb_long_out);
+    }
     return HITE_OK;
 }
 
@@ -1551,9 +1635,9 @@
     memset(&P, 0, sizeof P);
     P.win = d_win; P.win_off = d_win_off; P.win_len = d_win_len; P.row_first = d_row_first; P.n_cand = n_cand;
     P.ops_base = d_ops_base; P.ops = d_ops;
-    int32_t *row_cand, *strips, *order, *pwords, *flag, *flag2, *cols, *list, *list_esc, *list_fin;
+    int32_t *row_cand, *strips, *order, *pwords, *flag, *flag2, *cols, *cols2, *list, *list_esc, *list_fin;
     unsigned long long *skeys;
-    int64_t *plane_off, *pos, *pos2, *colpos, *scan_tmp, *scan_tmp2, *full_off, *boff, *boff2;
+    int64_t *plane_off, *scan_tmp, *scan_tmp2, *full_off, *boff, *boff2;
     int32_t *bk, *bk2;
     unsigned long long *rec;
     ACHK(aalloc(ctx, A, (size_t)total_rows, &row_cand));
@@ -1580,12 +1664,10 @@
     ACHK(aalloc(ctx, A, (size_t)total_rows, &list_esc));
     ACHK(aalloc(ctx, A, (size_t)total_rows, &list_fin));
     ACHK(aalloc(ctx, A, (size_t)total_rows, &flag2));
-    ACHK(aalloc(ctx, A, (size_t)total_rows + 1, &pos2));
-    ACHK(aalloc(ctx, A, (size_t)scan_tmp_elems(total_rows) + 16, &scan_tmp2));
-    ACHK(aalloc(ctx, A, (size_t)total_rows + 1, &pos));
-    ACHK(aalloc(ctx, A, (size_t)total_rows + 1, &colpos));
+    ACHK(aalloc(ctx, A, (size_t)total_rows, &cols2));
+    ACHK(aalloc(ctx, A, (size_t)2 * scan_tmp_elems(total_rows) + 16, &scan_tmp2));
     ACHK(aalloc(ctx, A, (size_t)total_rows, &full_off));
-    ACHK(aalloc(ctx, A, (size_t)scan_tmp_elems(total_rows > n_cand ? total_rows : n_cand) + 16, &scan_tmp));
+    ACHK(aalloc(ctx, A, (size_t)2 * scan_tmp_elems(total_rows > n_cand ? total_rows : n_cand) + 16, &scan_tmp));
     ACHK(aalloc(ctx, A, (size_t)total_rows, &P.U));
     ACHK(aalloc(ctx, A, (size_t)total_rows, &P.kst));
     ACHK(aalloc(ctx, A, (size_t)total_rows, &P.st));
@@ -1602,12 +1684,10 @@
     }
     ACHK(sorter_sort(srt, skeys, (unsigned *)order, total_rows, 11));
     hipLaunchKernelGGL(align_plane_words_kernel, dim3((n_cand + 255) / 256), dim3(256), 0, st, n_cand, d_row_first, d_win_len, pwords);
-    ACHK(scan_excl_buf<int32_t>(ctx, scan_tmp, pwords, n_cand, plane_off, st));
-    HITE_CHECK(ctx, hipMemcpyAsync(S->d_scal, plane_off + n_cand, 8, hipMemcpyDeviceToDevice, st));
-    HITE_CHECK(ctx, hipMemcpyAsync(S->h_pin, S->d_scal, 8, hipMemcpyDeviceToHost, st));
-    int64_t nl4 = 0, nltb = 0;
-    ACHK(assign_records(ctx, S, st, order, total_rows, strips, bk, boff, scan_tmp, rec, 1, 4, &nl4, &nltb));
-    const int64_t plane_words = S->h_pin[0];
+    ACHK(scan_excl_buf<int32_t>(ctx, scan_tmp, pwords, n_cand, plane_off, st, S->h_pin + AL_PIN_PLANES));
+    int64_t nl4 = 0, nltb = 0, n_early = 0;
+    ACHK(assign_records(ctx, S, st, order, total_rows, strips, bk, boff, scan_tmp, rec, AL_PIN_REC, 4, &nl4, &nltb, &n_early));
+    const int64_t plane_words = S->h_pin[AL_PIN_PLANES];
     uint4 *planes;
     ACHK(aalloc(ctx, A, (size_t)plane_words + 8, &planes));
     P.planes = planes; P.plane_off = plane_off; P.rec = rec;
@@ -1619,7 +1699,7 @@
     snprintf(name, sizeof name, "align_fwd4%s", tag ? tag : "");
     hipStream_t s2 = S->st2;
     char lname[40];
-    if (getenv("HITE_ALIGN_DEBUG")) fprintf(stderr, "[align%s] rows %d  block-strips %lld  lane-parallel prefix %lld forward, %lld traceback\n", tag ? tag : "", nrows, (long long)S->h_pin[1], (long long)nl4, (long long)nltb);
+    if (getenv("HITE_ALIGN_DEBUG")) fprintf(stderr, "[align%s] rows %d  block-strips %lld  lane-parallel prefix %lld forward, %lld traceback\n", tag ? tag : "", nrows, (long long)S->h_pin[AL_PIN_REC], (long long)nl4, (long long)nltb);
     if (nl4 > 0) {
         HITE_CHECK(ctx, hipEventRecord(S->ev_fork, st));
         HITE_CHECK(ctx, hipStreamWaitEvent(s2, S->ev_fork, 0));
@@ -1639,16 +1719,17 @@
     char wname[32];
     snprintf(wname, sizeof wname, "align_fwd_wide%s", tag ? tag : "");
     int64_t n_esc = 0, n_fin = 0;
+    int64_t ne = 0, cnt_early = 0, tcols_early = 0;
     const bool overlap = cap >= 16;
     if (cap >= 8 && !overlap) {
         tk = hite_prof_begin(ctx, wname, st);
         for (int level = 8; level <= cap; level *= 2) {
             int64_t cnt = 0;
-            ACHK(build_list(ctx, S, st, total_rows, order, strips, P, 0, level, cap, flag, nullptr, pos, colpos, scan_tmp, list, nullptr, &cnt, nullptr));
+            ACHK(build_list(ctx, S, st, total_rows, order, strips, P, 0, level, cap, flag, nullptr, scan_tmp, list, nullptr, &cnt, nullptr));
             if (cnt == 0) continue;
             int64_t nl8 = 0;
-            ACHK(assign_records(ctx, S, st, list, cnt, strips, bk, boff, scan_tmp, rec, 1, 8, &nl8));
-            if (getenv("HITE_ALIGN_DEBUG")) fprintf(stderr, "[align%s] level %d: pairs %lld  block-strips %lld  lane-parallel prefix %lld\n", tag ? tag : "", level, (long long)cnt, (long long)S->h_pin[1], (long long)nl8);
+            ACHK(assign_records(ctx, S, st, list, cnt, strips, bk, boff, scan_tmp, rec, AL_PIN_REC, 8, &nl8));
+            if (getenv("HITE_ALIGN_DEBUG")) fprintf(stderr, "[align%s] level %d: pairs %lld  block-strips %lld  lane-parallel prefix %lld\n", tag ? tag : "", level, (long long)cnt, (long long)S->h_pin[AL_PIN_REC], (long long)nl8);
             if (nl8 > 0) {
                 HITE_CHECK(ctx, hipEventRecord(S->ev_fork, st));
                 HITE_CHECK(ctx, hipStreamWaitEvent(s2, S->ev_fork, 0));
@@ -1665,9 +1746,9 @@
         hite_prof_end(ctx, tk, st);
     }
     if (overlap) {
-        ACHK(build_list(ctx, S, st, total_rows, order, strips, P, 2, 0, cap, flag, nullptr, pos, colpos, scan_tmp, list_esc, nullptr, &n_esc, nullptr));
+        ACHK(build_list(ctx, S, st, total_rows, order, strips, P, 2, 0, cap, flag, nullptr, scan_tmp, list_esc, nullptr, &n_esc, nullptr));
         if (n_esc > 0)
-            ACHK(build_list(ctx, S, st, total_rows, order, strips, P, 3, 0, cap, flag, nullptr, pos, colpos, scan_tmp, list_fin, nullptr, &n_fin, nullptr));
+            ACHK(build_list(ctx, S, st, total_rows, order, strips, P, 3, 0, cap, flag, nullptr, scan_tmp, list_fin, nullptr, &n_fin, nullptr));
     }
     if (n_esc > 0) {
         if (n_fin > 0) {
@@ -1678,9 +1759,9 @@
         tk = hite_prof_begin(ctx, wname, s2);
         for (int level = 8; level <= cap; level *= 2) {
             int64_t cnt = 0;
-            ACHK(build_list(ctx, S, s2, total_rows, order, strips, P, 0, level, cap, flag2, nullptr, pos2, colpos, scan_tmp2, list, nullptr, &cnt, nullptr, 8));
+            ACHK(build_list(ctx, S, s2, total_rows, order, strips, P, 0, level, cap, flag2, nullptr, scan_tmp2, list, nullptr, &cnt, nullptr, AL_PIN2_LIST));
             if (cnt == 0) continue;
-            ACHK(assign_records(ctx, S, s2, list, cnt, strips, bk2, boff2, scan_tmp2, rec, 10));
+            ACHK(assign_records(ctx, S, s2, list, cnt, strips, bk2, boff2, scan_tmp2, rec, AL_PIN2_REC));
             const dim3 grid((unsigned)((cnt + 63) / 64));
             if (level == 8) hipLaunchKernelGGL(HIP_KERNEL_NAME(align_fwd_kernel<8>), grid, dim3(64), 0, s2, P, list, (int)cnt);
             else if (level == 16) hipLaunchKernelGGL(HIP_KERNEL_NAME(align_fwd_kernel<16>), grid, dim3(64), 0, s2, P, list, (int)cnt);
@@ -1693,42 +1774,61 @@
         hipLaunchKernelGGL(align_tb_kernel, dim3((unsigned)((n_esc + 63) / 64)), dim3(64), 0, st, P, list_esc, (int)n_esc);
         hite_prof_end(ctx, tk, st);
     } else {
-        if (nltb > 0) {
+        ne = n_early > nltb ? n_early : nltb;
+        if (!S->fallback_early) ne = nltb;
+        if (ne > 0) {
             HITE_CHECK(ctx, hipEventRecord(S->ev_fork, st));
             HITE_CHECK(ctx, hipStreamWaitEvent(s2, S->ev_fork, 0));
             snprintf(lname, sizeof lname, "align_tb_strips%s", tag ? tag : "");
             const int tl = hite_prof_begin(ctx, lname, s2);
-            hipLaunchKernelGGL(align_tb_strips_kernel, dim3((unsigned)nltb), dim3(64), 0, s2, P, order, (int)nltb);
+            if (S->lanes_min != -2) hipLaunchKernelGGL(align_tb_strips_kernel, dim3((unsigned)ne), dim3(64), 0, s2, P, order, (int)ne);
+            else hipLaunchKernelGGL(align_tb_kernel, dim3((unsigned)((ne + 63) / 64)), dim3(64), 0, s2, P, order, (int)ne);
             hite_prof_end(ctx, tl, s2);
+        }
+        if (nrows > ne) {
+            tk = hite_prof_begin(ctx, name, st);
+            hipLaunchKernelGGL(align_tb_kernel, dim3((unsigned)((nrows - ne + 63) / 64)), dim3(64), 0, st, P, order + ne, (int)(nrows - ne));
+            hite_prof_end(ctx, tk, st);
+        }
+        if (ne > 0) {
+            if (S->fallback_early) {
+                AlignArgs Pe = P;
+                ACHK(build_list(ctx, S, s2, ne, order, strips, Pe, 1, 0, cap, flag2, cols2, scan_tmp2, list_esc, full_off, &cnt_early, &tcols_early, AL_PIN2_LIST));
+                if (cnt_early > 0) {
+                    const int tl = hite_prof_begin(ctx, "align_fallback_early", s2);
+                    ACHK(aalloc(ctx, A, (size_t)tcols_early * 2 * AL_WIDE_NW + 64, &Pe.fullbuf));
+                    ACHK(aalloc(ctx, A, (size_t)tcols_early + 16, &Pe.fullt));
+                    hipLaunchKernelGGL(align_wide_fwd_kernel, dim3((unsigned)cnt_early), dim3(64), 0, s2, Pe, list_esc, (int)cnt_early);
+                    hipLaunchKernelGGL(align_wide_tb_kernel, dim3((unsigned)cnt_early), dim3(64), 0, s2, Pe, list_esc, (int)cnt_early);
+                    hite_prof_end(ctx, tl, s2);
+                }
+            }
             HITE_CHECK(ctx, hipEventRecord(S->ev_join, s2));
-        }
-        if (nrows > nltb) {
-            tk = hite_prof_begin(ctx, name, st);
-            hipLaunchKernelGGL(align_tb_kernel, dim3((unsigned)((nrows - nltb + 63) / 64)), dim3(64), 0, st, P, order + nltb, (int)(nrows - nltb));
+            HITE_CHECK(ctx, hipStreamWaitEvent(st, S->ev_join, 0));
+        }
+        if (!S->fallback_early) ne = 0;
+    }
+    HITE_CHECK(ctx, hipGetLastError());
+    int64_t cnt_rest = 0, tcols_rest = 0;
+    {
+        ACHK(build_list(ctx, S, st, total_rows - ne, order + ne, strips, P, 1, 0, cap, flag, cols, scan_tmp, list, full_off, &cnt_rest, &tcols_rest));
+        if (cnt_rest > 0) {
+            tk = hite_prof_begin(ctx, "align_fallback", st);
+            ACHK(aalloc(ctx, A, (size_t)tcols_rest * 2 * AL_WIDE_NW + 64, &P.fullbuf));
+            ACHK(aalloc(ctx, A, (size_t)tcols_rest + 16, &P.fullt));
+            hipLaunchKernelGGL(align_wide_fwd_kernel, dim3((unsigned)cnt_rest), dim3(64), 0, st, P, list, (int)cnt_rest);
+            hipLaunchKernelGGL(align_wide_tb_kernel, dim3((unsigned)cnt_rest), dim3(64), 0, st, P, list, (int)cnt_rest);
             hite_prof_end(ctx, tk, st);
         }
-        if (nltb > 0) HITE_CHECK(ctx, hipStreamWaitEvent(st, S->ev_join, 0));
-    }
-    HITE_CHECK(ctx, hipGetLastError());
-    {
-        int64_t cnt = 0, tcols = 0;
-        ACHK(build_list(ctx, S, st, total_rows, order, strips, P, 1, 0, cap, flag, cols, pos, colpos, scan_tmp, list, full_off, &cnt, &tcols));
-        if (cnt > 0) {
-            tk = hite_prof_begin(ctx, "align_fallback", st);
-            ACHK(aalloc(ctx, A, (size_t)tcols * 2 * AL_WIDE_NW + 64, &P.fullbuf));
-            ACHK(aalloc(ctx, A, (size_t)tcols + 16, &P.fullt));
-            hipLaunchKernelGGL(align_wide_fwd_kernel, dim3((unsigned)cnt), dim3(64), 0, st, P, list, (int)cnt);
-            hipLaunchKernelGGL(align_wide_tb_kernel, dim3((unsigned)cnt), dim3(64), 0, st, P, list, (int)cnt);
-            hite_prof_end(ctx, tk, st);
-        }
-    }
-    HITE_CHECK(ctx, hipMemsetAsync(S->d_scal, 0, 64, st));
+    }
+    HITE_CHECK(ctx, hipMemsetAsync(S->d_scal, 0, 56, st));
     hipLaunchKernelGGL(align_stats_kernel, dim3((unsigned)(total_rows + 255 < 1024 * 256 ? (total_rows + 255) / 256 : 1024)), dim3(256), 0, st, total_rows, strips, P, d_row_dead, d_cand_flag,
                        (unsigned long long *)S->d_scal);
     if (d_info) hipLaunchKernelGGL(align_info_kernel, dim3((unsigned)((total_rows + 255) / 256)), dim3(256), 0, st, total_rows, P, d_info);
-    HITE_CHECK(ctx, hipMemcpyAsync(S->h_pin, S->d_scal, 56, hipMemcpyDeviceToHost, st));
+    HITE_CHECK(ctx, hipMemcpyAsync(S->h_pin + AL_PIN_STATS, S->d_scal, 56, hipMemcpyDeviceToHost, st));
     HITE_CHECK(ctx, hipStreamSynchronize(st));
-    for (int q = 0; q < 7; q++) S->stats[q] += S->h_pin[q];
+    for (int q = 0; q < 7; q++) S->stats[q] += S->h_pin[AL_PIN_STATS + q];
+    if (getenv("HITE_ALIGN_DEBUG")) ACHK(align_debug_fallback(ctx, tag, total_rows, strips, P.lvl, ne, cnt_early, cnt_rest));
     HITE_CHECK(ctx, hipGetLastError());
     return HITE_OK;
 }
diff --git a/hite_amd/csrc/hite_pipeline.hip b/hite_amd/csrc/hite_pipeline.hip
--- a/hite_amd/csrc/hite_pipeline.hip
+++ b/hite_amd/csrc/hite_pipeline.hip
@@ -31,11 +31,11 @@
 }
 
 template <typename TIn>
-static int scan_excl(hite_ctx *ctx, Arena &tmp, const TIn *d_in, int64_t n, int64_t *d_out , hipStream_t st) {
+static int scan_excl(hite_ctx *ctx, Arena &tmp, const TIn *d_in, int64_t n, int64_t *d_out , hipStream_t st, int64_t *h_total = nullptr) {
     void *bs = nullptr;
     int rc = arena_alloc(ctx, tmp, (size_t)scan_tmp_elems(n) * 8, &bs);
     if (rc) return rc;
-    return scan_excl_buf<TIn>(ctx, (int64_t *)bs, d_in, n, d_out, st);
+    return scan_excl_buf<TIn>(ctx, (int64_t *)bs, d_in, n, d_out, st, h_total);
 }
 
 __global__ void mode_a_kernel(int n, const int32_t *__restrict__ copy_first, const int64_t *__restrict__ len,
@@ -346,8 +346,9 @@
 };
 struct StageTimes;
 
+enum { PIN_TOTAL = 8 };
 static int read_scalars(hite_ctx *ctx, PipeState *S, hipStream_t st, int count) {
-    HITE_CHECK(ctx, hipMemcpyAsync(S->h_pin, S->d_scal, sizeof(int64_t) * count, hipMemcpyDeviceToHost, st));
+    if (count > 0) HITE_CHECK(ctx, hipMemcpyAsync(S->h_pin, S->d_scal, sizeof(int64_t) * count, hipMemcpyDeviceToHost, st));
     HITE_CHECK(ctx, hipStreamSynchronize(st));
     return HITE_OK;
 }
@@ -371,10 +372,9 @@
                        (const int32_t *)ctx->d_contig_rank, nrows, sel);
     hite_prof_end(ctx, tk, st);
     ACHK(arena_alloc(ctx, T, (size_t)(n + 1) * 8, &p)); row_first = (int64_t *)p;
-    ACHK(scan_excl<int32_t>(ctx, T, nrows, n, row_first, st));
-    HITE_CHECK(ctx, hipMemcpyAsync(S->d_scal, row_first + n, 8, hipMemcpyDeviceToDevice, st));
-    ACHK(read_scalars(ctx, S, st, 1));
-    const int64_t total_rows = S->h_pin[0];
+    ACHK(scan_excl<int32_t>(ctx, T, nrows, n, row_first, st, S->h_pin + PIN_TOTAL));
+    ACHK(read_scalars(ctx, S, st, 0));
+    const int64_t total_rows = S->h_pin[PIN_TOTAL];
     stats[0] += total_rows;
     ACHK(arena_alloc(ctx, K, sizeof(hite_call) * (size_t)n, &p)); out->calls = (hite_call *)p;
     HITE_CHECK(ctx, hipMemsetAsync(out->calls, 0, sizeof(hite_call) * (size_t)n, st));
@@ -392,16 +392,14 @@
     hipLaunchKernelGGL(row_meta_kernel, dim3(n), dim3(128), 0, st, n, row_first, nrows, sel, d_mode, d_len, row_first32,
                        row_copy, row_len, row_pad, row_trunc, (int32_t *)(S->d_scal + 2), d_clip, d_minus, row_cp0);
     ACHK(arena_alloc(ctx, T, (size_t)(total_rows + 1) * 8, &p)); win_off = (int64_t *)p;
-    ACHK(scan_excl<int32_t>(ctx, T, row_pad, total_rows, win_off, st));
+    ACHK(scan_excl<int32_t>(ctx, T, row_pad, total_rows, win_off, st, S->h_pin + PIN_TOTAL));
     ACHK(arena_alloc(ctx, T, (size_t)n * 8, &p)); ops_cnt = (int64_t *)p;
     ACHK(arena_alloc(ctx, T, (size_t)(n + 1) * 8, &p)); ops_base = (int64_t *)p;
     hipLaunchKernelGGL(ops_count_kernel, dim3((n + 255) / 256), dim3(256), 0, st, n, row_first, nrows, row_len, ops_cnt,
                        (unsigned long long *)(S->d_scal + 4));
-    ACHK(scan_excl<int64_t>(ctx, T, ops_cnt, n, ops_base, st));
-    HITE_CHECK(ctx, hipMemcpyAsync(S->d_scal, win_off + total_rows, 8, hipMemcpyDeviceToDevice, st));
-    HITE_CHECK(ctx, hipMemcpyAsync(S->d_scal + 1, ops_base + n, 8, hipMemcpyDeviceToDevice, st));
+    ACHK(scan_excl<int64_t>(ctx, T, ops_cnt, n, ops_base, st, S->h_pin + PIN_TOTAL + 1));
     ACHK(read_scalars(ctx, S, st, 6));
-    const int64_t win_bytes = S->h_pin[0], ops_elems = S->h_pin[1];
+    const int64_t win_bytes = S->h_pin[PIN_TOTAL], ops_elems = S->h_pin[PIN_TOTAL + 1];
     const int max_len = (int)(((int32_t *)(S->h_pin + 2))[0]);
     stats[1] += win_bytes;
     stats[3] += S->h_pin[4];
@@ -439,12 +437,11 @@
         }
     }
     hipLaunchKernelGGL(msa_size_kernel, dim3((n + 255) / 256), dim3(256), 0, st, n, eff, new_cols, jcls, msa_bytes, (int32_t *)(S->d_scal + 2));
-    ACHK(scan_excl<int64_t>(ctx, T, msa_bytes, n, msa_off, st));
-    ACHK(scan_excl<int32_t>(ctx, T, new_cols, n, col_off2, st));
-    HITE_CHECK(ctx, hipMemcpyAsync(S->d_scal, col_off2 + n, 8, hipMemcpyDeviceToDevice, st));
-    HITE_CHECK(ctx, hipMemcpyAsync(S->d_scal + 1, msa_off + n, 8, hipMemcpyDeviceToDevice, st));
+    ACHK(scan_excl<int64_t>(ctx, T, msa_bytes, n, msa_off, st, S->h_pin + PIN_TOTAL + 1));
+    ACHK(scan_excl<int32_t>(ctx, T, new_cols, n, col_off2, st, S->h_pin + PIN_TOTAL));
     ACHK(read_scalars(ctx, S, st, 3));
-    const int64_t msa_total = S->h_pin[1];
+    const int64_t total_cols2 = S->h_pin[PIN_TOTAL], msa_total = S->h_pin[PIN_TOTAL + 1];
+    const int max_cols2 = (int)(((int32_t *)(S->h_pin + 2))[0]);
     stats[2] += msa_total;
     ACHK(arena_alloc(ctx, T, (size_t)msa_total + 64, &p)); clean = (uint8_t *)p;
     tk = hite_prof_begin(ctx, extra == nullptr ? "star_fill_sparse_kernel" : (pass_b ? "star_fill_sparse_kernel_passB" : "star_fill_sparse_kernel_passA"), st);
@@ -462,9 +459,7 @@
     }
     ACHK(hite_star_msa_fill_sparse_dev(ctx, n, win, win_off, row_len, row_first32, ops_base, new_cols, last_extra, msa_off, clean, st));
     hite_prof_end(ctx, tk, st);
-    const int64_t total_cols2 = S->h_pin[0];
     if (cols_acc) *cols_acc += total_cols2;
-    const int max_cols2 = (int)(((int32_t *)(S->h_pin + 2))[0]);
     ACHK(arena_alloc(ctx, K, (size_t)total_cols2 + 8 * (size_t)n + 64, &p)); out->cons = (uint8_t *)p;
     tk = hite_prof_begin(ctx, extra == nullptr ? "judge_kernel" : (pass_b ? "judge_kernel_passB" : "judge_kernel_passA"), st);
     if (max_cols2 > 0)
@@ -600,14 +595,13 @@
                   len, mode_b, &B, stats + 4, stats + 9, stats + 11, true, st));
     hipLaunchKernelGGL(merge_calls_kernel, dim3((n_cand + 255) / 256), dim3(256), 0, st, n_cand, mode_a, A.calls, B.calls, d_calls,
                        src_pass, keep_len);
-    ACHK(scan_excl<int64_t>(ctx, S->tmp, keep_len, n_cand, out_off, st));
+    ACHK(scan_excl<int64_t>(ctx, S->tmp, keep_len, n_cand, out_off, st, S->h_pin + PIN_TOTAL));
     hipLaunchKernelGGL(copy_cons_kernel, dim3(n_cand), dim3(256), 0, st, n_cand, d_calls, src_pass, A.cons, B.cons, out_off, d_cons,
                        cons_cap);
     HITE_CHECK(ctx, hipGetLastError());
-    HITE_CHECK(ctx, hipMemcpyAsync(S->d_scal, out_off + n_cand, 8, hipMemcpyDeviceToDevice, st));
-    ACHK(read_scalars(ctx, S, st, 1));
-    if (stats_out) { memcpy(stats_out, stats, sizeof stats); stats_out[10] = S->h_pin[0]; }
-    const int64_t cons_need = S->h_pin[0];
+    ACHK(read_scalars(ctx, S, st, 0));
+    const int64_t cons_need = S->h_pin[PIN_TOTAL];
+    if (stats_out) { memcpy(stats_out, stats, sizeof stats); stats_out[10] = cons_need; }
     ACHK(arena_reset(ctx, S->keep, true));
     ACHK(arena_reset(ctx, S->tmp, true));
     if (cons_need > cons_cap) return HITE_ECAP;
diff --git a/hite_amd/csrc/hite_scan.h b/hite_amd/csrc/hite_scan.h
--- a/hite_amd/csrc/hite_scan.h
+++ b/hite_amd/csrc/hite_scan.h
@@ -16,8 +16,10 @@
     __syncthreads();
     if (threadIdx.x == 0) bsum[blockIdx.x] = s_w[0] + s_w[1] + s_w[2] + s_w[3];
 }
-static __global__ void __launch_bounds__(1024) scan_bsums_kernel(int64_t *__restrict__ bsum, int64_t nb, int64_t *__restrict__ total) {
+static __global__ void __launch_bounds__(1024) scan_bsums_kernel(int64_t *__restrict__ bsum, int64_t nb, int64_t *__restrict__ total,
+                                                                 int64_t *__restrict__ h_total) {
     __shared__ long long s_w[16];
+    bsum += (int64_t)blockIdx.x * nb;
     const int lane = threadIdx.x & 63, w = threadIdx.x >> 6;
     long long carry = 0;
     for (int64_t base = 0; base < nb; base += 1024) {
@@ -33,7 +35,10 @@
         if (k < nb) bsum[k] = carry + pre + x - v;
         carry += tot;
     }
-    if (threadIdx.x == 0) *total = carry;
+    if (threadIdx.x == 0) {
+        if (total) total[blockIdx.x] = carry;
+        if (h_total) h_total[blockIdx.x] = carry;
+    }
 }
 template <typename TIn>
 static __global__ void __launch_bounds__(256) scan_apply_kernel(const TIn *__restrict__ in, int64_t n, const int64_t *__restrict__ bsum,
@@ -58,10 +63,11 @@
 }
 static inline int64_t scan_tmp_elems(int64_t n) { int64_t nb = (n + SCAN_TILE - 1) / SCAN_TILE; return nb < 1 ? 1 : nb; }
 template <typename TIn>
-static int scan_excl_buf(hite_ctx *ctx, int64_t *d_bs, const TIn *d_in, int64_t n, int64_t *d_out , hipStream_t st) {
+static int scan_excl_buf(hite_ctx *ctx, int64_t *d_bs, const TIn *d_in, int64_t n, int64_t *d_out , hipStream_t st,
+                         int64_t *h_total = nullptr) {
     int64_t nb = scan_tmp_elems(n);
     hipLaunchKernelGGL(HIP_KERNEL_NAME(scan_sums_kernel<TIn>), dim3((unsigned)nb), dim3(256), 0, st, d_in, n, d_bs);
-    hipLaunchKernelGGL(scan_bsums_kernel, dim3(1), dim3(1024), 0, st, d_bs, nb, d_out + n);
+    hipLaunchKernelGGL(scan_bsums_kernel, dim3(1), dim3(1024), 0, st, d_bs, nb, d_out + n, h_total);
     hipLaunchKernelGGL(HIP_KERNEL_NAME(scan_apply_kernel<TIn>), dim3((unsigned)nb), dim3(256), 0, st, d_in, n, d_bs, d_out);
     HITE_CHECK(ctx, hipGetLastError());
     return HITE_OK;
```

Result: no change. 655,700 candidates/s (-0.4%).
